# wzx99/DCFP

Measured on AMD Instinct MI355X. Metric: training images/sec at 1024x2048 DeepLabv3-R101, higher is better.
Workload: dtype f32; 1 GPU; DeepLabv3-resnet101+ASPP os8, 4x3x1024x2048 per GPU, CE+0.4*deepsup CE (fused upsample), 3x3 stride-1 convs with >= 256 channels as fp32 Winograd F(2x2,3x3) (fwd / dgrad / wgrad), all other convs direct implicit GEMM, EIC step, SGD m0.9 wd5e-4; global_batch=4, parallelism=dp1

## Files before the change

### dcfp_amd/_lib.py

```python
import ctypes as C
import os
import subprocess
import threading

_HERE = os.path.dirname(os.path.abspath(__file__))
LIB_PATH = os.environ.get("DCFP_LIB") or os.path.join(_HERE, "libdcfp_hip.so")
CSRC = os.path.join(_HERE, "csrc")

_lib = None
_lock = threading.Lock()


class ConvDesc(C.Structure):
    _fields_ = [(n, C.c_int32) for n in
                ("N", "Cin", "H", "W", "Cout", "KH", "KW", "stride", "pad", "dil", "Hout", "Wout",
                 "x_pitch", "dy_pitch")]


class ConvF16Desc(C.Structure):
    _fields_ = [(n, C.c_int32) for n in
                ("N", "H", "W", "Cin8", "x_pitch", "Cout", "K", "stride", "pad", "dil", "Hout", "Wout",
                 "y_pitch", "y_off", "res_pitch", "res_off", "relu")]


class ConvF8Desc(C.Structure):
    _fields_ = [(n, C.c_int32) for n in
                ("N", "H", "W", "Cin16", "x_pitch", "Cout", "K", "stride", "pad", "dil", "Hout", "Wout",
                 "y_pitch", "y_off", "res_pitch", "res_off", "relu")] + [("res_mul", C.c_float)]


class EicEntry(C.Structure):
    _fields_ = [("gamma", C.c_void_p), ("grad", C.c_void_p), ("eic", C.c_void_p),
                ("n", C.c_int32), ("pad_", C.c_int32)]


class SgdEntry(C.Structure):
    _fields_ = [("param", C.c_void_p), ("grad", C.c_void_p), ("momentum_buf", C.c_void_p),
                ("n", C.c_int64), ("first_chunk", C.c_int64),
                ("weight_decay", C.c_float), ("pad_", C.c_int32)]


class GateEntry(C.Structure):
    _fields_ = [("gamma", C.c_void_p), ("beta", C.c_void_p), ("ggrad", C.c_void_p), ("bgrad", C.c_void_p),
                ("score", C.c_void_p), ("n", C.c_int32), ("pad_", C.c_int32)]


class FilterEntry(C.Structure):
    _fields_ = [("w", C.c_void_p), ("g", C.c_void_p), ("out", C.c_void_p), ("rows", C.c_int32), ("K", C.c_int32),
                ("first_unit", C.c_int64)]


class FpgmEntry(C.Structure):
    _fields_ = [("w", C.c_void_p), ("out", C.c_void_p), ("C", C.c_int32), ("K", C.c_int32),
                ("first_tile", C.c_int64), ("ws_off", C.c_int64)]


class AdamEntry(C.Structure):
    _fields_ = [("param", C.c_void_p), ("grad", C.c_void_p), ("exp_avg", C.c_void_p), ("exp_avg_sq", C.c_void_p),
                ("n", C.c_int64), ("first_chunk", C.c_int64)]


class BnRunning(C.Structure):
    _fields_ = [("running_mean", C.c_void_p), ("running_var", C.c_void_p), ("num_batches_tracked", C.c_void_p),
                ("momentum", C.c_float), ("pad_", C.c_int32)]


class WpEntry(C.Structure):
    _fields_ = [("w", C.c_void_p), ("wp", C.c_void_p), ("first_block", C.c_int64), ("n_blocks", C.c_int64)] + \
               [(n, C.c_int32) for n in ("T", "Ck", "CkP", "M", "Mpad", "sAm", "sAc", "perm8")]


class AugTap(C.Structure):
    _fields_ = [(n, C.c_int32) for n in ("src", "c0", "c1", "lsrc")]


class AugSample(C.Structure):
    _fields_ = [("image", C.c_void_p), ("label", C.c_void_p)] + \
               [(n, C.c_int32) for n in ("src_h", "src_w", "col_off", "row_off", "lut_a_off", "lut_b_off",
                                         "hsv_flags", "hue_delta")] + \
               [("sat_alpha", C.c_float), ("pad_", C.c_int32)]


class CcSample(C.Structure):
    _fields_ = [("label", C.c_void_p)] + \
               [(n, C.c_int32) for n in ("src_h", "src_w", "dst_h", "dst_w", "Hp", "Wp", "row_off", "col_off", "cls",
                                         "pad_")] + \
               [("work_off", C.c_int64)]


class VoteMap(C.Structure):
    _fields_ = [("logits", C.c_void_p)] + [(n, C.c_int32) for n in ("h", "w", "hs", "ws", "flip")] + \
               [("weight", C.c_float)]


class SlidePass(C.Structure):
    _fields_ = [("logits", C.c_void_p)] + \
               [(n, C.c_int32) for n in ("lh", "lw", "hs", "ws", "th", "tw", "rows", "cols", "flip")] + \
               [("weight", C.c_float)]


SLIDE_MAX_PASSES, SLIDE_MAX_TILES_PER_AXIS = 16, 32
AUG_SATURATION, AUG_HUE = 1, 2
SGD_CHUNK = 16384
FILTER_ABS_SUM, FILTER_L2, FILTER_DOT_SQ_ACC = 0, 1, 2
FPGM_TILE = 64
CONV_FWD, CONV_DGRAD, CONV_WGRAD = 0, 1, 2
E_BADDESC, E_UNSUPPORTED, E_WORKSPACE = -1, -2, -3

_P, _I, _L, _F, _Z = C.c_void_p, C.c_int, C.c_int64, C.c_float, C.c_size_t
_D = C.POINTER(ConvDesc)
_R = C.POINTER(BnRunning)
_H = C.POINTER(ConvF16Desc)
_H8 = C.POINTER(ConvF8Desc)

SIGNATURES = {
    "dcfp_abi_version": (_I, []),
    "dcfp_conv2d_workspace_bytes": (_Z, [_D, _I]),
    "dcfp_conv2d_wp_layout": (_I, [_D, _I, C.POINTER(WpEntry)]),
    "dcfp_conv2d_permute_weights_multi_f32": (_I, [_P, _I, _L, _P]),
    "dcfp_conv2d_pitch_supported": (_I, [_D]),
    "dcfp_conv2d_kernel_name": (_I, [_D, _I, C.c_char_p, _I]),
    "dcfp_conv2d_executed_fraction": (C.c_double, [_D, _I]),
    "dcfp_conv2d_workspace_is_scratch": (_I, [_D, _I]),
    "dcfp_conv2d_dgrad_fanin_supported": (_I, [_D]),
    "dcfp_conv2d_dgrad_fanin_f32_nchw": (_I, [_D, _P, _L, _P, _P, _P, _P, _P, _Z, _I, _P]),
    "dcfp_conv2d_dgrad_fanin_red_slots": (_L, [_D]),
    "dcfp_conv2d_dgrad_fanin_red_f32_nchw": (_I, [_D, _P, _L, _P, _P, _P, _P, _P, _P, _P, _P, _P, _Z, _I, _P]),
    "dcfp_bn_bwd_sums_from_partials_f32": (_I, [_P, _L, _I, _P, _F, _P, _P, _P, _P, _P]),
    "dcfp_conv2d_xform_bytes": (_Z, [_D]),
    "dcfp_conv2d_fwd_keep_f32_nchw": (_I, [_D, _P, _P, _P, _L, _P, _Z, _P, _P, _Z, _P]),
    "dcfp_conv2d_wgrad_kept_f32_nchw": (_I, [_D, _P, _L, _P, _Z, _P, _P, _Z, _P]),
    "dcfp_conv2d_fwd_f32_nchw": (_I, [_D, _P, _P, _P, _P, _L, _P, _Z, _I, _P]),
    "dcfp_conv2d_fwd_fused_f32_nchw": (_I, [_D, _P, _P, _P, _P, _P, _I, _P, _P, _Z, _I, _P]),
    "dcfp_conv2d_dgrad_f32_nchw": (_I, [_D, _P, _L, _P, _P, _I, _P, _Z, _I, _P]),
    "dcfp_conv2d_wgrad_f32_nchw": (_I, [_D, _P, _L, _P, _P, _P, _P, _Z, _P]),
    "dcfp_bn_workspace_bytes": (_Z, [_I, _I, _I]),
    "dcfp_bn_stats_f32": (_I, [_P, _L, _I, _I, _I, _P, _P, _R, _P, _Z, _P]),
    "dcfp_bn_apply_f32": (_I, [_P, _P, _P, _P, _P, _F, _P, _I, _P, _L, _I, _I, _I, _I, _I, _P]),
    "dcfp_bn_bwd_reduce_f32": (_I, [_P, _L, _P, _P, _L, _P, _P, _P, _P, _F, _I, _I, _I, _I, _P, _P, _P, _P,
                                    _P, _Z, _P]),
    "dcfp_bn_update_running_f32": (_I, [_P, _P, _I, _F, _F, _P, _P, _P, _P]),
    "dcfp_syncbn_combine_f32": (_I, [_P, _I, _I, _P, _P, _P, _R, _P]),
    "dcfp_syncbn_p2p_mailbox_bytes": (_Z, [_I, _I]),
    "dcfp_p2p_alloc": (_I, [_Z, _I, C.POINTER(C.c_void_p)]),
    "dcfp_p2p_free": (_I, [_P]),
    "dcfp_p2p_export": (_I, [_P, _P]),
    "dcfp_p2p_import": (_I, [_P, C.POINTER(C.c_void_p)]),
    "dcfp_p2p_unmap": (_I, [_P]),
    "dcfp_syncbn_p2p_exchange_f32": (_I, [C.POINTER(C.c_void_p), _I, _I, C.c_uint32, _I, _P, _I, _I, _P, _R,
                                          C.c_uint32, _P, _P]),
    "dcfp_bn_apply_relu_mask_f32": (_I, [_P, _P, _P, _P, _P, _F, _P, _P, _P, _I, _I, _I, _P]),
    "dcfp_conv2d_fwd_stat_slots": (_L, [_D, _P, _L]),
    "dcfp_conv2d_fwd_stats_f32_nchw": (_I, [_D, _P, _P, _P, _L, _P, _P, _Z, _I, _P]),
    "dcfp_bn_stats_from_partials_f32": (_I, [_P, _L, _I, _I, _P, _P, _R, _P]),
    "dcfp_bn_bwd_apply_f32": (_I, [_P, _L, _P, _P, _L, _P, _P, _P, _P, _F, _P, _P, _F, _P, _I, _P, _P,
                                   _I, _I, _I, _I, _I, _P]),
    "dcfp_bn_bwd_fused_sync_bytes": (_Z, [_I, _I, _I]),
    "dcfp_bn_bwd_fused_f32": (_I, [_P, _L, _P, _P, _L, _P, _P, _P, _P, _F, _F, _I, _P, _P, _I, _I, _I, _I, _I,
                                   _P, _P, _P, _P, _P, _Z, C.c_uint32, C.c_uint32, _P, _P]),
    "dcfp_maxpool3x3s2_fwd_f32": (_I, [_P, _P, _P, _I, _I, _I, _I, _I, _I, _P]),
    "dcfp_maxpool3x3s2_bwd_f32": (_I, [_P, _P, _P, _I, _I, _I, _I, _I, _I, _P]),
    "dcfp_rowsum_f32": (_I, [_P, _L, _P, _F, _I, _I, _I, _P]),
    "dcfp_broadcast_hw_f32": (_I, [_P, _F, _P, _L, _I, _I, _I, _I, _P]),
    "dcfp_add_f32": (_I, [_P, _P, _P, _L, _P]),
    "dcfp_channel_scale_f32": (_I, [_P, _P, _P, _I, _I, _I, _P]),
    "dcfp_upsample_bilinear_fwd_f32": (_I, [_P, _P, _I, _I, _I, _I, _I, _I, _I, _P]),
    "dcfp_upsample_bilinear_bwd_f32": (_I, [_P, _P, _I, _I, _I, _I, _I, _I, _I, _P]),
    "dcfp_resize_bilinear_into_f32": (_I, [_P, _L, _I, _I, _I, _I, _P, _L, _I, _I, _I, _I, _P]),
    "dcfp_resize_bilinear_adjoint_f32": (_I, [_P, _L, _I, _I, _I, _I, _I, _P, _L, _I, _I, _I, _I, _P]),
    "dcfp_ppm_pool_f32": (_I, [_P, _I, _I, _I, _I, _I, _P, _P, _I, _P, _L, _I, _P]),
    "dcfp_ppm_pool_adjoint_f32": (_I, [_P, _I, _I, _I, _I, _I, _P, _P, _L, _I, _P, _P]),
    "dcfp_ppm_resize_adjoint_f32": (_I, [_P, _L, _I, _I, _I, _I, _I, _P, _P, _I, _P]),
    "dcfp_upsample_ce_workspace_bytes": (_Z, [_I, _I, _I]),
    "dcfp_upsample_ce_fwd_f32": (_I, [_P, _P, _P, _I, _I, _I, _I, _I, _I, _I, _I, _P, _P, _P, _P,
                                      _Z, _P]),
    "dcfp_upsample_ce_bwd_f32": (_I, [_P, _P, _P, _I, _I, _I, _I, _I, _I, _I, _I, _P, _P, _P, _P]),
    "dcfp_upsample_ce_bwd_plan": (_I, [_I, _I, _I, _I, _I, _I, C.POINTER(C.c_int), C.POINTER(C.c_int),
                                       C.POINTER(C.c_int)]),
    "dcfp_ohem_zoom_gt_prob_f32": (_I, [_P, _P, _P, _I, _I, _I, _I, _I, _I, _I, _I, _I, _P, _P, _P]),
    "dcfp_ohem_threshold_f32": (_I, [_P, _P, _L, _I, _F, _L, _P, _P]),
    "dcfp_ohem_keep_mask_u8": (_I, [_P, _P, _L, _P, _P]),
    "dcfp_upsample_margin_f32": (_I, [_P, _I, _I, _I, _I, _I, _I, _I, _P, _P]),
    "dcfp_maxfilter2d_s1_f32": (_I, [_P, _P, _I, _I, _I, _I, _P]),
    "dcfp_upsample_wce_workspace_bytes": (_Z, [_I, _I, _I]),
    "dcfp_upsample_wce_fwd_f32": (_I, [_P, _P, _P, _I, _I, _I, _I, _I, _I, _I, _I, _P, _P, _P, _Z, _P]),
    "dcfp_upsample_wce_bwd_f32": (_I, [_P, _P, _P, _I, _I, _I, _I, _I, _I, _I, _I, _P, _P, _P, _P]),
    "dcfp_upsample_argmax_f32": (_I, [_P, _I, _I, _I, _I, _I, _I, _I, _P, _P]),
    "dcfp_confusion_matrix_i64": (_I, [_P, _P, _I, _L, _I, _P, _P]),
    "dcfp_vote_multiscale_f32": (_I, [C.POINTER(VoteMap), _I, _I, _I, _I, _I, _I, _I, _I, _P, _P, _P, _I, _P, _P]),
    "dcfp_gather_tiles_f32": (_I, [_P, _I, _I, _I, _I, _P, _I, _P, _I, _I, _I, _I, _P, _P]),
    "dcfp_vote_sliding_f32": (_I, [C.POINTER(SlidePass), _I, _P, _P, _I, _I, _I, _I, _I, _I, _I, _P, _P, _P, _I, _P, _P]),
    "dcfp_label_boundary_workspace_bytes": (_Z, [_I, _I, _I]),
    "dcfp_label_boundary_i32": (_I, [_P, _P, _I, _I, _I, _I, _I, _I, _P, _Z, _P]),
    "dcfp_label_boundary_i64": (_I, [_P, _P, _I, _I, _I, _I, _I, _I, _P, _Z, _P]),
    "dcfp_png_deflate_bound": (_Z, [_I, _I]),
    "dcfp_png_deflate_workspace_bytes": (_Z, [_I, _I, _I, _I]),
    "dcfp_png_deflate_labels_i32": (_I, [_P, _I, _I, _I, _P, _I, _P, _Z, _P, _P, _P, _Z, _P]),
    "dcfp_augment_u8_to_f32_nchw": (_I, [C.POINTER(AugSample), _I, _I, _I, _P, _L, _P, _L, _P, _L, _P, _I, _P, _P, _P, _P]),
    "dcfp_balance_weight_f32": (_I, [_P, _P, _P, _I, _L, _I, _I, _I, C.c_double, _P, _P]),
    "dcfp_components_workspace_bytes": (_Z, [_I, _I]),
    "dcfp_label_components_u8": (_I, [C.POINTER(CcSample), _I, _P, _L, _P, _P, _Z, _P, _P]),
    "dcfp_component_pixel_i32": (_I, [C.POINTER(CcSample), _I, _P, _Z, _P, _P, _P, _P, _P]),
    "dcfp_eic_update_f32": (_I, [_P, _I, _F, _F, _P]),
    "dcfp_sgd_momentum_f32": (_I, [_P, _I, _L, _F, _F, _I, _P]),
    "dcfp_adamw_f32": (_I, [_P, _I, _L, _F, _F, _F, _F, _F, _F, _F, _P]),
    "dcfp_conv2d_fwd_f16_nhwc": (_I, [_H, _P, _P, _P, _P, _P, _P]),
    "dcfp_conv2d_fwd_f16_nhwc_to_f32_nchw": (_I, [_H, _P, _P, _P, _P, _P]),
    "dcfp_maxpool3x3s2_nhwc_f16": (_I, [_P, _P, _I, _I, _I, _I, _I, _I, _I, _I, _P]),
    "dcfp_avgpool_nhwc_f16_workspace_bytes": (_Z, [_I, _I, _L]),
    "dcfp_avgpool_nhwc_f16": (_I, [_P, _P, _I, _L, _I, _I, _I, _P, _Z, _P]),
    "dcfp_broadcast_nhwc_f16": (_I, [_P, _I, _P, _I, _L, _I, _I, _I, _P]),
    "dcfp_nchw_f32_to_nhwc_f16": (_I, [_P, _P, _I, _I, _I, _I, _I, _P]),
    "dcfp_conv2d_fwd_f8_nhwc": (_I, [_H8, _P, _P, _P, _P, _P, _P, _P]),
    "dcfp_conv2d_fwd_f8_nhwc_to_f32_nchw": (_I, [_H8, _P, _P, _P, _P, _P, _P]),
    "dcfp_cast_nhwc_f16_to_f8": (_I, [_P, _I, _P, _I, _I, _L, _I, _F, _P]),
    "dcfp_maxpool3x3s2_nhwc_f8": (_I, [_P, _P, _I, _I, _I, _I, _I, _I, _I, _I, _P]),
    "dcfp_avgpool_nhwc_f8_to_f16": (_I, [_P, _P, _I, _L, _I, _I, _I, _F, _P, _Z, _P]),
    "dcfp_broadcast_nhwc_f16_to_f8": (_I, [_P, _I, _P, _I, _L, _I, _I, _I, _F, _P]),
    "dcfp_resize_bilinear_nhwc_f16": (_I, [_P, _I, _I, _I, _I, _I, _P, _I, _I, _I, _I, _I, _P]),
    "dcfp_pyramid_pool_nhwc_f16_workspace_bytes": (_Z, [_I, _I, _I, _I, _I, _P]),
    "dcfp_pyramid_pool_nhwc_f16": (_I, [_P, _I, _I, _I, _I, _I, _I, _I, _P, _P, _P, _P, _Z, _P]),
    "dcfp_kd_workspace_bytes": (_Z, [_I, _I, _I, _I, _I]),
    "dcfp_kd_fwd_f32": (_I, [_P, _P, _I, _I, _I, _I, _I, _F, _P, _Z, _P, _P, _P]),
    "dcfp_lovasz_workspace_bytes": (_Z, [_I, _I]),
    "dcfp_lovasz_hist_f32": (_I, [_P, _P, _I, _I, _I, _I, _I, _I, _I, _I, _I, _P, _P, _Z, _P]),
    "dcfp_lovasz_scan_f32": (_I, [_I, _I, _P, _Z, _P, _P, _P]),
    "dcfp_lovasz_bwd_f32": (_I, [_P, _P, _I, _I, _I, _I, _I, _I, _I, _I, _I, _P, _P, _P, _P, _P, _P]),
    "dcfp_lovasz_errors_u32": (_I, [_P, _P, _I, _I, _I, _I, _I, _I, _I, _I, _P, _P]),
    "dcfp_gate_taylor_f32": (_I, [_P, _I, _P]),
    "dcfp_gate_l1reg_f32": (_I, [_P, _I, _F, _P]),
    "dcfp_filter_reduce_units": (_L, [_I, _I]),
    "dcfp_filter_reduce_f32": (_I, [_P, _I, _L, _I, _P]),
    "dcfp_fpgm_workspace_bytes": (_Z, [_I]),
    "dcfp_fpgm_f32": (_I, [_P, _I, _L, _P, _Z, _P]),
}


def build(verbose=False):
    cmd = ["make", "-C", CSRC, "-j", str(min(8, os.cpu_count() or 1))]
    r = subprocess.run(cmd, capture_output=True, text=True)
    if verbose or r.returncode != 0:
        print(r.stdout[-4000:])
        print(r.stderr[-4000:])
    if r.returncode != 0:
        raise RuntimeError("building libdcfp_hip.so failed")
    return LIB_PATH


def lib():
    global _lib
    if _lib is not None:
        return _lib
    with _lock:
        if _lib is not None:
            return _lib
        if not os.path.exists(LIB_PATH):
            raise RuntimeError(
                f"{LIB_PATH} not found: run `python -c 'import __graft_entry__ as g; g.build()'` "
                "(or `make -C dcfp_amd/csrc`). dcfp_amd has no non-HIP fallback.")
        try:
            import torch
        except Exception:
            pass
        handle = C.CDLL(LIB_PATH, mode=C.RTLD_GLOBAL)
        for name, (res, args) in SIGNATURES.items():
            fn = getattr(handle, name)
            fn.restype = res
            fn.argtypes = args
        _lib = handle
    return _lib


def check(status, what):
    if status != 0:
        kind = "descriptor/shape" if status < 0 else "hipError_t"
        raise RuntimeError(f"{what} failed: status {status} ({kind})")
```

### dcfp_amd/csrc/conv_igemm.hip

```cpp
#include "common.h"
#include <string.h>
#include <stdio.h>
#include <stdlib.h>

namespace {

int check_desc(const DcfpConvDesc* d) {
    if (!d) return DCFP_E_BADDESC;
    if (d->N <= 0 || d->Cin <= 0 || d->Cout <= 0 || d->H <= 0 || d->W <= 0 || d->stride <= 0 ||
        d->dil <= 0 || d->pad < 0)
        return DCFP_E_BADDESC;
    if (d->KH != d->KW || (d->KH != 1 && d->KH != 3)) return DCFP_E_UNSUPPORTED;
    const int ho = (d->H + 2 * d->pad - d->dil * (d->KH - 1) - 1) / d->stride + 1;
    const int wo = (d->W + 2 * d->pad - d->dil * (d->KW - 1) - 1) / d->stride + 1;
    if (ho != d->Hout || wo != d->Wout || ho <= 0 || wo <= 0) return DCFP_E_BADDESC;
    if ((d->x_pitch != 0 && (d->x_pitch < d->W || (d->x_pitch & 3))) ||
        (d->dy_pitch != 0 && (d->dy_pitch < d->Wout || (d->dy_pitch & 3))))
        return DCFP_E_BADDESC;
    if ((long long)d->Cin * d->H * (d->x_pitch ? d->x_pitch : d->W) >= (1LL << 29) ||
        (long long)d->Cout * d->Hout * (d->dy_pitch ? d->dy_pitch : d->Wout) >= (1LL << 29) ||
        (long long)d->Cout * d->Cin * d->KH * d->KW >= (1LL << 29))
        return DCFP_E_UNSUPPORTED;
    return DCFP_OK;
}

}

extern "C" int dcfp_abi_version(void) { return 2; }

int dcfp_wgrad_kernel_name(const DcfpConvDesc* d, char* buf, int buf_len);
double dcfp_wgrad_exec_fraction(const DcfpConvDesc* d);
double dcfp_igemm2_exec_fraction(int T, int M, int Ck, int N, int Hi, int Wi, int Ho, int Wo, int sn, int sd,
                                 int off0, int offstep, bool pitched);
size_t dcfp_igemm2_workspace_bytes(int T, int M, int Ck, long long px, int sd);
const char* dcfp_igemm2_cfg_args(int M, long long px, int sd);
int dcfp_igemm2_run(const float* in, long long in_nstride, const float* w, int sAm, int sAc,
                    const float* bias, float* out, long long out_nstride, int N, int M, int Ck, int T,
                    int Hi, int Wi, int Ho, int Wo, int sn, int sd, int off0, int offstep,
                    int accumulate, void* workspace, size_t workspace_bytes, hipStream_t stream,
                    const float* scale = nullptr, const float* shift = nullptr,
                    const float* residual = nullptr, int relu = 0, float* stat_part = nullptr, int wp_valid = 0,
                    int in_pitch = 0, long long wp_nstride = 0, const float* fan_src = nullptr,
                    const unsigned long long* fan_mask = nullptr, const Igemm2Red* red = nullptr);
bool dcfp_wino_ok(int N, int H, int W, int d, int M, int Ck);
size_t dcfp_wino_workspace_bytes(int N, int H, int W, int d, int M, int Ck);
double dcfp_wino_exec_fraction(int N, int H, int W, int d, int M, int Ck);
int dcfp_wino_run(const float* in, long long in_nstride, int in_pitch, const float* w, int sAm, int sAc, int flip,
                  float* out, long long out_nstride, int N, int M, int Ck, int H, int W, int d, int accumulate,
                  void* workspace, size_t workspace_bytes, hipStream_t stream, float* xform_out = nullptr,
                  float* stat_part = nullptr, const float* scale = nullptr, const float* shift = nullptr,
                  const float* residual = nullptr, int relu = 0, int wp_valid = 0);
long long dcfp_wino_stat_slots(int N, int H, int W, int d);
bool dcfp_stem_shape(const DcfpConvDesc* d);
int dcfp_stem_fwd(const DcfpConvDesc* d, const float* x, const float* w, const float* bias, float* y, long long y_nstride,
                  hipStream_t stream, float* stat_part = nullptr);
long long dcfp_stem_stat_slots(const DcfpConvDesc* d, const float* y, long long y_nstride);
bool dcfp_gemv_shape(const DcfpConvDesc* d);
int dcfp_gemv_fwd(const DcfpConvDesc* d, const float* x, const float* w, const float* bias, float* y, long long y_nstride,
                  hipStream_t stream);
int dcfp_gemv_dgrad(const DcfpConvDesc* d, const float* dy, long long dy_nstride, const float* w, float* dx, int accumulate,
                    hipStream_t stream);
bool dcfp_wino_fused_ok(int N, int H, int W, int d, int M, int Ck, long long in_nstride, int pitch);
size_t dcfp_wino_fused_workspace_bytes(int N, int H, int W, int d, int M, int Ck);
void dcfp_wino_fused_pads(int N, int H, int W, int d, int M, int Ck, int* CkP, int* Mpad);
size_t dcfp_wino_xform_bytes(int N, int H, int W, int d, int C);
bool dcfp_wgrad_is_winograd(const DcfpConvDesc* d);
bool dcfp_wgrad_wants_xform(const DcfpConvDesc* d);
long long dcfp_igemm2_stat_slots(int M, int P, int N, long long out_nstride, const float* out);
bool dcfp_igemm2_dma_shape(int T, int M, int Ck, int P, long long px, int sn, int sd, int off0, int HiWi, int Wo);
bool dcfp_igemm2_persist();
void dcfp_igemm2_wp_layout(int T, int M, int Ck, int P, long long px, int sn, int sd, int off0, int offstep, int HiWi,
                           int Wo, bool pitched, int sAm, int sAc, DcfpWpEntry* e);
bool dcfp_igemm2_use_dma8(int T, int M, int P, long long px, int sn, int sd, int off0, int offstep, int HiWi,
                          int Wo, bool pitched);
int dcfp_igemm2_permute_multi(const DcfpWpEntry* table, int n, long long total_blocks, hipStream_t stream);


size_t dcfp_igemm3_workspace_bytes(int T, int M, int Ck);
int dcfp_igemm3_run(const float* in, long long in_nstride, const float* w, int sAm, int sAc,
                    const float* bias, float* out, long long out_nstride, int N, int M, int Ck, int T,
                    int Hi, int Wi, int Ho, int Wo, int off0, int offstep, int accumulate,
                    void* workspace, size_t workspace_bytes, hipStream_t stream,
                    const float* scale = nullptr, const float* shift = nullptr,
                    const float* residual = nullptr, int relu = 0, int wp_valid = 0);
int dcfp_igemm2_cfg_id(int M, long long px, int sd);
static bool math_bf16x3() {
    static const bool v = [] { const char* e = getenv("DCFP_CONV_MATH"); return e && !strcmp(e, "bf16x3"); }();
    return v;
}
static bool igemm3_ok(int M, long long px, int sn, int sd) {
    return math_bf16x3() && sn == 1 && sd == 1 && dcfp_igemm2_cfg_id(M, px, sd) == 4;
}

static int wino_kind(const DcfpConvDesc* d, int pass) {
    static const int mode = [] { const char* e = getenv("DCFP_CONV_WINOGRAD"); return e ? atoi(e) : 1; }();
    if (mode == 0) return 0;
    if (d->KH != 3 || d->KW != 3 || d->stride != 1 || d->pad != d->dil || d->Hout != d->H || d->Wout != d->W)
        return 0;
    if (math_bf16x3()) return 0;
    const bool fwd = pass == DCFP_CONV_FWD;
    const int M = fwd ? d->Cout : d->Cin, Ck = fwd ? d->Cin : d->Cout;
    const int sp = fwd ? d->x_pitch : d->dy_pitch;
    const bool pitched = sp && sp != d->W;
    const bool three = dcfp_wino_ok(d->N, d->H, d->W, d->dil, M, Ck);
    const bool fused = dcfp_wino_fused_ok(d->N, d->H, d->W, d->dil, M, Ck, (long long)Ck * d->H * (sp ? sp : d->W), sp);
    if (!three && !fused) return 0;
    if (mode == 2) return three ? 1 : 2;
    const double nominal = 2.0 * d->N * (double)d->H * d->W * (double)M * Ck * 9.0;
    const double f_direct = fwd ? dcfp_igemm2_exec_fraction(9, M, Ck, d->N, d->H, d->W, d->H, d->W, 1, 1, -d->pad, d->dil, pitched)
                                : dcfp_igemm2_exec_fraction(9, M, Ck, d->N, d->H, d->W, d->H, d->W, 1, 1, d->pad, -d->dil, pitched);
    const double t_direct = nominal * f_direct / (M % 256 != 0 ? 115e12 : 143e12);
    const double f_wino = dcfp_wino_exec_fraction(d->N, d->H, d->W, d->dil, M, Ck);
    double t_wino = 1e30;
    if (three) {
        const double tiles = f_wino * 9.0 / 16.0 * d->N * (double)d->H * d->W;
        const double rate = Ck <= 256 ? (M >= 1024 ? 130e12 : 118e12) : (M <= 256 ? 127e12 : 135e12);
        const double pix = (double)d->N * d->H * d->W;
        const double t_in = (4.0 * pix * Ck + 64.0 * tiles * Ck) / 4.2e12;
        const double t_out = (64.0 * tiles * M + 4.0 * pix * M * (fwd ? 1.0 : 2.0)) / 5.4e12;
        const double mpad = (double)((M + 255) / 256 * 256) / M;
        t_wino = nominal * f_wino * mpad / rate + t_in + t_out + 20e-6;
    }
    if (fused) {
        const double nk = (double)((Ck + 15) / 16 * 2);
        const double mpad = (double)((M + 63) / 64 * 64) / M;
        const double t_f = nominal * f_wino * mpad / (125e12 * nk / (nk + 4.0)) + 10e-6;
        if (t_f < t_wino) t_wino = t_f;
    }
    if (!(t_wino < 0.97 * t_direct)) return 0;
    return three ? 1 : 2;
}
static bool wino_pass(const DcfpConvDesc* d, int pass) { return wino_kind(d, pass) != 0; }

static bool wino_keeps_u(const DcfpConvDesc* d, int pass) {
    static const bool on = [] { const char* e = getenv("DCFP_WINO_KEEP_U"); return !e || atoi(e) != 0; }();
    if (!on || (pass != DCFP_CONV_FWD && pass != DCFP_CONV_DGRAD) || !wino_pass(d, pass)) return false;
    const bool fwd = pass == DCFP_CONV_FWD;
    const int M = fwd ? d->Cout : d->Cin, Ck = fwd ? d->Cin : d->Cout;
    const int sp = fwd ? d->x_pitch : d->dy_pitch;
    if (!dcfp_wino_fused_ok(d->N, d->H, d->W, d->dil, M, Ck, (long long)Ck * d->H * (sp ? sp : d->W), sp)) return false;
    if (fwd && Ck > 256 && dcfp_wino_ok(d->N, d->H, d->W, d->dil, M, Ck) && dcfp_conv2d_xform_bytes(d) > 0) return false;
    return true;
}

extern "C" int dcfp_conv2d_workspace_is_scratch(const DcfpConvDesc* d, int pass) {
    if (check_desc(d) != DCFP_OK || pass == DCFP_CONV_WGRAD) return 0;
    return (wino_pass(d, pass) && !wino_keeps_u(d, pass)) ? 1 : 0;
}

size_t dcfp_conv2d_fwd_dgrad_workspace_bytes_(const DcfpConvDesc* d, int pass) {
    if (check_desc(d) != DCFP_OK) return 0;
    if (const int wk = wino_kind(d, pass)) {
        const int M = pass == DCFP_CONV_FWD ? d->Cout : d->Cin, Ck = pass == DCFP_CONV_FWD ? d->Cin : d->Cout;
        if (wino_keeps_u(d, pass)) {
            const size_t u = dcfp_wino_fused_workspace_bytes(d->N, d->H, d->W, d->dil, M, Ck);
            const size_t direct = dcfp_igemm2_workspace_bytes(9, M, Ck, (long long)d->N * d->H * d->W, 1);
            return u > direct ? u : direct;
        }
        return wk == 1 ? dcfp_wino_workspace_bytes(d->N, d->H, d->W, d->dil, M, Ck)
                       : dcfp_wino_fused_workspace_bytes(d->N, d->H, d->W, d->dil, M, Ck);
    }
    const int T = d->KH * d->KW;
    size_t b2, b3 = 0;
    if (pass == DCFP_CONV_FWD) {
        const long long px = (long long)d->N * d->Hout * d->Wout;
        b2 = dcfp_igemm2_workspace_bytes(T, d->Cout, d->Cin, px, 1);
        if (igemm3_ok(d->Cout, px, d->stride, 1)) b3 = dcfp_igemm3_workspace_bytes(T, d->Cout, d->Cin);
    } else {
        const long long px = (long long)d->N * d->H * d->W;
        b2 = dcfp_igemm2_workspace_bytes(T, d->Cin, d->Cout, px, d->stride);
        if (igemm3_ok(d->Cin, px, 1, d->stride)) b3 = dcfp_igemm3_workspace_bytes(T, d->Cin, d->Cout);
    }
    return b2 > b3 ? b2 : b3;
}

extern "C" int dcfp_conv2d_kernel_name(const DcfpConvDesc* d, int pass, char* buf, int buf_len) {
    int rc = check_desc(d);
    if (rc) return rc;
    if (!buf || buf_len <= 0) return DCFP_E_BADDESC;
    if (dcfp_gemv_shape(d)) return snprintf(buf, buf_len, "gemv_1x1_map_kernel");
    if (pass == DCFP_CONV_WGRAD) return dcfp_wgrad_kernel_name(d, buf, buf_len);
    if (pass == DCFP_CONV_FWD && dcfp_stem_shape(d)) return snprintf(buf, buf_len, "stem_fwd_kernel");
    if (const int wk = wino_kind(d, pass))
        return wk == 1 ? snprintf(buf, buf_len, "winograd_f2x2_3x3 (igemm2_dma1p_kernel<false,true>)")
                       : snprintf(buf, buf_len, "winograd_f2x2_3x3 fused (wino_fused_kernel)");
    const int M = pass == DCFP_CONV_FWD ? d->Cout : d->Cin;
    const long long px = pass == DCFP_CONV_FWD ? (long long)d->N * d->Hout * d->Wout : (long long)d->N * d->H * d->W;
    const int sd = pass == DCFP_CONV_FWD ? 1 : d->stride;
    if (igemm3_ok(M, px, pass == DCFP_CONV_FWD ? d->stride : 1, sd))
        return snprintf(buf, buf_len, "igemm3_kernel<%d>", d->KH * d->KW);
    const int P = pass == DCFP_CONV_FWD ? d->Hout * d->Wout : d->H * d->W;
    const int HiWi = pass == DCFP_CONV_FWD ? d->H * d->W : d->Hout * d->Wout;
    const int Ck = pass == DCFP_CONV_FWD ? d->Cin : d->Cout;
    {
        const int sp = pass == DCFP_CONV_FWD ? d->x_pitch : d->dy_pitch;
        const bool pitched = sp && sp != (pass == DCFP_CONV_FWD ? d->W : d->Wout);
        if (dcfp_igemm2_use_dma8(d->KH * d->KW, M, P, px, pass == DCFP_CONV_FWD ? d->stride : 1, sd,
                                 pass == DCFP_CONV_FWD ? -d->pad : d->pad, pass == DCFP_CONV_FWD ? d->dil : -d->dil,
                                 HiWi, pass == DCFP_CONV_FWD ? d->Wout : d->W, pitched))
            return snprintf(buf, buf_len, "igemm2_dma8_kernel<%d>", d->KH * d->KW);
    }
    if (dcfp_igemm2_dma_shape(d->KH * d->KW, M, Ck, P, px, pass == DCFP_CONV_FWD ? d->stride : 1, sd, d->pad, HiWi,
                              pass == DCFP_CONV_FWD ? d->Wout : d->W)) {
        if (d->KH == 1 && dcfp_igemm2_persist()) return snprintf(buf, buf_len, "igemm2_dma1p_kernel");
        const int src_pitch = pass == DCFP_CONV_FWD ? d->x_pitch : d->dy_pitch;
        const bool pitched = src_pitch && src_pitch != (pass == DCFP_CONV_FWD ? d->W : d->Wout);
        return snprintf(buf, buf_len, "igemm2_dma_kernel<%d,%s>", d->KH * d->KW,
                        (d->KH == 3 && ((d->pad | d->dil) & 3) != 0 && !pitched) ? "true" : "false");
    }
    return snprintf(buf, buf_len, "igemm2_kernel<%d,%s>", d->KH * d->KW, dcfp_igemm2_cfg_args(M, px, sd));
}

extern "C" double dcfp_conv2d_executed_fraction(const DcfpConvDesc* d, int pass) {
    if (check_desc(d) != DCFP_OK) return 1.0;
    if (pass == DCFP_CONV_WGRAD) return dcfp_wgrad_exec_fraction(d);
    const bool fwd = pass == DCFP_CONV_FWD;
    if (wino_pass(d, pass))
        return fwd ? dcfp_wino_exec_fraction(d->N, d->H, d->W, d->dil, d->Cout, d->Cin)
                   : dcfp_wino_exec_fraction(d->N, d->H, d->W, d->dil, d->Cin, d->Cout);
    const int M = fwd ? d->Cout : d->Cin;
    const long long px = fwd ? (long long)d->N * d->Hout * d->Wout : (long long)d->N * d->H * d->W;
    if (igemm3_ok(M, px, fwd ? d->stride : 1, fwd ? 1 : d->stride)) return 1.0;
    const int sp = fwd ? d->x_pitch : d->dy_pitch;
    const bool pitched = sp && sp != (fwd ? d->W : d->Wout);
    return fwd ? dcfp_igemm2_exec_fraction(d->KH * d->KW, d->Cout, d->Cin, d->N, d->H, d->W, d->Hout, d->Wout, d->stride, 1,
                                           -d->pad, d->dil, pitched)
               : dcfp_igemm2_exec_fraction(d->KH * d->KW, d->Cin, d->Cout, d->N, d->Hout, d->Wout, d->H, d->W, 1, d->stride,
                                           d->pad, -d->dil, pitched);
}

extern "C" int64_t dcfp_conv2d_fwd_stat_slots(const DcfpConvDesc* d, const float* y, int64_t y_nstride);

extern "C" size_t dcfp_conv2d_xform_bytes(const DcfpConvDesc* d) {
    if (check_desc(d) != DCFP_OK) return 0;
    if (!wino_pass(d, DCFP_CONV_FWD) || !dcfp_wgrad_wants_xform(d)) return 0;
    return dcfp_wino_xform_bytes(d->N, d->H, d->W, d->dil, d->Cin);
}

extern "C" int dcfp_conv2d_fwd_keep_f32_nchw(const DcfpConvDesc* d, const float* x, const float* w, float* y,
                                             int64_t y_nstride, float* xform_out, size_t xform_bytes,
                                             float* stat_partials, void* workspace, size_t workspace_bytes,
                                             dcfp_stream_t stream) {
    int rc = check_desc(d);
    if (rc) return rc;
    if (!x || !w || !y || !xform_out) return DCFP_E_BADDESC;
    const size_t need = dcfp_conv2d_xform_bytes(d);
    if (need == 0) return DCFP_E_UNSUPPORTED;
    if (xform_bytes < need) return DCFP_E_WORKSPACE;
    const int T = 9;
    return dcfp_wino_run(x, (long long)d->Cin * d->H * (d->x_pitch ? d->x_pitch : d->W), d->x_pitch, w, d->Cin * T, T, 0, y,
                         y_nstride ? y_nstride : (long long)d->Cout * d->Hout * d->Wout, d->N, d->Cout, d->Cin, d->H, d->W,
                         d->dil, 0, workspace, workspace_bytes, dcfp_s(stream), xform_out,
                         (stat_partials && dcfp_conv2d_fwd_stat_slots(d, y, y_nstride) > 0) ? stat_partials : nullptr);
}

extern "C" int dcfp_conv2d_fwd_f32_nchw(const DcfpConvDesc* d, const float* x, const float* w,
                                        const float* bias, float* y, int64_t y_nstride,
                                        void* workspace, size_t workspace_bytes, int wp_valid,
                                        dcfp_stream_t stream) {
    int rc = check_desc(d);
    if (rc) return rc;
    if (!x || !w || !y) return DCFP_E_BADDESC;
    const int T = d->KH * d->KW;
    if (d->x_pitch && d->x_pitch != d->W && math_bf16x3()) return DCFP_E_UNSUPPORTED;
    if (dcfp_gemv_shape(d)) return dcfp_gemv_fwd(d, x, w, bias, y, y_nstride, dcfp_s(stream));
    if (dcfp_stem_shape(d)) return dcfp_stem_fwd(d, x, w, bias, y, y_nstride, dcfp_s(stream));
    if (!bias && wino_pass(d, DCFP_CONV_FWD))
        return dcfp_wino_run(x, (long long)d->Cin * d->H * (d->x_pitch ? d->x_pitch : d->W), d->x_pitch, w, d->Cin * T, T,
                             0, y, y_nstride ? y_nstride : (long long)d->Cout * d->Hout * d->Wout, d->N, d->Cout,
                             d->Cin, d->H, d->W, d->dil, 0, workspace, workspace_bytes, dcfp_s(stream), nullptr, nullptr,
                             nullptr, nullptr, nullptr, 0, (wp_valid && wino_keeps_u(d, DCFP_CONV_FWD)) ? 1 : 0);
    if (!bias && igemm3_ok(d->Cout, (long long)d->N * d->Hout * d->Wout, d->stride, 1))
        return dcfp_igemm3_run(x, (long long)d->Cin * d->H * d->W, w, d->Cin * T, T, bias, y,
                               y_nstride ? y_nstride : (long long)d->Cout * d->Hout * d->Wout, d->N,
                               d->Cout, d->Cin, T, d->H, d->W, d->Hout, d->Wout, -d->pad, d->dil, 0,
                               workspace, workspace_bytes, dcfp_s(stream), nullptr, nullptr, nullptr, 0, wp_valid);
    return dcfp_igemm2_run(x, (long long)d->Cin * d->H * (d->x_pitch ? d->x_pitch : d->W), w, d->Cin * T, T, bias, y,
                           y_nstride ? y_nstride : (long long)d->Cout * d->Hout * d->Wout, d->N,
                           d->Cout, d->Cin, T, d->H, d->W, d->Hout, d->Wout, d->stride, 1, -d->pad,
                           d->dil, 0, workspace, workspace_bytes, dcfp_s(stream), nullptr, nullptr, nullptr, 0,
                           nullptr, wp_valid, d->x_pitch);
}

extern "C" int64_t dcfp_conv2d_fwd_stat_slots(const DcfpConvDesc* d, const float* y, int64_t y_nstride) {
    if (check_desc(d) != DCFP_OK) return 0;
    if (dcfp_stem_shape(d)) return dcfp_stem_stat_slots(d, y, y_nstride);
    if (wino_pass(d, DCFP_CONV_FWD))
        return (y_nstride % 4 == 0 && dcfp_aligned16(y)) ? dcfp_wino_stat_slots(d->N, d->H, d->W, d->dil) : 0;
    if (igemm3_ok(d->Cout, (long long)d->N * d->Hout * d->Wout, d->stride, 1)) return 0;
    return dcfp_igemm2_stat_slots(d->Cout, d->Hout * d->Wout, d->N,
                                  y_nstride ? y_nstride : (long long)d->Cout * d->Hout * d->Wout, y);
}

extern "C" int dcfp_conv2d_fwd_stats_f32_nchw(const DcfpConvDesc* d, const float* x, const float* w,
                                              float* y, int64_t y_nstride, float* stat_partials,
                                              void* workspace, size_t workspace_bytes, int wp_valid,
                                              dcfp_stream_t stream) {
    int rc = check_desc(d);
    if (rc) return rc;
    if (!x || !w || !y || !stat_partials) return DCFP_E_BADDESC;
    if (dcfp_conv2d_fwd_stat_slots(d, y, y_nstride) <= 0) return DCFP_E_UNSUPPORTED;
    const int T = d->KH * d->KW;
    if (dcfp_stem_shape(d)) return dcfp_stem_fwd(d, x, w, nullptr, y, y_nstride, dcfp_s(stream), stat_partials);
    if (wino_pass(d, DCFP_CONV_FWD))
        return dcfp_wino_run(x, (long long)d->Cin * d->H * (d->x_pitch ? d->x_pitch : d->W), d->x_pitch, w, d->Cin * T, T, 0, y,
                             y_nstride ? y_nstride : (long long)d->Cout * d->Hout * d->Wout, d->N, d->Cout, d->Cin, d->H, d->W,
                             d->dil, 0, workspace, workspace_bytes, dcfp_s(stream), nullptr, stat_partials, nullptr, nullptr,
                             nullptr, 0, (wp_valid && wino_keeps_u(d, DCFP_CONV_FWD)) ? 1 : 0);
    return dcfp_igemm2_run(x, (long long)d->Cin * d->H * (d->x_pitch ? d->x_pitch : d->W), w, d->Cin * T, T, nullptr, y,
                           y_nstride ? y_nstride : (long long)d->Cout * d->Hout * d->Wout, d->N,
                           d->Cout, d->Cin, T, d->H, d->W, d->Hout, d->Wout, d->stride, 1, -d->pad,
                           d->dil, 0, workspace, workspace_bytes, dcfp_s(stream), nullptr, nullptr,
                           nullptr, 0, stat_partials, wp_valid, d->x_pitch);
}

extern "C" int dcfp_conv2d_dgrad_f32_nchw(const DcfpConvDesc* d, const float* dy,
                                          int64_t dy_nstride, const float* w, float* dx,
                                          int accumulate, void* workspace, size_t workspace_bytes,
                                          int wp_valid, dcfp_stream_t stream) {
    int rc = check_desc(d);
    if (rc) return rc;
    if (!dy || !w || !dx) return DCFP_E_BADDESC;
    const int T = d->KH * d->KW;
    if (d->dy_pitch && d->dy_pitch != d->Wout && math_bf16x3()) return DCFP_E_UNSUPPORTED;
    if (dcfp_gemv_shape(d)) return dcfp_gemv_dgrad(d, dy, dy_nstride, w, dx, accumulate ? 1 : 0, dcfp_s(stream));
    if (wino_pass(d, DCFP_CONV_DGRAD))
        return dcfp_wino_run(dy, dy_nstride ? dy_nstride : (long long)d->Cout * d->Hout * (d->dy_pitch ? d->dy_pitch : d->Wout),
                             d->dy_pitch, w, T, d->Cin * T, 1, dx, (long long)d->Cin * d->H * d->W, d->N, d->Cin, d->Cout,
                             d->H, d->W, d->dil, accumulate ? 1 : 0, workspace, workspace_bytes, dcfp_s(stream), nullptr,
                             nullptr, nullptr, nullptr, nullptr, 0, (wp_valid && wino_keeps_u(d, DCFP_CONV_DGRAD)) ? 1 : 0);
    if (igemm3_ok(d->Cin, (long long)d->N * d->H * d->W, 1, d->stride))
        return dcfp_igemm3_run(dy, dy_nstride ? dy_nstride : (long long)d->Cout * d->Hout * d->Wout, w,
                               T, d->Cin * T, nullptr, dx, (long long)d->Cin * d->H * d->W, d->N, d->Cin,
                               d->Cout, T, d->Hout, d->Wout, d->H, d->W, d->pad, -d->dil,
                               accumulate ? 1 : 0, workspace, workspace_bytes, dcfp_s(stream), nullptr, nullptr,
                               nullptr, 0, wp_valid);
    return dcfp_igemm2_run(dy, dy_nstride ? dy_nstride : (long long)d->Cout * d->Hout * (d->dy_pitch ? d->dy_pitch : d->Wout), w,
                           T, d->Cin * T, nullptr, dx, (long long)d->Cin * d->H * d->W, d->N, d->Cin,
                           d->Cout, T, d->Hout, d->Wout, d->H, d->W, 1, d->stride, d->pad, -d->dil,
                           accumulate ? 1 : 0, workspace, workspace_bytes, dcfp_s(stream), nullptr, nullptr, nullptr, 0,
                           nullptr, wp_valid, d->dy_pitch);
}

extern "C" int dcfp_conv2d_dgrad_fanin_supported(const DcfpConvDesc* d) {
    if (check_desc(d) != DCFP_OK || d->KH != 1 || d->stride != 1 || d->pad != 0 || math_bf16x3()) return 0;
    const int P = d->H * d->W;
    const long long px = (long long)d->N * P;
    if (d->Cin % 256 != 0 || P % 256 != 0 || !dcfp_igemm2_persist()) return 0;
    if (igemm3_ok(d->Cin, px, 1, 1)) return 0;
    return dcfp_igemm2_dma_shape(1, d->Cin, d->Cout, P, px, 1, 1, 0, P, d->W) ? 1 : 0;
}

extern "C" int dcfp_conv2d_dgrad_fanin_f32_nchw(const DcfpConvDesc* d, const float* dy, int64_t dy_nstride, const float* w,
                                                float* dx, const float* fan_src, const void* fan_mask, void* workspace,
                                                size_t workspace_bytes, int wp_valid, dcfp_stream_t stream) {
    int rc = check_desc(d);
    if (rc) return rc;
    if (!dy || !w || !dx || !fan_src || !fan_mask) return DCFP_E_BADDESC;
    if (!dcfp_conv2d_dgrad_fanin_supported(d)) return DCFP_E_UNSUPPORTED;
    return dcfp_igemm2_run(dy, dy_nstride ? dy_nstride : (long long)d->Cout * d->Hout * d->Wout, w, 1, d->Cin, nullptr, dx,
                           (long long)d->Cin * d->H * d->W, d->N, d->Cin, d->Cout, 1, d->Hout, d->Wout, d->H, d->W, 1, 1, 0, -1,
                           0, workspace, workspace_bytes, dcfp_s(stream), nullptr, nullptr, nullptr, 0, nullptr, wp_valid, 0, 0,
                           fan_src, static_cast<const unsigned long long*>(fan_mask));
}

bool dcfp_igemm2p_fan_red_ok(int Mpad, int CkP);
int dcfp_igemm2_ck_pad();
extern "C" int64_t dcfp_conv2d_dgrad_fanin_red_slots(const DcfpConvDesc* d) {
    if (!dcfp_conv2d_dgrad_fanin_supported(d)) return 0;
    const int pad = dcfp_igemm2_ck_pad();
    const int ckp = (d->Cout + pad - 1) / pad * pad;
    if (!dcfp_igemm2p_fan_red_ok(d->Cin, ckp)) return 0;
    return (int64_t)d->N * d->H * d->W / 128;
}

extern "C" int dcfp_conv2d_dgrad_fanin_red_f32_nchw(const DcfpConvDesc* d, const float* dy, int64_t dy_nstride,
                                                    const float* w, float* dx, const float* fan_src, const void* fan_mask,
                                                    const float* red_x, const void* red_mask, const float* red_mean,
                                                    float* red_part, void* workspace, size_t workspace_bytes, int wp_valid,
                                                    dcfp_stream_t stream) {
    int rc = check_desc(d);
    if (rc) return rc;
    if (!dy || !w || !dx || !fan_src || !fan_mask || !red_x || !red_mask || !red_mean || !red_part) return DCFP_E_BADDESC;
    if (dcfp_conv2d_dgrad_fanin_red_slots(d) <= 0) return DCFP_E_UNSUPPORTED;
    if (reinterpret_cast<uintptr_t>(red_part) & 7u) return DCFP_E_BADDESC;
    const Igemm2Red red = {red_x, static_cast<const unsigned long long*>(red_mask), red_mean, red_part};
    return dcfp_igemm2_run(dy, dy_nstride ? dy_nstride : (long long)d->Cout * d->Hout * d->Wout, w, 1, d->Cin, nullptr, dx,
                           (long long)d->Cin * d->H * d->W, d->N, d->Cin, d->Cout, 1, d->Hout, d->Wout, d->H, d->W, 1, 1, 0, -1,
                           0, workspace, workspace_bytes, dcfp_s(stream), nullptr, nullptr, nullptr, 0, nullptr, wp_valid, 0, 0,
                           fan_src, static_cast<const unsigned long long*>(fan_mask), &red);
}

extern "C" int dcfp_conv2d_fwd_fused_f32_nchw(const DcfpConvDesc* d, const float* x, const float* w,
                                              const float* scale, const float* shift,
                                              const float* residual, int relu, float* y,
                                              void* workspace, size_t workspace_bytes, int wp_valid,
                                              dcfp_stream_t stream) {
    int rc = check_desc(d);
    if (rc) return rc;
    if (!x || !w || !y || !scale || !shift) return DCFP_E_BADDESC;
    const int T = d->KH * d->KW;
    if (wino_pass(d, DCFP_CONV_FWD))
        return dcfp_wino_run(x, (long long)d->Cin * d->H * d->W, 0, w, d->Cin * T, T, 0, y,
                             (long long)d->Cout * d->Hout * d->Wout, d->N, d->Cout, d->Cin, d->H, d->W, d->dil, 0, workspace,
                             workspace_bytes, dcfp_s(stream), nullptr, nullptr, scale, shift, residual, relu ? 1 : 0);
    if (igemm3_ok(d->Cout, (long long)d->N * d->Hout * d->Wout, d->stride, 1))
        return dcfp_igemm3_run(x, (long long)d->Cin * d->H * d->W, w, d->Cin * T, T, nullptr, y,
                               (long long)d->Cout * d->Hout * d->Wout, d->N, d->Cout, d->Cin, T, d->H, d->W,
                               d->Hout, d->Wout, -d->pad, d->dil, 0, workspace, workspace_bytes,
                               dcfp_s(stream), scale, shift, residual, relu ? 1 : 0, wp_valid);
    return dcfp_igemm2_run(x, (long long)d->Cin * d->H * d->W, w, d->Cin * T, T, nullptr, y,
                           (long long)d->Cout * d->Hout * d->Wout, d->N, d->Cout, d->Cin, T, d->H, d->W,
                           d->Hout, d->Wout, d->stride, 1, -d->pad, d->dil, 0, workspace, workspace_bytes,
                           dcfp_s(stream), scale, shift, residual, relu ? 1 : 0, nullptr, wp_valid);
}

extern "C" int dcfp_conv2d_wp_layout(const DcfpConvDesc* d, int pass, DcfpWpEntry* e) {
    int rc = check_desc(d);
    if (rc) return rc;
    if (!e || (pass != DCFP_CONV_FWD && pass != DCFP_CONV_DGRAD)) return DCFP_E_BADDESC;
    const int T = d->KH * d->KW;
    if (wino_pass(d, pass)) {
        if (!wino_keeps_u(d, pass)) return DCFP_E_UNSUPPORTED;
        const bool fwd = pass == DCFP_CONV_FWD;
        e->T = 16; e->M = fwd ? d->Cout : d->Cin; e->Ck = fwd ? d->Cin : d->Cout;
        dcfp_wino_fused_pads(d->N, d->H, d->W, d->dil, e->M, e->Ck, &e->CkP, &e->Mpad);
        e->sAm = fwd ? d->Cin * T : T; e->sAc = fwd ? T : d->Cin * T; e->perm8 = fwd ? 2 : 3;
        const long long pairs = (long long)e->CkP * e->Mpad;
        e->n_blocks = (pairs + DCFP_WP_BLOCK_ELEMS - 1) / DCFP_WP_BLOCK_ELEMS;
        return DCFP_OK;
    }
    if (pass == DCFP_CONV_FWD) {
        const long long px = (long long)d->N * d->Hout * d->Wout;
        if (igemm3_ok(d->Cout, px, d->stride, 1)) return DCFP_E_UNSUPPORTED;
        dcfp_igemm2_wp_layout(T, d->Cout, d->Cin, d->Hout * d->Wout, px, d->stride, 1, -d->pad, d->dil, d->H * d->W,
                              d->Wout, d->x_pitch && d->x_pitch != d->W, d->Cin * T, T, e);
    } else {
        const long long px = (long long)d->N * d->H * d->W;
        if (igemm3_ok(d->Cin, px, 1, d->stride)) return DCFP_E_UNSUPPORTED;
        dcfp_igemm2_wp_layout(T, d->Cin, d->Cout, d->H * d->W, px, 1, d->stride, d->pad, -d->dil, d->Hout * d->Wout,
                              d->W, d->dy_pitch && d->dy_pitch != d->Wout, T, d->Cin * T, e);
    }
    const long long total = (long long)e->T * e->CkP * e->Mpad;
    e->n_blocks = (total + DCFP_WP_BLOCK_ELEMS - 1) / DCFP_WP_BLOCK_ELEMS;
    return DCFP_OK;
}

extern "C" int dcfp_conv2d_permute_weights_multi_f32(const DcfpWpEntry* table, int n, int64_t total_blocks,
                                                     dcfp_stream_t stream) {
    if (n == 0 || total_blocks == 0) return DCFP_OK;
    if (!table || n < 0 || total_blocks < 0 || total_blocks > 0x7fffffffLL) return DCFP_E_BADDESC;
    return dcfp_igemm2_permute_multi(table, n, total_blocks, dcfp_s(stream));
}

bool dcfp_wgrad_pitch_ok(const DcfpConvDesc* d);

extern "C" int dcfp_conv2d_pitch_supported(const DcfpConvDesc* d) {
    if (check_desc(d) != DCFP_OK || math_bf16x3()) return 0;
    if (d->KH != 3 || d->stride != 1 || d->pad != d->dil || d->Hout != d->H || d->Wout != d->W) return 0;
    const int xp = d->x_pitch ? d->x_pitch : d->W, dp = d->dy_pitch ? d->dy_pitch : d->Wout;
    if (xp < d->W + d->pad && xp != d->W) return 0;
    if (dp < d->Wout + d->pad && dp != d->Wout) return 0;
    const long long pxo = (long long)d->N * d->Hout * d->Wout, pxi = (long long)d->N * d->H * d->W;
    if (xp != d->W && dp != d->Wout && wino_kind(d, DCFP_CONV_FWD) == 2 && wino_kind(d, DCFP_CONV_DGRAD) == 2)
        return dcfp_wgrad_pitch_ok(d) ? 1 : 0;
    if (!dcfp_igemm2_dma_shape(9, d->Cout, d->Cin, d->Hout * d->Wout, pxo, 1, 1, -d->pad, d->H * d->W, d->Wout) &&
        !dcfp_igemm2_use_dma8(9, d->Cout, d->Hout * d->Wout, pxo, 1, 1, -d->pad, d->dil, d->H * d->W, d->Wout, true))
        return 0;
    if (!dcfp_igemm2_dma_shape(9, d->Cin, d->Cout, d->H * d->W, pxi, 1, 1, d->pad, d->Hout * d->Wout, d->W) &&
        !dcfp_igemm2_use_dma8(9, d->Cin, d->H * d->W, pxi, 1, 1, d->pad, -d->dil, d->Hout * d->Wout, d->W, true))
        return 0;
    return dcfp_wgrad_pitch_ok(d) ? 1 : 0;
}
```

### dcfp_amd/csrc/conv_igemm2.hip

```cpp
#include "igemm2_common.h"
#include <queue>
#include <vector>
#include <stdio.h>
#include <stdlib.h>

namespace {

__device__ __forceinline__ int wp_row(int m, int perm8) {
    if (!perm8) return m;
    const int j = m & 255;
    return (m & ~255) + 32 * (j & 7) + (j >> 3);
}

__global__ void __launch_bounds__(256)
permute_weights_kernel(const float* __restrict__ w, float* __restrict__ wp, int T, int Ck, int CkP,
                       int M, int Mpad, int sAm, int sAc, int perm8) {
    const long long total = (long long)T * CkP * Mpad;
    for (long long i = (long long)blockIdx.x * 256 + threadIdx.x; i < total;
         i += (long long)gridDim.x * 256) {
        const int m = wp_row((int)(i % Mpad), perm8);
        const long long r = i / Mpad;
        const int c = (int)(r % CkP);
        const int t = (int)(r / CkP);
        float v = 0.f;
        if (m < M && c < Ck) v = w[(long long)m * sAm + (long long)c * sAc + t];
        wp[i] = v;
    }
}

constexpr int kWpBlockElems = DCFP_WP_BLOCK_ELEMS;
__global__ void __launch_bounds__(256)
permute_weights_multi_kernel(const DcfpWpEntry* __restrict__ table, int n) {
    const long long blk = blockIdx.x;
    int lo = 0, hi = n - 1;
    while (lo < hi) {
        const int mid = (lo + hi + 1) >> 1;
        if (table[mid].first_block <= blk) lo = mid; else hi = mid - 1;
    }
    const DcfpWpEntry e = table[lo];
    const long long base = (blk - e.first_block) * kWpBlockElems;
    if (e.perm8 >= 2) {
        const long long pairs = (long long)e.CkP * e.Mpad;
#pragma unroll 1
        for (int u = 0; u < kWpBlockElems / 256; ++u) {
            const long long i = base + u * 256 + threadIdx.x;
            if (i >= pairs) return;
            wino_filter2_pair(e.w, e.sAm, e.sAc, e.perm8 == 3, e.M, e.Ck, e.Mpad, i, e.wp);
        }
        return;
    }
    const long long total = (long long)e.T * e.CkP * e.Mpad;
#pragma unroll
    for (int u = 0; u < kWpBlockElems / 256; ++u) {
        const long long i = base + u * 256 + threadIdx.x;
        if (i >= total) return;
        const int m = wp_row((int)(i % e.Mpad), e.perm8);
        const long long r = i / e.Mpad;
        const int c = (int)(r % e.CkP);
        const int t = (int)(r / e.CkP);
        float v = 0.f;
        if (m < e.M && c < e.Ck) v = e.w[(long long)m * e.sAm + (long long)c * e.sAc + t];
        e.wp[i] = v;
    }
}

__device__ __forceinline__ float half_xor(float v, int mask) {
    switch (mask) {
        case 1: return __builtin_bit_cast(float, __builtin_amdgcn_ds_swizzle(__builtin_bit_cast(int, v), (1 << 10) | 0x1f));
        case 2: return __builtin_bit_cast(float, __builtin_amdgcn_ds_swizzle(__builtin_bit_cast(int, v), (2 << 10) | 0x1f));
        case 4: return __builtin_bit_cast(float, __builtin_amdgcn_ds_swizzle(__builtin_bit_cast(int, v), (4 << 10) | 0x1f));
        case 8: return __builtin_bit_cast(float, __builtin_amdgcn_ds_swizzle(__builtin_bit_cast(int, v), (8 << 10) | 0x1f));
        default: return __builtin_bit_cast(float, __builtin_amdgcn_ds_swizzle(__builtin_bit_cast(int, v), (16 << 10) | 0x1f));
    }
}

template <int TAPS, int TM, int TN, int WM, int WN, bool SD, bool ACC, int KB = 16>
__global__ void __launch_bounds__(64 * WM * WN, (TM * TN <= 8 && WM * WN == 4 && !ACC) ? 2 : 1)
igemm2_kernel(const Igemm2Params p) {
    constexpr int BK = KB;
    constexpr int NPART = BK / 4;
    constexpr int BM = WM * TM * 32, BN = WN * TN * 32, NT = 64 * WM * WN;
    constexpr int AX = BM / 4;
    constexpr int AROWS = (NT / AX) < BK ? (NT / AX) : BK;
    constexpr int APASS = BK / AROWS;
    constexpr int TX = BN / 4, TY = NT / TX, RPT = BK / TY;
    static_assert(APASS >= 1 && APASS * AROWS == BK, "A loader shape");
    static_assert(TY >= 1 && RPT >= 1 && TY * RPT == BK, "B loader shape");

    extern __shared__ __attribute__((aligned(16))) float smem[];
    float* As = smem;
    float* Bs = smem + 2 * BK * BM;

    const int group = 8 * p.tiles_m;
    const int g = blockIdx.x / group, local = blockIdx.x - g * group;
    const int nt = g * 8 + (local & 7);
    const int mt = local >> 3;
    if (nt >= p.tiles_n_total) return;
    const int img = nt / p.tiles_per_img;
    const int ti_img = nt - img * p.tiles_per_img;
    const int phase = SD ? (p.zfold ? p.zfold - 1 : ti_img / p.tiles_per_phase) : 0;
    const int ph_h = SD ? phase / p.sd : 0, ph_w = SD ? phase - ph_h * p.sd : 0;
    const int p0 = (SD && !p.zfold ? ti_img - phase * p.tiles_per_phase : ti_img) * BN;
    const int m0 = mt * BM;

    const int tid = threadIdx.x;
    const int lane = tid & 63, wid = tid >> 6;
    const int wm = wid / WN, wn = wid - wm * WN;
    const int l31 = lane & 31, lhi = lane >> 5;

    const int ax = tid % AX, ay = tid / AX;
    const bool a_on = ay < BK;
    const float* a_src = p.wp + m0 + 4 * ax;

    const int tx = tid % TX, ty = tid / TX;
    int bh[4], bw[4];
    bool pv[4];
#pragma unroll
    for (int e = 0; e < 4; ++e) {
        const int pp = p0 + 4 * tx + e;
        if constexpr (SD) {
            const int a = pp / p.Wc, b = pp - a * p.Wc;
            const int oh = a * p.sd + ph_h, ow = b * p.sd + ph_w;
            pv[e] = a < p.Hc && oh < p.Ho && ow < p.Wo;
            bh[e] = oh * p.sn;
            bw[e] = ow * p.sn;
        } else {
            pv[e] = pp < p.P;
            const int oh = pp / p.Wo;
            const int ow = pp - oh * p.Wo;
            bh[e] = oh * p.sn;
            bw[e] = ow * p.sn;
        }
    }
    const int HiWi = p.Hi * p.Wi;
    const __amdgpu_buffer_rsrc_t b_rsrc = __builtin_amdgcn_make_buffer_rsrc(
        const_cast<float*>(p.in + (long long)img * p.in_nstride), 0, p.Ck * HiWi * 4, 0x00020000);

    const int ksteps_per_tap = p.CkP / BK;
    unsigned long long tap_list = 0;
    int ntaps = TAPS;
    if constexpr (SD) {
        ntaps = 0;
        for (int t = 0; t < TAPS; ++t) {
            const int kh = (TAPS == 9) ? t / 3 : 0, kw = (TAPS == 9) ? t - kh * 3 : 0;
            const int sh = ph_h + p.off0 + kh * p.offstep, sw = ph_w + p.off0 + kw * p.offstep;
            if (sh % p.sd == 0 && sw % p.sd == 0) {
                tap_list |= (unsigned long long)t << (4 * ntaps);
                ++ntaps;
            }
        }
    }
    const int nk = ntaps * ksteps_per_tap;

    unsigned boff[4];
    bool bvec = false;
    f32x4 areg[APASS];
    float breg[RPT][4];

    auto set_tap = [&](int t) {
        const int kh = (TAPS == 9) ? t / 3 : 0;
        const int kw = (TAPS == 9) ? t - kh * 3 : 0;
        const int offh = p.off0 + kh * p.offstep;
        const int offw = p.off0 + kw * p.offstep;
#pragma unroll
        for (int e = 0; e < 4; ++e) {
            int hh = bh[e] + offh, ww = bw[e] + offw;
            bool ok = pv[e] && hh >= 0 && ww >= 0;
            if (SD) {
                ok = ok && (hh % p.sd == 0) && (ww % p.sd == 0);
                hh /= p.sd;
                ww /= p.sd;
            }
            ok = ok && hh < p.Hi && ww < p.Wi;
            boff[e] = ok ? (unsigned)(hh * p.Wi + ww) * 4u : kOob;
        }
        const bool none = boff[0] == kOob && boff[1] == kOob && boff[2] == kOob && boff[3] == kOob;
        const bool run = boff[0] != kOob && boff[1] == boff[0] + 4u && boff[2] == boff[0] + 8u &&
                         boff[3] == boff[0] + 12u;
        bvec = none || run;
    };
    auto load_part = [&](int kt, auto part_) {
        constexpr int PART = decltype(part_)::value;
#ifdef DCFP_TAP_INNER
        const int cb = kt / TAPS;
        const int t = kt - cb * TAPS;
        const int c0 = cb * BK;
        if (PART == 0 && (TAPS > 1 || kt == 0)) set_tap(t);
#else
        const int ti_ = kt / ksteps_per_tap;
        const int c0 = (kt - ti_ * ksteps_per_tap) * BK;
        const int t = SD ? (int)((tap_list >> (4 * ti_)) & 15ull) : ti_;
        if (PART == 0 && c0 == 0) set_tap(t);
#endif
        static_for<0, APASS>([&](auto j_) {
            constexpr int j = decltype(j_)::value;
            if constexpr ((j % NPART) == PART) {
                if (a_on)
                    areg[j] = *reinterpret_cast<const f32x4*>(
                        a_src + (long long)(t * p.CkP + c0 + ay + AROWS * j) * p.Mpad);
            }
        });
        static_for<0, RPT>([&](auto q_) {
            constexpr int q = decltype(q_)::value;
// ... 656 lines not shown
size_t dcfp_igemm2_workspace_bytes(int T, int M, int Ck, long long px, int sd) {
    return (size_t)T * round_up(Ck, ck_pad()) * round_up(M, 256) * sizeof(float);
}

int dcfp_igemm2_cfg_id(int M, long long px, int sd) { return pick_cfg(M, px, sd).id; }

long long dcfp_igemm2_stat_slots(int M, int P, int N, long long out_nstride, const float* out) {
    const TileCfg c = pick_cfg(M, (long long)N * P, 1);
    if (c.id != 0 && c.id != 1 && c.id != 2 && c.id != 4) return 0;
    if (M % c.bm != 0 || P % c.bn != 0 || P % 4 != 0 || out_nstride % 4 != 0 || !dcfp_aligned16(out)) return 0;
    return (long long)N * (P / c.bn) * (c.bn / 128);
}

const char* dcfp_igemm2_cfg_args(int M, long long px, int sd) {
    switch (pick_cfg(M, px, sd).id) {
        case 0: return "1,4,1,4,0";
        case 1: return "2,4,1,4,0";
        case 2: return "2,4,2,2,0";
        case 3: return "2,2,2,2,0";
        case 4: return "4,4,2,2,0";
        default: return "2,4,2,2,1";
    }
}

bool dcfp_igemm2_use_dma8(int T, int M, int P, long long px, int sn, int sd, int off0, int offstep, int HiWi,
                          int Wo, bool pitched) {
    static const int mode = [] { const char* e = getenv("DCFP_IGEMM_DMA8"); return e ? atoi(e) : 1; }();
    static const bool dma = [] { const char* e = getenv("DCFP_IGEMM_DMA"); return !e || atoi(e) != 0; }();
    const bool on = mode != 0;
    if (!on || !dma || deep_k() || sn != 1 || sd != 1 || HiWi != P || Wo % 4 != 0) return false;
    if (T == 1 ? off0 != 0 : ((((off0 | offstep) & 3) != 0 && !pitched) || off0 + 2 * offstep != -off0)) return false;
    const long long tiles = ((long long)P + 255) / 256 * (px / P) * ((M + 255) / 256);
    if (tiles < 192) return false;
    if (mode == 2) return true;
    const TileCfg c = pick_cfg(M, px, sd);
    if (M % c.bm == 0) return false;
    if (c.bm <= 64) return true;
    const long long old_rows = (long long)((M + c.bm - 1) / c.bm) * c.bm, new_rows = (long long)((M + 31) / 32) * 32;
    return 10 * new_rows <= 9 * old_rows;
}

bool dcfp_igemm2_dma_shape(int T, int M, int Ck, int P, long long px, int sn, int sd, int off0, int HiWi, int Wo);

static int tile_live_rows(const Igemm2Params& p, int ti) {
    int oh_lo, oh_hi;
    if (p.tile2d) {
        const int rows = 256 >> p.tile2d;
        oh_lo = (ti / (p.Wi >> p.tile2d)) * rows;
        oh_hi = oh_lo + rows - 1;
    } else {
        const int p0 = ti * 256;
        oh_lo = p0 / p.Wo;
        oh_hi = (p0 + 255 < p.P ? p0 + 255 : p.P - 1) / p.Wo;
    }
    oh_hi = oh_hi < p.Ho ? oh_hi : p.Ho - 1;
    int lo = 0, hi = 2;
    auto live = [&](int kh) { const int o = p.off0 + kh * p.offstep; return oh_hi + o >= 0 && oh_lo + o < p.Hi; };
    while (lo < 2 && !live(lo)) ++lo;
    while (hi > lo && !live(hi)) --hi;
    return hi - lo + 1;
}

static int pick_tapskip(const Igemm2Params& p, int bn) {
    static const int forced = [] { const char* e = getenv("DCFP_IGEMM_TAPSKIP"); return e ? atoi(e) : -1; }();
    if (bn != 256) return 0;
    const bool t2d = p.tile2d != 0;
    if (forced >= 0) return (forced == 2 && t2d) ? 1 : forced;
    if (t2d) return 1;
    struct Key { int Ho, Wo, Hi, N, tm, off0, offstep, mode; };
    thread_local Key cache[16];
    thread_local int used = 0;
    for (int i = 0; i < used; ++i) {
        const Key& k = cache[i];
        if (k.Ho == p.Ho && k.Wo == p.Wo && k.Hi == p.Hi && k.N == p.N && k.tm == p.tiles_m && k.off0 == p.off0 &&
            k.offstep == p.offstep)
            return k.mode;
    }
    const int T = p.tiles_per_img, cus = dcfp_num_cus();
    std::vector<float> work((size_t)T);
    bool any = false;
    for (int ti = 0; ti < T; ++ti) {
        const int live = tile_live_rows(p, ti);
        any |= live < 3;
        work[ti] = (float)live + 0.1f;
    }
    int mode = 0;
    if (any) {
        auto makespan = [&](int m) {
            std::priority_queue<float, std::vector<float>, std::greater<float>> free_at;
            for (int i = 0; i < cus; ++i) free_at.push(0.f);
            float end = 0.f;
            const long long groups = ((long long)p.tiles_n_total + 7) / 8;
            for (long long g = 0; g < groups; ++g)
                for (int mt = 0; mt < p.tiles_m; ++mt)
                    for (int l = 0; l < 8; ++l) {
                        const long long nt = g * 8 + l;
                        if (nt >= p.tiles_n_total) continue;
                        int ti = (int)(nt % T);
                        if (m == 2) {
                            const int k = (int)(nt / p.N), c = T >> 1;
                            ti = (k & 1) ? c - 1 - (k >> 1) : c + (k >> 1);
                        }
                        const float t0 = free_at.top();
                        free_at.pop();
                        const float t1 = t0 + (m == 0 ? 3.1f : work[ti]);
                        free_at.push(t1);
                        end = t1 > end ? t1 : end;
                    }
            return end;
        };
        const float m0 = makespan(0), m1 = makespan(1), m2 = makespan(2);
        const float best = m2 <= m1 ? m2 : m1;
        if (best <= 0.97f * m0) mode = m2 <= m1 ? 2 : 1;
    }
    if (used < 16) {
        cache[used++] = Key{p.Ho, p.Wo, p.Hi, p.N, p.tiles_m, p.off0, p.offstep, mode};
    }
    return mode;
}

double dcfp_igemm2_exec_fraction(int T, int M, int Ck, int N, int Hi, int Wi, int Ho, int Wo, int sn, int sd,
                                 int off0, int offstep, bool pitched) {
    if (T != 9 || sn != 1 || sd != 1) return 1.0;
    const long long px = (long long)N * Ho * Wo;
    const bool d8 = dcfp_igemm2_use_dma8(T, M, Ho * Wo, px, sn, sd, off0, offstep, Hi * Wi, Wo, pitched);
    if (!d8 && !dcfp_igemm2_dma_shape(T, M, Ck, Ho * Wo, px, sn, sd, off0, Hi * Wi, Wo)) return 1.0;
    Igemm2Params p = {};
    p.N = N; p.Hi = Hi; p.Wi = Wi; p.Ho = Ho; p.Wo = Wo; p.P = Ho * Wo; p.off0 = off0; p.offstep = offstep;
    p.tiles_per_img = (p.P + 255) / 256; p.tiles_n_total = p.tiles_per_img * N; p.tiles_m = (M + 255) / 256;
    {
        static const int t2d = [] { const char* e = getenv("DCFP_IGEMM_2D"); return e ? atoi(e) : 5; }();
        const bool fits = (t2d == 4 || t2d == 5) && Hi % (256 >> t2d) == 0 && Wi % (1 << t2d) == 0;
        p.tile2d = (!d8 && fits && !pitched && ((off0 | offstep) & 3) != 0 && Ho == Hi && Wo == Wi) ? t2d : 0;
    }
    if (pick_tapskip(p, 256) == 0) return 1.0;
    long long live = 0;
    for (int ti = 0; ti < p.tiles_per_img; ++ti) live += tile_live_rows(p, ti);
    return (double)live / (3.0 * p.tiles_per_img);
}

void dcfp_igemm2_wp_layout(int T, int M, int Ck, int P, long long px, int sn, int sd, int off0, int offstep, int HiWi,
                           int Wo, bool pitched, int sAm, int sAc, DcfpWpEntry* e) {
    const TileCfg c = pick_cfg(M, px, sd);
    const bool d8 = dcfp_igemm2_use_dma8(T, M, P, px, sn, sd, off0, offstep, HiWi, Wo, pitched);
    e->T = T; e->Ck = Ck; e->CkP = round_up(Ck, ck_pad()); e->M = M; e->Mpad = round_up(M, d8 ? 256 : c.bm);
    e->sAm = sAm; e->sAc = sAc; e->perm8 = d8 ? 1 : 0;
}

int dcfp_igemm2_permute_multi(const DcfpWpEntry* table, int n, long long total_blocks, hipStream_t stream) {
    hipLaunchKernelGGL(permute_weights_multi_kernel, dim3((unsigned)total_blocks), dim3(256), 0, stream, table, n);
    DCFP_RETURN_LAUNCH();
}

bool dcfp_igemm2_persist() {
    static const bool persist = [] { const char* e = getenv("DCFP_IGEMM_PERSIST"); return !e || atoi(e) != 0; }();
    return persist;
}

bool dcfp_igemm2_dma_shape(int T, int M, int Ck, int P, long long px, int sn, int sd, int off0, int HiWi, int Wo) {
    static const bool dma = [] { const char* e = getenv("DCFP_IGEMM_DMA"); return !e || atoi(e) != 0; }();
    static const bool dma9 = [] { const char* e = getenv("DCFP_IGEMM_DMA9"); return !e || atoi(e) != 0; }();
    if (!dma || pick_cfg(M, px, sd).id != 4 || sn != 1 || sd != 1 || HiWi != P || Wo % 4 != 0) return false;
    return T == 1 ? off0 == 0 : dma9;
}

int dcfp_igemm2_run(const float* in, long long in_nstride, const float* w, int sAm, int sAc,
                    const float* bias, float* out, long long out_nstride, int N, int M, int Ck, int T,
                    int Hi, int Wi, int Ho, int Wo, int sn, int sd, int off0, int offstep,
                    int accumulate, void* workspace, size_t workspace_bytes, hipStream_t stream,
                    const float* scale, const float* shift, const float* residual, int relu,
                    float* stat_part, int wp_valid, int in_pitch, long long wp_nstride, const float* fan_src,
                    const unsigned long long* fan_mask, const Igemm2Red* red) {
    const long long px = (long long)N * Ho * Wo;
    const TileCfg c = pick_cfg(M, px, sd);
    Igemm2Params p;
    p.stat_part = stat_part;
    p.wp_nstride = wp_nstride;
    p.fan_src = fan_src; p.fan_mask = fan_mask;
    p.red_x = red ? red->x : nullptr; p.red_mask = red ? red->mask : nullptr;
    p.red_mean = red ? red->mean : nullptr; p.red_part = red ? red->part : nullptr;
    if (red && !fan_src) return DCFP_E_BADDESC;
    p.in = in; p.bias = bias; p.out = out;
    p.scale = scale; p.shift = shift; p.residual = residual; p.relu = relu;
    p.in_nstride = in_nstride; p.out_nstride = out_nstride;
    p.N = N; p.M = M; p.Ck = Ck; p.CkP = round_up(Ck, ck_pad()); p.Mpad = round_up(M, c.bm);
    const bool plain = !scale && !relu && !stat_part;
    const bool d8 = plain && !wp_nstride && !fan_src && dcfp_igemm2_use_dma8(T, M, Ho * Wo, px, sn, sd, off0, offstep, Hi * Wi, Wo,
                                                                 in_pitch > 0 && in_pitch != Wi);
    if (d8) p.Mpad = round_up(M, 256);
    p.Hi = Hi; p.Wi = Wi; p.Ho = Ho; p.Wo = Wo; p.P = Ho * Wo;
    p.in_pitch = in_pitch > 0 ? in_pitch : Wi;
    const bool pitched = p.in_pitch != Wi;
    if (pitched) {
        const int reach = off0 < 0 ? -off0 : off0;
        if (T != 9 || p.in_pitch < Wi + reach || off0 + 2 * offstep != -off0 || (p.in_pitch & 3) ||
            (!d8 && (bias || !dcfp_igemm2_dma_shape(T, M, Ck, Ho * Wo, px, sn, sd, off0, Hi * Wi, Wo))) || scale || relu)
            return DCFP_E_UNSUPPORTED;
        if (!d8 && stat_part && dcfp_igemm2_use_dma8(T, M, Ho * Wo, px, sn, sd, off0, offstep, Hi * Wi, Wo, true))
            return DCFP_E_UNSUPPORTED;
    }
    {
        static const int t2d = [] { const char* e = getenv("DCFP_IGEMM_2D"); return e ? atoi(e) : 5; }();
        const bool fits = (t2d == 4 || t2d == 5) && Hi % (256 >> t2d) == 0 && Wi % (1 << t2d) == 0;
        p.tile2d = (fits && !pitched && T == 9 && ((off0 | offstep) & 3) != 0 && Ho == Hi && Wo == Wi) ? t2d : 0;
    }
    p.tapskip = 0;
    {
        static const int nt = [] { const char* e = getenv("DCFP_IGEMM_NT"); return e ? atoi(e) : 0; }();
        p.nt_store = nt;
    }
    p.tiles_per_img = (p.P + (d8 ? 256 : c.bn) - 1) / (d8 ? 256 : c.bn);
    p.Hc = p.Wc = p.tiles_per_phase = p.zfold = 0;
    if (sd > 1) {
        p.Hc = (Ho + sd - 1) / sd; p.Wc = (Wo + sd - 1) / sd;
        p.tiles_per_phase = (p.Hc * p.Wc + c.bn - 1) / c.bn;
        p.tiles_per_img = sd * sd * p.tiles_per_phase;
        if (T == 1) {
            const int ph = ((-off0) % sd + sd) % sd;
            p.zfold = ph * sd + ph + 1;
            p.tiles_per_img = p.tiles_per_phase;
        }
    }
    p.tiles_n_total = p.tiles_per_img * N;
    p.tiles_m = p.Mpad / (d8 ? 256 : c.bm);
    p.sn = sn; p.sd = sd; p.off0 = off0; p.offstep = offstep;
    p.accumulate = accumulate;
    p.vec_store = (p.P % 4 == 0) && (out_nstride % 4 == 0) && dcfp_aligned16(out);
    if (T == 9 && sd == 1 && sn == 1) p.tapskip = pick_tapskip(p, d8 ? 256 : c.bn);
    const size_t need = (size_t)T * p.CkP * p.Mpad * sizeof(float);
    if (!workspace || workspace_bytes < need || !dcfp_aligned16(workspace)) return DCFP_E_WORKSPACE;
    float* wp = static_cast<float*>(workspace);
    p.wp = wp;
    if (!wp_valid) {
        const long long total = (long long)T * p.CkP * p.Mpad;
        long long b = (total + 255) / 256;
        if (b > 2048) b = 2048;
        hipLaunchKernelGGL(permute_weights_kernel, dim3((unsigned)b), dim3(256), 0, stream, w, wp, T,
                           Ck, p.CkP, M, p.Mpad, sAm, sAc, d8 ? 1 : 0);
    }
    if (d8) {
        if (!p.vec_store || wp_nstride || fan_src) return DCFP_E_UNSUPPORTED;
        return dcfp_igemm2n_launch(p, T, stream);
    }
    if (dcfp_igemm2_dma_shape(T, M, Ck, p.P, px, sn, sd, off0, Hi * Wi, Wo) && p.vec_store && !bias && !scale &&
        !relu && !(stat_part && accumulate)) {
        const long long groups = ((long long)p.tiles_n_total + 7) / 8;
        const long long blocks = groups * 8 * p.tiles_m;
        const size_t lds = stat_part ? (size_t)4 * 64 * 33 * 8 : (size_t)2 * BK * 512 * sizeof(float);
        auto launch = [&](auto kern) -> int {
            hipError_t e = hipFuncSetAttribute(reinterpret_cast<const void*>(kern),
                                               hipFuncAttributeMaxDynamicSharedMemorySize, (int)lds);
            if (e != hipSuccess) return (int)e;
            hipLaunchKernelGGL(kern, dim3((unsigned)blocks), dim3(256), lds, stream, p);
            DCFP_RETURN_LAUNCH();
        };
        if (T == 1) {
            if (fan_src && (M % 256 != 0 || p.P % 256 != 0 || !dcfp_igemm2_persist())) return DCFP_E_UNSUPPORTED;
            if (dcfp_igemm2_persist()) return dcfp_igemm2p_launch(p, stream);
            if (wp_nstride) return DCFP_E_UNSUPPORTED;
            return accumulate ? launch(igemm2_dma_kernel<1, false, true>) : launch(igemm2_dma_kernel<1, false, false>);
        }
        if (((off0 | offstep) & 3) == 0 || pitched)
            return accumulate ? launch(igemm2_dma_kernel<9, false, true>) : launch(igemm2_dma_kernel<9, false, false>);
        return accumulate ? launch(igemm2_dma_kernel<9, true, true>) : launch(igemm2_dma_kernel<9, true, false>);
    }
    if (wp_nstride || fan_src) return DCFP_E_UNSUPPORTED;
    return T == 1 ? launch_taps<1>(p, c.id, stream) : launch_taps<9>(p, c.id, stream);
}

int dcfp_igemm2_ck_pad() { return ck_pad(); }
```

### dcfp_amd/csrc/conv_winograd.hip

```cpp
#include "igemm2_common.h"

int dcfp_igemm2_run(const float* in, long long in_nstride, const float* w, int sAm, int sAc,
                    const float* bias, float* out, long long out_nstride, int N, int M, int Ck, int T,
                    int Hi, int Wi, int Ho, int Wo, int sn, int sd, int off0, int offstep,
                    int accumulate, void* workspace, size_t workspace_bytes, hipStream_t stream,
                    const float* scale, const float* shift, const float* residual, int relu, float* stat_part,
                    int wp_valid, int in_pitch, long long wp_nstride, const float* fan_src = nullptr,
                    const unsigned long long* fan_mask = nullptr, const Igemm2Red* red = nullptr);
bool dcfp_igemm2_dma_shape(int T, int M, int Ck, int P, long long px, int sn, int sd, int off0, int HiWi, int Wo);
bool dcfp_igemm2_use_dma8(int T, int M, int P, long long px, int sn, int sd, int off0, int offstep, int HiWi,
                          int Wo, bool pitched);
bool dcfp_igemm2_persist();
int dcfp_igemm2_ck_pad();
bool dcfp_wino_fused_ok(int N, int H, int W, int d, int M, int Ck, long long in_nstride, int pitch);
size_t dcfp_wino_fused_workspace_bytes(int N, int H, int W, int d, int M, int Ck);
int dcfp_wino_fused_run(const float* in, long long in_nstride, int in_pitch, const float* w, int sAm, int sAc, int flip,
                        float* out, long long out_nstride, int N, int M, int Ck, int H, int W, int d, int accumulate,
                        void* workspace, size_t workspace_bytes, hipStream_t stream, float* xform_out, float* stat_part,
                        const float* scale, const float* shift, const float* residual, int relu, int wp_valid);

namespace {

inline long long align64(long long v) { return (v + 63) / 64 * 64; }

struct WinoPlan {
    int TH, TW;
    long long T;
    long long T16;
    int CkP, Mpad;
    long long u_floats, v_floats, m_floats;
};

WinoPlan wino_plan(int N, int H, int W, int d, int M, int Ck) {
    WinoPlan pl;
    pl.TH = d * ((H + 2 * d - 1) / (2 * d));
    pl.TW = d * ((W + 2 * d - 1) / (2 * d));
    pl.TW = (pl.TW + 3) / 4 * 4;
    pl.T = (long long)N * pl.TH * pl.TW;
    pl.T16 = (pl.T + 15) / 16 * 16;
    pl.CkP = (Ck + dcfp_igemm2_ck_pad() - 1) / dcfp_igemm2_ck_pad() * dcfp_igemm2_ck_pad();
    pl.Mpad = (M + 255) / 256 * 256;
    pl.u_floats = align64(16LL * pl.CkP * pl.Mpad);
    pl.v_floats = align64(16LL * Ck * pl.T16);
    pl.m_floats = align64(16LL * M * pl.T16);
    return pl;
}

__global__ void __launch_bounds__(256) wino_filter_kernel(const float* __restrict__ w, int sAm, int sAc, int flip,
                                                          int M, int Ck, int CkP, int Mpad, float* __restrict__ U) {
    const long long plane = (long long)CkP * Mpad;
    for (long long idx = (long long)blockIdx.x * 256 + threadIdx.x; idx < plane; idx += (long long)gridDim.x * 256) {
        const int c = (int)(idx / Mpad), m = (int)(idx - (long long)c * Mpad);
        float g[9];
        if (m < M && c < Ck) {
            const float* src = w + (long long)m * sAm + (long long)c * sAc;
#pragma unroll
            for (int t = 0; t < 9; ++t) g[t] = src[flip ? 8 - t : t];
        } else {
#pragma unroll
            for (int t = 0; t < 9; ++t) g[t] = 0.f;
        }
        float r[4][3];
#pragma unroll
        for (int k = 0; k < 3; ++k) {
            const float g0 = g[k], g1 = g[3 + k], g2 = g[6 + k];
            r[0][k] = g0;
            r[1][k] = 0.5f * ((g0 + g2) + g1);
            r[2][k] = 0.5f * ((g0 + g2) - g1);
            r[3][k] = g2;
        }
#pragma unroll
        for (int i = 0; i < 4; ++i) {
            const float a = r[i][0], b = r[i][1], cc = r[i][2];
            U[(4 * i + 0) * plane + idx] = a;
            U[(4 * i + 1) * plane + idx] = 0.5f * ((a + cc) + b);
            U[(4 * i + 2) * plane + idx] = 0.5f * ((a + cc) - b);
            U[(4 * i + 3) * plane + idx] = cc;
        }
    }
}

template <int VEC>
struct VecT;
template <>
struct VecT<1> { typedef float type; };
template <>
struct VecT<2> { typedef float type __attribute__((ext_vector_type(2))); };
template <>
struct VecT<4> { typedef float type __attribute__((ext_vector_type(4))); };

template <int VEC>
__device__ __forceinline__ void vload(const float* p, float (&v)[VEC]) {
    if constexpr (VEC == 1) v[0] = *p;
    else {
        const typename VecT<VEC>::type t = *reinterpret_cast<const typename VecT<VEC>::type*>(p);
#pragma unroll
        for (int i = 0; i < VEC; ++i) v[i] = t[i];
    }
}
template <int VEC>
__device__ __forceinline__ void vstore(float* p, const float (&v)[VEC]) {
    if constexpr (VEC == 1) *p = v[0];
    else {
        typename VecT<VEC>::type t;
#pragma unroll
        for (int i = 0; i < VEC; ++i) t[i] = v[i];
        *reinterpret_cast<typename VecT<VEC>::type*>(p) = t;
    }
}

template <int VEC>
__global__ void __launch_bounds__(256) wino_input_kernel(const float* __restrict__ x, long long x_nstride, int pitch,
                                                         int N, int C, int H, int W, int d, int TH, int TW,
                                                         float* __restrict__ V, long long rowlen) {
    const int tpi = TH * TW;
    const long long tg = ((long long)blockIdx.x * 256 + threadIdx.x) * VEC;
    if (tg >= rowlen) return;
    const int c = blockIdx.z;
    const int n = (int)(tg / tpi), t = (int)(tg - (long long)n * tpi);
    const long long plane = (long long)C * rowlen;
    float* dst = V + (long long)c * rowlen + tg;
    float q[4][4][VEC];
    if (n >= N) {
        float z[VEC];
#pragma unroll
        for (int v = 0; v < VEC; ++v) z[v] = 0.f;
#pragma unroll
        for (int k = 0; k < 16; ++k) vstore<VEC>(dst + k * plane, z);
        return;
    }
    const int trow = t / TW, tcol = t - trow * TW;
    const int h0 = trow + d * (trow / d) - d, w0 = tcol + d * (tcol / d) - d;
    const float* src = x + (long long)n * x_nstride + (long long)c * H * pitch;
    float p[4][4][VEC];
#pragma unroll
    for (int r = 0; r < 4; ++r) {
        const int h = h0 + r * d;
        const bool hok = (unsigned)h < (unsigned)H;
#pragma unroll
        for (int s = 0; s < 4; ++s) {
            const int ww = w0 + s * d;
            if (hok && ww >= 0 && ww + VEC <= W) vload<VEC>(src + (long long)h * pitch + ww, p[r][s]);
            else {
#pragma unroll
                for (int v = 0; v < VEC; ++v)
                    p[r][s][v] = (hok && (unsigned)(ww + v) < (unsigned)W) ? src[(long long)h * pitch + ww + v] : 0.f;
            }
        }
    }
#pragma unroll
    for (int s = 0; s < 4; ++s)
#pragma unroll
        for (int v = 0; v < VEC; ++v) {
            q[0][s][v] = p[0][s][v] - p[2][s][v];
            q[1][s][v] = p[1][s][v] + p[2][s][v];
            q[2][s][v] = p[2][s][v] - p[1][s][v];
            q[3][s][v] = p[1][s][v] - p[3][s][v];
        }
#pragma unroll
    for (int r = 0; r < 4; ++r) {
        float o[4][VEC];
#pragma unroll
        for (int v = 0; v < VEC; ++v) {
            o[0][v] = q[r][0][v] - q[r][2][v];
            o[1][v] = q[r][1][v] + q[r][2][v];
            o[2][v] = q[r][2][v] - q[r][1][v];
            o[3][v] = q[r][1][v] - q[r][3][v];
        }
#pragma unroll
        for (int s = 0; s < 4; ++s) vstore<VEC>(dst + (4 * r + s) * plane, o[s]);
    }
}
// ... 370 lines not shown
```

### dcfp_amd/csrc/conv_winograd2.hip

```cpp
#include "wino_patch.h"
#include <stdlib.h>

namespace {

constexpr int FBK = 8;
constexpr int FSTAGE = 16 * FBK * 64;

struct WinoFusedParams {
    const float* in;
    const float* in_base;
    unsigned in_bytes;
    int lead;
    long long in_nstride;
    int pitch;
    const float* ug;
    float* out;
    long long out_nstride;
    float* xform_out;
    float* stat_part;
    const float* scale;
    const float* shift;
    const float* residual;
    int relu;
    int N, M, Ck, H, W, d, TH, TW;
    long long T, T16;
    int mblocks, tblocks, nk;
    int accumulate;
    int ragged_c;
    int vec_epi;
    unsigned out_bytes;
};

template <int DM, bool SIDE, bool RAGGED>
__global__ void __launch_bounds__(256, 1) wino_fused_kernel(const WinoFusedParams p) {
    constexpr int NV = PatchCfg<DM>::NV;
    extern __shared__ __attribute__((aligned(16))) float smem[];
    const int tid = threadIdx.x, lane = tid & 63, wid = tid >> 6, wm = wid >> 1, wn = wid & 1;
    const int l31 = lane & 31, lhi = lane >> 5;
    const int wid_s = __builtin_amdgcn_readfirstlane(wid);
    const int xcd = blockIdx.x & 7, jb = blockIdx.x >> 3;
    const int mb = jb % p.mblocks, tb = (jb / p.mblocks) * 8 + xcd;
    if (tb >= p.tblocks) return;
    const long long t0 = (long long)tb * 64;
    const int nk = p.nk, d = p.d, H = p.H, W = p.W, TW = p.TW, tpi = p.TH * p.TW, pitch = p.pitch;

    const unsigned lds0 = (unsigned)(size_t)(lds_ptr)smem;
    const u32x4 a_desc = make_desc(p.ug, 0x7ffffffcu);
    const unsigned lane16 = lane * 16u;

    const int ch = 2 * wid + lhi;
    const long long tp = t0 + 2 * l31;
    unsigned voff[NV];
    {
        const bool tvalid = tp < p.T;
        const long long tq = tvalid ? tp : 0;
        const int n = (int)(tq / tpi), tt = (int)(tq - (long long)n * tpi);
        const int trow = tt / TW, tcol = tt - trow * TW;
        const int h0 = trow + d * (trow / d) - d, w0 = tcol + d * (tcol / d) - d;
        const long long base = (long long)n * p.in_nstride + (long long)lhi * H * pitch + p.lead;
#pragma unroll
        for (int r = 0; r < 4; ++r) {
            const int h = h0 + r * d;
            const bool rok = tvalid && (unsigned)h < (unsigned)H;
            const long long row = base + (long long)h * pitch;
            if constexpr (DM == 1 || DM == 2) {
                voff[2 * r] = (rok && w0 < W) ? (unsigned)((row + w0) * 4) : kOob;
                voff[2 * r + 1] = (rok && w0 + 4 < W) ? (unsigned)((row + w0 + 4) * 4) : kOob;
            } else {
#pragma unroll
                for (int s = 0; s < 4; ++s) {
                    const int ww = w0 + s * d;
                    voff[4 * r + s] = (rok && (unsigned)ww < (unsigned)W) ? (unsigned)((row + ww) * 4) : kOob;
                }
            }
        }
    }
    const __amdgpu_buffer_rsrc_t in_rsrc = __builtin_amdgcn_make_buffer_rsrc(const_cast<float*>(p.in_base), 0,
                                                                             p.in_bytes, 0x00020000);
    const unsigned chan_bytes = (unsigned)(H * pitch) * 4u;
    float R[2][4][8], q[4][8];
    auto load_step = [&](int kt, auto b_) {
        constexpr int b = decltype(b_)::value;
        const unsigned soff = __builtin_amdgcn_readfirstlane((unsigned)(kt * FBK + 2 * wid_s) * chan_bytes);
        if constexpr (RAGGED) {
            unsigned vm[NV];
            const bool cok = kt * FBK + ch < p.Ck;
#pragma unroll
            for (int i = 0; i < NV; ++i) vm[i] = cok ? voff[i] : kOob;
            load_patches<DM>(in_rsrc, vm, soff, R[b]);
        } else {
            load_patches<DM>(in_rsrc, voff, soff, R[b]);
        }
    };
    auto issue_a = [&](int kt, int buf) {
        const unsigned abase = (unsigned)((kt * p.mblocks + mb) * FSTAGE) * 4u;
        static_for<0, 8>([&](auto q_) {
            constexpr int qq = decltype(q_)::value;
            const unsigned piece = (unsigned)(wid_s * 8 + qq);
            const unsigned la = __builtin_amdgcn_readfirstlane(lds0 + (unsigned)(buf * 2 * FSTAGE) * 4u + piece * 1024u);
            const unsigned a_s = __builtin_amdgcn_readfirstlane(abase + piece * 1024u);
            const unsigned av = lane16;
            const u32x4 ad = a_desc;
            asm volatile("s_mov_b32 m0, %0\n\ts_nop 0\n\tbuffer_load_dwordx4 %1, %2, %3 offen lds"
                         :: "s"(la), "v"(av), "s"(ad), "s"(a_s) : "memory", "m0");
        });
    };
    auto retire = [&]() {
        asm volatile("s_waitcnt vmcnt(0) lgkmcnt(0)" ::: "memory");
        __builtin_amdgcn_s_barrier();
    };
    auto retire_keep_loads = [&](bool stored) {
        if (SIDE && stored) {
            if constexpr (NV == 8) asm volatile("s_waitcnt vmcnt(24) lgkmcnt(0)" ::: "memory");
            else asm volatile("s_waitcnt vmcnt(32) lgkmcnt(0)" ::: "memory");
        } else {
            if constexpr (NV == 8) asm volatile("s_waitcnt vmcnt(8) lgkmcnt(0)" ::: "memory");
            else asm volatile("s_waitcnt vmcnt(16) lgkmcnt(0)" ::: "memory");
        }
        __builtin_amdgcn_s_barrier();
    };
    const long long vplane = (long long)p.Ck * p.T16;
    const unsigned vs_lane = (SIDE && tp < p.T16) ? (unsigned)(((long long)lhi * p.T16 + tp) * 4) : kOob;
    auto side_on = [&](int kt) -> bool { return SIDE && kt % p.mblocks == mb; };
    auto side_off = [&](int kt) -> unsigned {
        bool on = true;
        if constexpr (RAGGED) on = kt * FBK + ch < p.Ck;
        return on ? vs_lane : kOob;
    };
    auto side_store = [&](auto xi_, f32x2 o, int kt, unsigned vs) {
        constexpr int XI = decltype(xi_)::value;
        const __amdgpu_buffer_rsrc_t v_rsrc = __builtin_amdgcn_make_buffer_rsrc(p.xform_out + XI * vplane, 0,
                                                                                (unsigned)(vplane * 4), 0x00020000);
        const unsigned soff = __builtin_amdgcn_readfirstlane((unsigned)((long long)(kt * FBK + 2 * wid_s) * p.T16 * 4));
        __builtin_amdgcn_raw_buffer_store_b64(__builtin_bit_cast(u32x2, o), v_rsrc, vs, soff, 0);
    };
    auto produce = [&](auto xi_, int buf) -> f32x2 {
        constexpr int XI = decltype(xi_)::value;
        const f32x2 o = col_transform<DM, XI>(q);
        float* bs = smem + buf * 2 * FSTAGE + FSTAGE + (XI * FBK + ch) * 64 + 2 * l31;
        *reinterpret_cast<f32x2*>(bs) = o;
        return o;
    };

    f32x16 acc[16];
#pragma unroll
    for (int i = 0; i < 16; ++i)
#pragma unroll
        for (int r = 0; r < 16; ++r) acc[i][r] = 0.f;

    load_step(0, std::integral_constant<int, 0>{});
    row_transform<DM>(R[0], q);
    __builtin_amdgcn_sched_barrier(0);
    issue_a(0, 0);
    {
        const unsigned vs = side_off(0);
        const bool st = side_on(0);
        static_for<0, 16>([&](auto xi_) {
            const f32x2 o = produce(xi_, 0);
            if constexpr (SIDE) {
                if (st) side_store(xi_, o, 0, vs);
            }
        });
    }
    load_step(1, std::integral_constant<int, 1>{});
    __builtin_amdgcn_sched_barrier(0);
    load_step(nk > 2 ? 2 : 1, std::integral_constant<int, 0>{});
    retire();

    const int a_lane = wm * 256 + lane * 4;
    const int b_lane = lhi * 64 + wn * 32 + l31;
    f32x4 af[2] = {{0.f, 0.f, 0.f, 0.f}, {0.f, 0.f, 0.f, 0.f}};
    float bf[2][4] = {{0.f, 0.f, 0.f, 0.f}, {0.f, 0.f, 0.f, 0.f}};
    auto step = [&](auto prod_, auto par_, int kt) {
        constexpr bool PROD = decltype(prod_)::value;
        constexpr int cur = decltype(par_)::value, rb = cur ^ 1;
        unsigned vs = kOob;
        bool st = false;
        if constexpr (PROD) { vs = side_off(kt + 1); st = side_on(kt + 1); }
        const float* As = smem + cur * 2 * FSTAGE + a_lane;
        const float* Bs = smem + cur * 2 * FSTAGE + FSTAGE + b_lane;
        const int ktl = kt + 3 < nk ? kt + 3 : nk - 1;
        const unsigned l_soff = __builtin_amdgcn_readfirstlane((unsigned)(ktl * FBK + 2 * wid_s) * chan_bytes);
        unsigned vm[NV];
        if constexpr (PROD) {
// ... 39 lines not shown
            if constexpr (PROD) {
                float* bs = smem + (cur ^ 1) * 2 * FSTAGE + FSTAGE + (g * FBK + ch) * 64 + 2 * l31;
                *reinterpret_cast<f32x2*>(bs) = o;
                if constexpr (SIDE) {
                    if constexpr (g < 8) okeep[g] = o;
                    else if (st) {
                        side_store(std::integral_constant<int, g - 8>{}, okeep[g - 8], kt + 1, vs);
                        side_store(g_, o, kt + 1, vs);
                    }
                }
            }
            __builtin_amdgcn_sched_barrier(0);
            acc[pg] = __builtin_amdgcn_mfma_f32_32x32x2f32(af[fb ^ 1][2], bf[fb ^ 1][2], acc[pg], 0, 0, 0);
            __builtin_amdgcn_sched_barrier(0);
            if constexpr (PROD && g >= 8) {
                constexpr int per = NV / 8;
                static_for<0, per>([&](auto j_) { load_one<DM, (g - 8) * per + decltype(j_)::value>(in_rsrc, vm, l_soff, R[rb]); });
            }
            acc[pg] = __builtin_amdgcn_mfma_f32_32x32x2f32(af[fb ^ 1][3], bf[fb ^ 1][3], acc[pg], 0, 0, 0);
            __builtin_amdgcn_sched_barrier(0);
        });
    };

    constexpr std::integral_constant<int, 0> even{};
    constexpr std::integral_constant<int, 1> odd{};
    int kt = 0;
    for (; kt + 3 < nk; kt += 2) {
        step(std::true_type{}, even, kt);
        retire_keep_loads(side_on(kt + 1));
        step(std::true_type{}, odd, kt + 1);
        retire_keep_loads(side_on(kt + 2));
    }
    step(std::true_type{}, even, nk - 2);
    retire();
    step(std::false_type{}, odd, nk - 1);
#pragma unroll
    for (int kk = 0; kk < 4; ++kk)
        acc[15] = __builtin_amdgcn_mfma_f32_32x32x2f32(af[1][kk], bf[1][kk], acc[15], 0, 0, 0);

    const long long te = t0 + wn * 32 + l31;
    const bool tv = te < p.T;
    const long long tq = tv ? te : 0;
    const int n = (int)(tq / tpi), tt = (int)(tq - (long long)n * tpi);
    const int trow = tt / TW, tcol = tt - trow * TW;
    const int ho = trow + d * (trow / d), wo = tcol + d * (tcol / d);
    const bool okr0 = tv && ho < H, okr1 = tv && ho + d < H;
    const bool okc0 = wo < W, okc1 = wo + d < W;
    const long long HW = (long long)H * W;
    const int m_lane = mb * 64 + wm * 32 + 4 * lhi;
    const int acc_out = p.accumulate;
    float* const sp0 = p.stat_part;
    const long long slot = (long long)tb * 2 + wn;
    auto out_transform = [&](int r, float (&o)[2][2]) {
        float u[2][4];
#pragma unroll
        for (int s = 0; s < 4; ++s) {
            u[0][s] = (acc[0 + s][r] + acc[4 + s][r]) + acc[8 + s][r];
            u[1][s] = (acc[4 + s][r] - acc[8 + s][r]) - acc[12 + s][r];
        }
#pragma unroll
        for (int rr = 0; rr < 2; ++rr) {
            o[rr][0] = (u[rr][0] + u[rr][1]) + u[rr][2];
            o[rr][1] = (u[rr][1] - u[rr][2]) - u[rr][3];
        }
    };
    auto red32 = [&](float v) -> float {
        auto dpp = [](float x, auto ctrl_) {
            constexpr int ctrl = decltype(ctrl_)::value;
            return __builtin_bit_cast(float, __builtin_amdgcn_update_dpp(0, __builtin_bit_cast(int, x), ctrl, 0xF, 0xF, true));
        };
        v += dpp(v, std::integral_constant<int, 0xB1>{});
        v += dpp(v, std::integral_constant<int, 0x4E>{});
        v += dpp(v, std::integral_constant<int, 0x141>{});
        v += dpp(v, std::integral_constant<int, 0x140>{});
        v += __builtin_bit_cast(float, __builtin_amdgcn_update_dpp(0, __builtin_bit_cast(int, v), 0x142, 0xA, 0xF, false));
        const float lo = __builtin_bit_cast(float, __builtin_amdgcn_readlane(__builtin_bit_cast(int, v), 31));
        const float hi = __builtin_bit_cast(float, __builtin_amdgcn_readlane(__builtin_bit_cast(int, v), 63));
        return lhi ? hi : lo;
    };
    auto stats = [&](int m, const float (&o)[2][2]) {
        const float sum = red32((o[0][0] + o[0][1]) + (o[1][0] + o[1][1]));
        const float mean = sum * (1.0f / 128.0f);
        const float d0 = o[0][0] - mean, d1 = o[0][1] - mean, d2 = o[1][0] - mean, d3 = o[1][1] - mean;
        const float m2 = red32((d0 * d0 + d1 * d1) + (d2 * d2 + d3 * d3));
        if (l31 == 0 && m < p.M && t0 + wn * 32 < p.T) {
            float* sp = sp0 + (slot * p.M + m) * 2;
            sp[0] = mean; sp[1] = m2;
        }
    };
    if (p.vec_epi) {
        auto xor1 = [](float v) { return __builtin_bit_cast(float, __builtin_amdgcn_mov_dpp(__builtin_bit_cast(int, v), 0xB1, 0xF, 0xF, true)); };
        auto xor2 = [](float v) { return __builtin_bit_cast(float, __builtin_amdgcn_mov_dpp(__builtin_bit_cast(int, v), 0x4E, 0xF, 0xF, true)); };
        const bool odd = l31 & 1, hi2 = l31 & 2;
        int row, col;
        bool ok;
        if constexpr (DM == 4) {
            const int i = l31 & 3;
            row = ho + (i >> 1) * d;
            col = wo - i + (i & 1) * d;
            ok = tv && row < H && col < W;
        } else if constexpr (DM == 2) {
            row = ho + (odd ? d : 0);
            col = wo - (odd ? 1 : 0);
            ok = tv && row < H && col < W;
        } else {
            row = ho + (odd ? 1 : 0);
            col = wo - (odd ? 2 : 0);
            ok = tv && row < H && col < W;
        }
        const unsigned evoff = ok ? (unsigned)(((long long)n * p.out_nstride + (long long)m_lane * HW + (long long)row * W + col) * 4) : kOob;
        const __amdgpu_buffer_rsrc_t o_rsrc = __builtin_amdgcn_make_buffer_rsrc(p.out, 0, p.out_bytes, 0x00020000);
        const unsigned HW4 = (unsigned)HW * 4u;
        static_for<0, 16>([&](auto r_) {
            constexpr int r = decltype(r_)::value;
            constexpr int mr = (r & 3) + 8 * (r >> 2);
            float o[2][2];
            out_transform(r, o);
            if (sp0) stats(m_lane + mr, o);
            f32x4 v;
            if constexpr (DM == 4) {
                const float x0 = odd ? o[0][0] : o[0][1], x1 = odd ? o[1][0] : o[1][1];
                const float y0 = xor1(x0), y1 = xor1(x1);
                const float b0 = odd ? y0 : o[0][0], b1 = odd ? o[0][1] : y0, b2 = odd ? y1 : o[1][0], b3 = odd ? o[1][1] : y1;
                const float z0 = hi2 ? b0 : b2, z1 = hi2 ? b1 : b3;
                const float w0 = xor2(z0), w1 = xor2(z1);
                v[0] = hi2 ? w0 : b0; v[1] = hi2 ? w1 : b1; v[2] = hi2 ? b2 : w0; v[3] = hi2 ? b3 : w1;
            } else {
                const float s0 = odd ? o[0][0] : o[1][0], s1 = odd ? o[0][1] : o[1][1];
                const float r0 = xor1(s0), r1 = xor1(s1);
                if constexpr (DM == 2) {
                    v[0] = odd ? r0 : o[0][0]; v[1] = odd ? o[1][0] : r0; v[2] = odd ? r1 : o[0][1]; v[3] = odd ? o[1][1] : r1;
                } else {
                    v[0] = odd ? r0 : o[0][0]; v[1] = odd ? r1 : o[0][1]; v[2] = odd ? o[1][0] : r0; v[3] = odd ? o[1][1] : r1;
                }
            }
            const unsigned vo = (m_lane + mr < p.M) ? evoff : kOob;
            const unsigned so = __builtin_amdgcn_readfirstlane((unsigned)mr * HW4);
            if (p.scale) {
                const int mm = m_lane + mr < p.M ? m_lane + mr : p.M - 1;
                const float sc = p.scale[mm], sf = p.shift[mm];
#pragma unroll
                for (int e = 0; e < 4; ++e) v[e] = fmaf(v[e], sc, sf);
                if (p.residual) {
                    const __amdgpu_buffer_rsrc_t r_rsrc = __builtin_amdgcn_make_buffer_rsrc(const_cast<float*>(p.residual), 0,
                                                                                            p.out_bytes, 0x00020000);
                    v += __builtin_bit_cast(f32x4, __builtin_amdgcn_raw_buffer_load_b128(r_rsrc, vo, so, 0));
                }
                if (p.relu) {
#pragma unroll
                    for (int e = 0; e < 4; ++e) v[e] = v[e] > 0.f ? v[e] : 0.f;
                }
            }
            if (acc_out) v += __builtin_bit_cast(f32x4, __builtin_amdgcn_raw_buffer_load_b128(o_rsrc, vo, so, 0));
            __builtin_amdgcn_raw_buffer_store_b128(__builtin_bit_cast(u32x4, v), o_rsrc, vo, so, 0);
        });
        return;
    }
    float* obase = p.out + (long long)n * p.out_nstride + (long long)ho * W + wo;
    const long long dW = (long long)d * W;
#pragma unroll
    for (int r = 0; r < 16; ++r) {
        const int m = m_lane + (r & 3) + 8 * (r >> 2);
        float o[2][2];
        out_transform(r, o);
        if (m < p.M && p.scale) {
            const float sc = p.scale[m], sf = p.shift[m];
            const float* rs = p.residual ? p.residual + (obase - p.out) + (long long)m * HW : nullptr;
            const long long offs[2][2] = {{0, d}, {dW, dW + d}};
            const bool oks[2][2] = {{okr0 && okc0, okr0 && okc1}, {okr1 && okc0, okr1 && okc1}};
#pragma unroll
            for (int rr = 0; rr < 2; ++rr)
#pragma unroll
                for (int cc = 0; cc < 2; ++cc) {
                    float t = fmaf(o[rr][cc], sc, sf);
                    if (rs && oks[rr][cc]) t += rs[offs[rr][cc]];
                    o[rr][cc] = p.relu ? (t > 0.f ? t : 0.f) : t;
                }
        }
        if (m < p.M) {
            float* e = obase + (long long)m * HW;
            if (acc_out) {
                if (okr0 && okc0) e[0] += o[0][0];
                if (okr0 && okc1) e[d] += o[0][1];
                if (okr1 && okc0) e[dW] += o[1][0];
                if (okr1 && okc1) e[dW + d] += o[1][1];
            } else {
                if (okr0 && okc0) e[0] = o[0][0];
                if (okr0 && okc1) e[d] = o[0][1];
                if (okr1 && okc0) e[dW] = o[1][0];
                if (okr1 && okc1) e[dW + d] = o[1][1];
            }
        }
        if (sp0) stats(m, o);
    }
}

__global__ void __launch_bounds__(256) wino_filter2_kernel(const float* __restrict__ w, int sAm, int sAc, int flip, int M,
                                                           int Ck, int CkP, int Mpad, float* __restrict__ Ug) {
    const long long total = (long long)CkP * Mpad;
    for (long long idx = (long long)blockIdx.x * 256 + threadIdx.x; idx < total; idx += (long long)gridDim.x * 256)
        wino_filter2_pair(w, sAm, sAc, flip, M, Ck, Mpad, idx, Ug);
}

struct FusedPlan {
    int TH, TW, mblocks, tblocks, nk, CkP, Mpad;
    long long T, T16, ug_floats;
};
FusedPlan fused_plan(int N, int H, int W, int d, int M, int Ck) {
    FusedPlan pl;
    pl.TH = d * ((H + 2 * d - 1) / (2 * d));
    pl.TW = d * ((W + 2 * d - 1) / (2 * d));
    pl.TW = (pl.TW + 3) / 4 * 4;
    pl.T = (long long)N * pl.TH * pl.TW;
    pl.T16 = (pl.T + 15) / 16 * 16;
    pl.CkP = (Ck + 15) / 16 * 16;
    pl.Mpad = (M + 63) / 64 * 64;
    pl.mblocks = pl.Mpad / 64;
    pl.tblocks = (int)((pl.T + 63) / 64);
    pl.nk = pl.CkP / 8;
    pl.ug_floats = ((long long)16 * pl.CkP * pl.Mpad + 63) / 64 * 64;
    return pl;
}

}

bool dcfp_wino_fused_enabled() {
    static const int v = [] { const char* e = getenv("DCFP_WINO_FUSED"); return e ? atoi(e) : 1; }();
    return v != 0;
}

static int fused_mode(int N, int H, int W, int d, int Ck, long long in_nstride, int pitch) {
    if (pitch <= 0) pitch = W;
    const long long span = (long long)(N - 1) * in_nstride + (long long)((Ck + 15) / 16 * 16) * H * pitch + 64;
    if (span * 4 >= 0x7fffff00LL) return -1;
    if (d == 1 && pitch >= W + 4) return 1;
    if (d == 2 && pitch >= W + 4) return 2;
    if (d >= 4 && d % 2 == 0 && W % 2 == 0) return 4;
    return -1;
}

bool dcfp_wino_fused_ok(int N, int H, int W, int d, int M, int Ck, long long in_nstride, int pitch) {
    if (!dcfp_wino_fused_enabled()) return false;
    if (M < 48 || Ck < 48) return false;
    const FusedPlan pl = fused_plan(N, H, W, d, M, Ck);
    if (pl.T16 >= (1LL << 30) || (long long)pl.tblocks * pl.mblocks + 8 * pl.mblocks >= (1LL << 31)) return false;
    if ((long long)pl.CkP * pl.Mpad * 16 * 4 >= 0x7fffff00LL) return false;
    return fused_mode(N, H, W, d, Ck, in_nstride, pitch) >= 0;
}

void dcfp_wino_fused_pads(int N, int H, int W, int d, int M, int Ck, int* CkP, int* Mpad) {
    const FusedPlan pl = fused_plan(N, H, W, d, M, Ck);
    *CkP = pl.CkP; *Mpad = pl.Mpad;
}

size_t dcfp_wino_fused_workspace_bytes(int N, int H, int W, int d, int M, int Ck) {
    return (size_t)fused_plan(N, H, W, d, M, Ck).ug_floats * sizeof(float);
}

int dcfp_wino_fused_run(const float* in, long long in_nstride, int in_pitch, const float* w, int sAm, int sAc, int flip,
                        float* out, long long out_nstride, int N, int M, int Ck, int H, int W, int d, int accumulate,
                        void* workspace, size_t workspace_bytes, hipStream_t stream, float* xform_out, float* stat_part,
                        const float* scale, const float* shift, const float* residual, int relu, int wp_valid) {
    const FusedPlan pl = fused_plan(N, H, W, d, M, Ck);
    if (!workspace || !dcfp_aligned16(workspace) || workspace_bytes < (size_t)pl.ug_floats * sizeof(float))
        return DCFP_E_WORKSPACE;
    const int pitch = in_pitch > 0 ? in_pitch : W;
    const int mode = fused_mode(N, H, W, d, Ck, in_nstride, pitch);
    if (mode < 0) return DCFP_E_UNSUPPORTED;
    float* Ug = static_cast<float*>(workspace);
    if (!wp_valid) {
        long long b = ((long long)pl.CkP * pl.Mpad + 255) / 256;
        if (b > 4096) b = 4096;
        hipLaunchKernelGGL(wino_filter2_kernel, dim3((unsigned)b), dim3(256), 0, stream, w, sAm, sAc, flip, M, Ck, pl.CkP,
                           pl.Mpad, Ug);
    }
    WinoFusedParams p;
    p.in = in;
    p.lead = (mode == 1 || mode == 2) ? 4 : 0;
    p.in_base = in - p.lead;
    p.in_bytes = (unsigned)(((long long)(N - 1) * in_nstride + (long long)Ck * H * pitch + p.lead) * 4);
    p.in_nstride = in_nstride;
    p.pitch = pitch;
    p.ug = Ug;
    p.out = out;
    p.out_nstride = out_nstride;
    p.xform_out = xform_out;
    p.stat_part = stat_part;
    p.scale = scale; p.shift = shift; p.residual = residual; p.relu = relu;
    p.N = N; p.M = M; p.Ck = Ck; p.H = H; p.W = W; p.d = d; p.TH = pl.TH; p.TW = pl.TW;
    p.T = pl.T; p.T16 = pl.T16;
    p.mblocks = pl.mblocks; p.tblocks = pl.tblocks; p.nk = pl.nk;
    p.accumulate = accumulate;
    p.ragged_c = (Ck % 16) != 0;
    {
        const long long ospan = ((long long)(N - 1) * out_nstride + (long long)M * H * W) * 4;
        p.vec_epi = W % 4 == 0 && out_nstride % 4 == 0 && dcfp_aligned16(out) && ospan < 0x7fffff00LL &&
                    (mode != 4 || d % 4 == 0);
        p.out_bytes = p.vec_epi ? (unsigned)ospan : 0u;
        static const int no_vec = [] { const char* e = getenv("DCFP_WF_SCALAR_EPI"); return e ? atoi(e) : 0; }();
        if (no_vec) p.vec_epi = 0;
    }
    const long long grid = (long long)((pl.tblocks + 7) / 8) * 8 * pl.mblocks;
    const size_t lds = (size_t)4 * FSTAGE * sizeof(float);
    auto launch = [&](auto kern) -> int {
        hipError_t e = hipFuncSetAttribute(reinterpret_cast<const void*>(kern), hipFuncAttributeMaxDynamicSharedMemorySize,
                                           (int)lds);
        if (e != hipSuccess) return (int)e;
        hipLaunchKernelGGL(kern, dim3((unsigned)grid), dim3(256), lds, stream, p);
        DCFP_RETURN_LAUNCH();
    };
    if (xform_out && (long long)Ck * pl.T16 * 4 >= 0x7fffff00LL) return DCFP_E_UNSUPPORTED;
    const bool ragged = (Ck % 16) != 0;
#define DCFP_WF(DM_) (xform_out ? (ragged ? launch(wino_fused_kernel<DM_, true, true>) : launch(wino_fused_kernel<DM_, true, false>)) \
                                : (ragged ? launch(wino_fused_kernel<DM_, false, true>) : launch(wino_fused_kernel<DM_, false, false>)))
    switch (mode) {
        case 1: return DCFP_WF(1);
        case 2: return DCFP_WF(2);
        case 4: return DCFP_WF(4);
        default: return DCFP_E_UNSUPPORTED;
    }
#undef DCFP_WF
}
```

### dcfp_amd/csrc/conv_winograd3.hip

```cpp
#include "wino_patch.h"
#include <stdlib.h>

namespace {

constexpr int GBK = 8;
constexpr int GKH = 144;
constexpr int GHALF = 2 * GKH;
constexpr int GCOMP = 2 * GHALF;
constexpr int GSTAGE = 16 * GCOMP;
constexpr unsigned kSat = 0xffffffffu;

struct WinoWgParams {
    const float* x_base;
    unsigned x_bytes;
    const float* dy_base;
    unsigned dy_bytes;
    const unsigned* table;
    unsigned table_bytes;
    float* out;
    int M, C, mblocks, cblocks, nblk;
    unsigned x_chan_bytes, dy_chan_bytes;
    int kchunk;
    long long T16;
    int d;
};

__global__ void __launch_bounds__(256) wino_wg_table_kernel(unsigned* __restrict__ table, long long npairs, long long T, int N,
                                                            int H, int W, int d, int TH, int TW, long long x_nstride,
                                                            int x_pitch, int lead, long long dy_nstride, int dy_pitch, int dm) {
    const long long pi = (long long)blockIdx.x * 256 + threadIdx.x;
    if (pi >= npairs) return;
    unsigned e[8] = {kOob, kOob, kOob, kOob, kOob, kOob, 0u, 0u};
    const long long t = 2 * pi;
    if (t < T) {
        const int tpi = TH * TW;
        const int n = (int)(t / tpi), tt = (int)(t - (long long)n * tpi);
        const int trow = tt / TW, tcol = tt - trow * TW;
        const int ho = trow + d * (trow / d), wo = tcol + d * (tcol / d);
        if (ho < H && wo < W) {
            const int h0 = ho - d, w0 = wo - d;
            for (int r = 0; r < 4; ++r) {
                const int h = h0 + r * d;
                if (h >= 0 && h < H)
                    e[r] = dm == 4 ? (unsigned)(((long long)n * x_nstride + (long long)h * x_pitch) * 4)
                                   : (unsigned)(((long long)n * x_nstride + (long long)h * x_pitch + w0 + lead) * 4);
            }
            for (int r = 0; r < 2; ++r) {
                const int h = ho + r * d;
                if (h < H)
                    e[4 + r] = dm == 4 ? (unsigned)(((long long)n * dy_nstride + (long long)h * dy_pitch) * 4)
                                       : (unsigned)(((long long)n * dy_nstride + (long long)h * dy_pitch + wo) * 4);
            }
            if (dm == 4) {
                unsigned m = 0;
                for (int s = 0; s < 4; ++s)
                    if (w0 + s * d >= 0 && w0 + s * d < W) m |= 1u << s;
                for (int s = 0; s < 2; ++s)
                    if (wo + s * d < W) m |= 16u << s;
                e[6] = m;
                e[7] = (unsigned)(w0 * 4);
            }
        }
    }
    u32x4* dst = reinterpret_cast<u32x4*>(table + pi * 8);
    dst[0] = u32x4{e[0], e[1], e[2], e[3]};
    dst[1] = u32x4{e[4], e[5], e[6], e[7]};
}

__global__ void __launch_bounds__(256) wino_dw_reduce_kernel(const float* __restrict__ slabs, int splits, long long mc,
                                                             float* __restrict__ dw) {
    const long long i = (long long)blockIdx.x * 256 + threadIdx.x;
    if (i >= mc) return;
    float u[16];
#pragma unroll
    for (int k = 0; k < 16; ++k) u[k] = slabs[k * mc + i];
    int s = 1;
    for (; s + 4 <= splits; s += 4) {
        float v[4][16];
#pragma unroll
        for (int q = 0; q < 4; ++q) {
            const float* sl = slabs + (long long)(s + q) * 16 * mc + i;
#pragma unroll
            for (int k = 0; k < 16; ++k) v[q][k] = sl[k * mc];
        }
#pragma unroll
        for (int q = 0; q < 4; ++q)
#pragma unroll
            for (int k = 0; k < 16; ++k) u[k] += v[q][k];
    }
    for (; s < splits; ++s) {
        const float* sl = slabs + (long long)s * 16 * mc + i;
#pragma unroll
        for (int k = 0; k < 16; ++k) u[k] += sl[k * mc];
    }
    float t[3][4];
#pragma unroll
    for (int s = 0; s < 4; ++s) {
        const float u0 = u[0 + s], u1 = u[4 + s], u2 = u[8 + s], u3 = u[12 + s];
        t[0][s] = u0 + 0.5f * (u1 + u2);
        t[1][s] = 0.5f * (u1 - u2);
        t[2][s] = 0.5f * (u1 + u2) + u3;
    }
    float* o = dw + i * 9;
#pragma unroll
    for (int r = 0; r < 3; ++r) {
        o[3 * r + 0] = t[r][0] + 0.5f * (t[r][1] + t[r][2]);
        o[3 * r + 1] = 0.5f * (t[r][1] - t[r][2]);
        o[3 * r + 2] = 0.5f * (t[r][1] + t[r][2]) + t[r][3];
    }
}

__device__ __forceinline__ unsigned sat_add(unsigned a, unsigned b) {
    unsigned r;
    asm("v_add_u32_e64 %0, %1, %2 clamp" : "=v"(r) : "v"(a), "v"(b));
    return r;
}

template <int DM> __device__ __forceinline__ constexpr int dcolA(int s) { return DM == 1 ? s : 2 * s; }
template <int DM> __device__ __forceinline__ constexpr int dcolB(int s) { return DM == 1 ? 2 + s : 2 * s + 1; }
template <int DM> struct DyCfg { static constexpr int NY = DM == 4 ? 4 : 2; };

template <int DM, int I>
__device__ __forceinline__ void load_dy_one(const __amdgpu_buffer_rsrc_t rsrc, const unsigned (&voff)[DyCfg<DM>::NY],
                                            float (&D)[2][4]) {
    if constexpr (DM == 4) {
        constexpr int r = I >> 1, s = I & 1;
        const f32x2 a = __builtin_bit_cast(f32x2, __builtin_amdgcn_raw_buffer_load_b64(rsrc, voff[I], 0, 0));
        D[r][2 * s] = a[0]; D[r][2 * s + 1] = a[1];
    } else {
        const f32x4 a = __builtin_bit_cast(f32x4, __builtin_amdgcn_raw_buffer_load_b128(rsrc, voff[I], 0, 0));
        D[I][0] = a[0]; D[I][1] = a[1]; D[I][2] = a[2]; D[I][3] = a[3];
    }
}

template <int DM, int XI>
__device__ __forceinline__ f32x2 dy_component(const float (&U)[4][4]) {
    constexpr int i = XI >> 2, j = XI & 3;
    const float a0 = U[i][dcolA<DM>(0)], a1 = U[i][dcolA<DM>(1)], b0 = U[i][dcolB<DM>(0)], b1 = U[i][dcolB<DM>(1)];
    f32x2 o;
    if constexpr (j == 0) { o[0] = a0; o[1] = b0; }
    if constexpr (j == 1) { o[0] = a0 + a1; o[1] = b0 + b1; }
    if constexpr (j == 2) { o[0] = a0 - a1; o[1] = b0 - b1; }
    if constexpr (j == 3) { o[0] = a1; o[1] = b1; }
    return o;
}

template <int DM, bool RAGGED>
__global__ void __launch_bounds__(256, 1) wino_wgrad_fused_kernel(const WinoWgParams p) {
    constexpr int NX = PatchCfg<DM>::NV, NY = DyCfg<DM>::NY, NT = 2 + NX + NY;
    extern __shared__ __attribute__((aligned(16))) float smem[];
    const int tid = threadIdx.x, lane = tid & 63, wid = tid >> 6, wm = wid >> 1, wn = wid & 1;
    const int l31 = lane & 31, lhi = lane >> 5;
    const int per = (p.nblk + 7) >> 3;
    const int xcd = blockIdx.x & 7, jb = blockIdx.x >> 3;
// ... 86 lines not shown
            if constexpr (g == 0) { U[0][c] = Dd[0][c]; U[3][c] = Dd[1][c]; }
            if constexpr (g == 1) { U[1][c] = Dd[0][c] + Dd[1][c]; asm volatile("" : "+v"(U[1][c])); }
            if constexpr (g == 2) { U[2][c] = Dd[0][c] - Dd[1][c]; asm volatile("" : "+v"(U[2][c])); }
        }
    };
    auto retire = [&]() {
        __builtin_amdgcn_s_waitcnt(0xC07F);
        __builtin_amdgcn_s_barrier();
    };

    f32x16 acc[16];
#pragma unroll
    for (int i = 0; i < 16; ++i)
#pragma unroll
        for (int r = 0; r < 16; ++r) acc[i][r] = 0.f;

    constexpr std::integral_constant<int, 0> even{};
    constexpr std::integral_constant<int, 1> odd{};
    load_entry(0); make_offsets(); load_all(even);
    load_entry(1); make_offsets(); load_all(odd);
    row_transform<DM>(R[0], q);
    static_for<0, 4>([&](auto g_) { dy_rows(g_, D[0]); });
    __builtin_amdgcn_sched_barrier(0);
    static_for<0, 16>([&](auto xi_) { produce_y(xi_, 0); produce_x(xi_, 0); });
    load_entry(nk > 2 ? 2 : 1); make_offsets(); load_all(even);
    load_entry(nk > 3 ? 3 : nk - 1);
    asm volatile("s_waitcnt vmcnt(0) lgkmcnt(0)" ::: "memory");
    __builtin_amdgcn_s_barrier();

    const int a_lane = wm * GHALF + lhi * GKH + l31 * 4;
    const int b_lane = wn * GHALF + lhi * GKH + l31 * 4;
    f32x4 af[2] = {{0.f, 0.f, 0.f, 0.f}, {0.f, 0.f, 0.f, 0.f}};
    f32x4 bf[2] = {{0.f, 0.f, 0.f, 0.f}, {0.f, 0.f, 0.f, 0.f}};
    auto step = [&](auto prod_, auto par_, int kt) {
        constexpr bool PROD = decltype(prod_)::value;
        constexpr int cur = decltype(par_)::value, rb = cur ^ 1;
        const float* As = smem + cur * 2 * GSTAGE + a_lane;
        const float* Bs = smem + cur * 2 * GSTAGE + GSTAGE + b_lane;
        const int k_entry = kt + 4 < nk ? kt + 4 : nk - 1;
        static_for<0, 16>([&](auto g_) {
            constexpr int g = decltype(g_)::value;
            constexpr int fb = g & 1, pg = (g + 15) & 15;
            af[fb] = *reinterpret_cast<const f32x4*>(As + g * GCOMP);
            bf[fb] = *reinterpret_cast<const f32x4*>(Bs + g * GCOMP);
            f32x2 ox = {0.f, 0.f}, oy = {0.f, 0.f};
            if constexpr (PROD) {
                if constexpr (g < 4) {
                    row_transform_one<DM, g>(R[rb], q);
#pragma unroll
                    for (int c = 0; c < PatchCfg<DM>::NCOL; ++c) asm volatile("" : "+v"(q[g][c]));
                    dy_rows(g_, D[rb]);
                }
                oy = dy_component<DM, g>(U);
                ox = col_transform<DM, g>(q);
                asm volatile("" : "+v"(ox), "+v"(oy));
                if constexpr (g == 7) make_offsets();
            }
            __builtin_amdgcn_sched_barrier(0);
            acc[pg] = __builtin_amdgcn_mfma_f32_32x32x2f32(af[fb ^ 1][0], bf[fb ^ 1][0], acc[pg], 0, 0, 0);
            acc[pg] = __builtin_amdgcn_mfma_f32_32x32x2f32(af[fb ^ 1][1], bf[fb ^ 1][1], acc[pg], 0, 0, 0);
            __builtin_amdgcn_sched_barrier(0);
            if constexpr (PROD) {
                *reinterpret_cast<f32x2*>(smem + rb * 2 * GSTAGE + g * GCOMP + pw) = oy;
                *reinterpret_cast<f32x2*>(smem + rb * 2 * GSTAGE + GSTAGE + g * GCOMP + pw) = ox;
            }
            __builtin_amdgcn_sched_barrier(0);
            acc[pg] = __builtin_amdgcn_mfma_f32_32x32x2f32(af[fb ^ 1][2], bf[fb ^ 1][2], acc[pg], 0, 0, 0);
            __builtin_amdgcn_sched_barrier(0);
            if constexpr (PROD && g >= 8) {
                constexpr int lo = (g - 8) * NT / 8, hi = (g - 7) * NT / 8;
                static_for<lo, hi>([&](auto i_) { vmem_op(i_, std::integral_constant<int, rb>{}, k_entry); });
            }
            acc[pg] = __builtin_amdgcn_mfma_f32_32x32x2f32(af[fb ^ 1][3], bf[fb ^ 1][3], acc[pg], 0, 0, 0);
            __builtin_amdgcn_sched_barrier(0);
        });
    };

    int kt = 0;
    for (; kt + 3 < nk; kt += 2) {
        step(std::true_type{}, even, kt);
        retire();
        step(std::true_type{}, odd, kt + 1);
        retire();
    }
    step(std::true_type{}, even, nk - 2);
    retire();
    step(std::false_type{}, odd, nk - 1);
#pragma unroll
    for (int kk = 0; kk < 4; ++kk)
        acc[15] = __builtin_amdgcn_mfma_f32_32x32x2f32(af[1][kk], bf[1][kk], acc[15], 0, 0, 0);

    const long long mc = (long long)p.M * p.C;
    const __amdgpu_buffer_rsrc_t o_rsrc = __builtin_amdgcn_make_buffer_rsrc(p.out + (long long)split * 16 * mc, 0,
                                                                            (unsigned)(16 * mc * 4), 0x00020000);
    const int m0 = mb * 64 + wm * 32 + 4 * lhi, c0 = cb * 64 + wn * 32 + l31;
    const unsigned ov = (!RAGGED || c0 < p.C) ? (unsigned)(((long long)m0 * p.C + c0) * 4) : kOob;
    const unsigned C4 = (unsigned)p.C * 4u, mc4 = (unsigned)(mc * 4);
    static_for<0, 16>([&](auto xi_) {
        constexpr int XI = decltype(xi_)::value;
        constexpr bool neg = ((XI >> 2) == 3) != ((XI & 3) == 3);
        static_for<0, 16>([&](auto r_) {
            constexpr int r = decltype(r_)::value, mr = (r & 3) + 8 * (r >> 2);
            const unsigned so = __builtin_amdgcn_readfirstlane((unsigned)XI * mc4 + (unsigned)mr * C4);
            const unsigned vo = (!RAGGED || m0 + mr < p.M) ? ov : kOob;
            const float v = neg ? -acc[XI][r] : acc[XI][r];
            __builtin_amdgcn_raw_buffer_store_b32(__builtin_bit_cast(unsigned, v), o_rsrc, vo, so, 0);
        });
    });
}

struct WgPlan {
    int TH, TW, mblocks, cblocks, splits, kchunk, mode, lead;
    long long T, T16, table_floats, slab_floats;
};

int wg_mode(int N, int H, int W, int d, int M, int C, long long x_nstride, int x_pitch, long long dy_nstride, int dy_pitch) {
    const long long xspan = ((long long)(N - 1) * x_nstride + (long long)((C + 63) / 64 * 64) * H * x_pitch + 64) * 4;
    const long long yspan = ((long long)(N - 1) * dy_nstride + (long long)((M + 63) / 64 * 64) * H * dy_pitch + 64) * 4;
    if (xspan >= 0x7fffff00LL || yspan >= 0x7fffff00LL) return -1;
    if ((d == 1 || d == 2) && x_pitch >= W + 4 && W % 4 == 0) return d;
    if (d >= 4 && d % 2 == 0 && W % 2 == 0) return 4;
    return -1;
}

WgPlan wg_plan(int N, int H, int W, int d, int M, int C) {
    WgPlan pl;
    pl.TH = d * ((H + 2 * d - 1) / (2 * d));
    pl.TW = d * ((W + 2 * d - 1) / (2 * d));
    pl.TW = (pl.TW + 3) / 4 * 4;
    pl.T = (long long)N * pl.TH * pl.TW;
    pl.T16 = (pl.T + 15) / 16 * 16;
    pl.mblocks = (M + 63) / 64;
    pl.cblocks = (C + 63) / 64;
    const long long tiles = (long long)pl.mblocks * pl.cblocks, slots = dcfp_num_cus();
    long long max_splits = pl.T16 / (32 * GBK);
    if (max_splits < 1) max_splits = 1;
    long long splits = 1;
    double best = -1.0;
    for (long long sp = 1; sp <= max_splits && tiles * sp <= 2 * slots; ++sp) {
        const long long blocks = tiles * sp, rounds = (blocks + slots - 1) / slots;
        const double eff = (double)blocks / (double)(rounds * slots);
        if (eff > best + 0.02) { best = eff; splits = sp; }
    }
    long long kchunk = (pl.T16 + splits - 1) / splits;
    kchunk = (kchunk + 15) / 16 * 16;
    splits = (pl.T16 + kchunk - 1) / kchunk;
    pl.splits = (int)splits;
    pl.kchunk = (int)kchunk;
    pl.table_floats = (pl.T16 / 2 * 8 + 63) / 64 * 64;
    pl.slab_floats = (long long)pl.splits * 16 * M * C;
    return pl;
}

}

bool dcfp_wino_wgrad_fused_enabled() {
    static const int v = [] { const char* e = getenv("DCFP_WINO_WGRAD_FUSED"); return e ? atoi(e) : 1; }();
    return v != 0;
}

bool dcfp_wino_wgrad_fused_ok(int N, int H, int W, int d, int M, int C, long long x_nstride, int x_pitch,
                              long long dy_nstride, int dy_pitch) {
    if (!dcfp_wino_wgrad_fused_enabled()) return false;
    if (M < 48 || C < 48) return false;
    if (x_pitch <= 0) x_pitch = W;
    if (dy_pitch <= 0) dy_pitch = W;
    if (wg_mode(N, H, W, d, M, C, x_nstride, x_pitch, dy_nstride, dy_pitch) < 0) return false;
    const WgPlan pl = wg_plan(N, H, W, d, M, C);
    if (pl.T16 >= (1LL << 30) || pl.T16 / 2 * 32 >= 0x7fffff00LL) return false;
    if (16LL * M * C * 4 >= 0x7fffff00LL) return false;
    return (long long)pl.mblocks * pl.cblocks * pl.splits < (1LL << 28);
}

size_t dcfp_wino_wgrad_fused_workspace_bytes(int N, int H, int W, int d, int M, int C) {
    const WgPlan pl = wg_plan(N, H, W, d, M, C);
    return (size_t)(pl.table_floats + pl.slab_floats) * sizeof(float);
}

int dcfp_wino_wgrad_fused_run(const float* dy, long long dy_nstride, int dy_pitch, const float* x, long long x_nstride,
                              int x_pitch, float* dw, int N, int M, int C, int H, int W, int d, void* workspace,
                              size_t workspace_bytes, hipStream_t stream) {
    if (x_pitch <= 0) x_pitch = W;
    if (dy_pitch <= 0) dy_pitch = W;
    const int mode = wg_mode(N, H, W, d, M, C, x_nstride, x_pitch, dy_nstride, dy_pitch);
    if (mode < 0) return DCFP_E_UNSUPPORTED;
    const WgPlan pl = wg_plan(N, H, W, d, M, C);
    if (!workspace || !dcfp_aligned16(workspace) || workspace_bytes < dcfp_wino_wgrad_fused_workspace_bytes(N, H, W, d, M, C))
        return DCFP_E_WORKSPACE;
    unsigned* table = static_cast<unsigned*>(workspace);
    float* slabs = static_cast<float*>(workspace) + pl.table_floats;
    const int lead = mode == 4 ? 0 : 4;
    const long long npairs = pl.T16 / 2;
    hipLaunchKernelGGL(wino_wg_table_kernel, dim3((unsigned)((npairs + 255) / 256)), dim3(256), 0, stream, table, npairs, pl.T,
                       N, H, W, d, pl.TH, pl.TW, x_nstride, x_pitch, lead, dy_nstride, dy_pitch, mode);
    WinoWgParams p;
    p.x_base = x - lead;
    p.x_bytes = (unsigned)(((long long)(N - 1) * x_nstride + (long long)C * H * x_pitch + lead) * 4);
    p.dy_base = dy;
    p.dy_bytes = (unsigned)(((long long)(N - 1) * dy_nstride + (long long)M * H * dy_pitch) * 4);
    p.table = table;
    p.table_bytes = (unsigned)(npairs * 32);
    p.out = slabs;
    p.M = M; p.C = C; p.mblocks = pl.mblocks; p.cblocks = pl.cblocks;
    p.nblk = pl.mblocks * pl.cblocks * pl.splits;
    p.x_chan_bytes = (unsigned)((long long)H * x_pitch * 4);
    p.dy_chan_bytes = (unsigned)((long long)H * dy_pitch * 4);
    p.kchunk = pl.kchunk;
    p.T16 = pl.T16;
    p.d = d;
    const unsigned grid = (unsigned)(((p.nblk + 7) / 8) * 8);
    const size_t lds = (size_t)4 * GSTAGE * sizeof(float);
    auto launch = [&](auto kern) -> int {
        hipError_t e = hipFuncSetAttribute(reinterpret_cast<const void*>(kern), hipFuncAttributeMaxDynamicSharedMemorySize,
                                           (int)lds);
        if (e != hipSuccess) return (int)e;
        hipLaunchKernelGGL(kern, dim3(grid), dim3(256), lds, stream, p);
        hipError_t e2 = hipGetLastError();
        return e2 == hipSuccess ? DCFP_OK : (int)e2;
    };
    const bool ragged = (M % 64) != 0 || (C % 64) != 0;
    int rc;
#define DCFP_WG(DM_) (ragged ? launch(wino_wgrad_fused_kernel<DM_, true>) : launch(wino_wgrad_fused_kernel<DM_, false>))
    switch (mode) {
        case 1: rc = DCFP_WG(1); break;
        case 2: rc = DCFP_WG(2); break;
        default: rc = DCFP_WG(4); break;
    }
#undef DCFP_WG
    if (rc) return rc;
    const long long mc = (long long)M * C;
    hipLaunchKernelGGL(wino_dw_reduce_kernel, dim3((unsigned)((mc + 255) / 256)), dim3(256), 0, stream, slabs, pl.splits, mc, dw);
    DCFP_RETURN_LAUNCH();
}
```

### dcfp_amd/ops.py

```python
import ctypes as C
import os
import weakref

import torch
import torch.distributed as dist

from . import _lib, arena, syncbn_p2p
from ._lib import ConvDesc, BnRunning, check

_ws_cache = {}
WEIGHT_EPOCH = [0]

_PROFILE = None


def profile_start():
    global _PROFILE
    _PROFILE = []


def profile_stop():
    global _PROFILE
    recs, _PROFILE = _PROFILE, None
    torch.cuda.synchronize()
# ... 153 lines not shown
_WP_TABLE = {"version": 0, "built": -1, "dev": None, "n": 0, "blocks": 0, "entries": []}


def _wp_buffer(w, which, d, nbytes, variant=""):
    key = (which, d.N, d.H, d.W, d.stride, d.pad, d.dil, d.x_pitch, d.dy_pitch, variant)
    tag = (w.data_ptr(), w._version, WEIGHT_EPOCH[0], torch.cuda.current_stream().cuda_stream)
    cache = getattr(w, "_dcfp_wp", None)
    if cache is None:
        cache = {}
        try:
            w._dcfp_wp = cache
            _WP_OWNERS.add(w)
        except Exception:
            return _workspace("conv", nbytes, w.device), 0
    ent = cache.get(key)
    if ent is not None and ent[1].numel() >= nbytes:
        if ent[0] == tag:
            return ent[1], 1
        cache[key] = (tag, ent[1], ent[2])
        return ent[1], 0
    if len(cache) > 8:
        cache.clear()
    buf = torch.empty(max(int(nbytes), 256), dtype=torch.uint8, device=w.device)
    cache[key] = (tag, buf, ConvDesc(*[getattr(d, f[0]) for f in ConvDesc._fields_]))
    _WP_TABLE["version"] += 1
    return buf, 0


def _conv_workspace(w, which, d, variant=""):
    L = _lib.lib()
    nbytes = L.dcfp_conv2d_workspace_bytes(C.byref(d), which)
    if L.dcfp_conv2d_workspace_is_scratch(C.byref(d), which):
        return _workspace("conv_scratch", nbytes, w.device), 0
    return _wp_buffer(w, which, d, nbytes, variant)


def refresh_wp():
    T = _WP_TABLE
    L = _lib.lib()
    stream = torch.cuda.current_stream().cuda_stream
    if T["built"] != T["version"]:
        ents, recs, first = [], [], 0
        for w in list(_WP_OWNERS):
            if not w.is_cuda or not w.is_contiguous():
                continue
            for key, (tag, buf, desc) in list(w._dcfp_wp.items()):
                if key[-1]:
                    continue
                e = _lib.WpEntry()
                if L.dcfp_conv2d_wp_layout(C.byref(desc), key[0], C.byref(e)) != 0:
                    continue
                e.w, e.wp, e.first_block = w.data_ptr(), buf.data_ptr(), first
                first += e.n_blocks
                recs.append(e); ents.append((weakref.ref(w), key))
        T["entries"], T["n"], T["blocks"] = ents, len(recs), first
        if recs:
            arr = (_lib.WpEntry * len(recs))(*recs)
            host = torch.frombuffer(bytearray(bytes(arr)), dtype=torch.uint8)
            T["dev"] = host.to(torch.device("cuda", torch.cuda.current_device()))
        T["built"] = T["version"]
        T["ptrs"] = [e.w for e in recs]
    if not T["n"]:
        return
    live = []
    for (wr, key), ptr in zip(T["entries"], T["ptrs"]):
        w = wr()
        if w is None or w.data_ptr() != ptr or key not in w._dcfp_wp:
            T["version"] += 1
            return
        live.append((w, key))
    check(L.dcfp_conv2d_permute_weights_multi_f32(C.c_void_p(T["dev"].data_ptr()), T["n"], T["blocks"],
                                                  C.c_void_p(stream)), "permute_weights_multi")
    for w, key in live:
        _, buf, desc = w._dcfp_wp[key]
        w._dcfp_wp[key] = ((w.data_ptr(), w._version, WEIGHT_EPOCH[0], stream), buf, desc)


def _bn_run(running_mean, running_var, momentum, nbt):
    upd = running_mean is not None and momentum is not None
    if not upd and nbt is None:
        return None
    r = BnRunning()
    r.running_mean = running_mean.data_ptr() if upd else None
    r.running_var = running_var.data_ptr() if upd else None
    r.num_batches_tracked = nbt.data_ptr() if nbt is not None else None
    r.momentum = float(momentum) if upd else 0.0
    return r


def _rp(run):
    return C.byref(run) if run is not None else None


FANIN_RED_USED = [0]
FANIN_BN_SUMS = os.environ.get("DCFP_FANIN_BN_SUMS", "1") not in ("0",)
FANIN_BN_SUMS_ALWAYS = os.environ.get("DCFP_FANIN_BN_SUMS", "1") == "2"
KEEP_XFORM = os.environ.get("DCFP_KEEP_XFORM", "1") not in ("0",)


def conv2d_fwd(x, w, bias=None, stride=1, pad=0, dil=1, want_stats=False, bn_run=None, out=None, keep=None):
    _require(x, "x"); _require(w, "weight")
    xp = _pitch_of(x)
    if not xp:
        x = x.contiguous()
    w = w if w.is_contiguous() else w.contiguous()
    d = _desc(x.shape, w.shape, stride, pad, dil, xp, 0)
    yns = 0
    if out is None:
        y = torch.empty((d.N, d.Cout, d.Hout, d.Wout), dtype=torch.float32, device=x.device)
    else:
        y = out
        st = y.stride()
        if tuple(y.shape) != (d.N, d.Cout, d.Hout, d.Wout) or st[3] != 1 or st[2] != d.Wout or st[1] != d.Hout * d.Wout:
            raise RuntimeError("conv2d_fwd: out must be [N,Cout,Ho,Wo] with dense images (a channel slice is fine)")
        yns = st[0]
    if bias is not None:
        _require(bias, "bias"); bias = bias.contiguous()
    L = _lib.lib()
    variant = "bias" if (bias is not None and d.KH == 3 and conv_kernel_name(d, _lib.CONV_FWD).startswith("winograd")) else ""
    ws, valid = _conv_workspace(w, _lib.CONV_FWD, d, variant)
    if keep is not None and KEEP_XFORM and bias is None:
        xb = L.dcfp_conv2d_xform_bytes(C.byref(d))
        if xb > 0:
            xf = torch.empty(xb, dtype=torch.uint8, device=x.device)
            slots = L.dcfp_conv2d_fwd_stat_slots(C.byref(d), _p(y), yns) if want_stats else 0
            part = _workspace("bn_stat_partials", slots * d.Cout * 2 * 4, x.device) if slots > 0 else None
            _timed("conv_fwd", d, _conv_flops(d), lambda: check(
                L.dcfp_conv2d_fwd_keep_f32_nchw(C.byref(d), _p(x), _p(w), _p(y), yns, _p(xf), xb, _p(part), _p(ws),
                                                ws.numel(), _stream()), "conv2d_fwd_keep"))
            keep["xform"] = xf
            if part is not None:
                mv = torch.empty((2, d.Cout), dtype=torch.float32, device=x.device)
                check(L.dcfp_bn_stats_from_partials_f32(_p(part), slots, 128, d.Cout, _p(mv[0]), _p(mv[1]),
                                                        _rp(bn_run), _stream()), "bn_stats_from_partials")
                return y, (mv[0], mv[1], bn_run is not None)
            return (y, None) if want_stats else y
    if want_stats and bias is None:
        slots = L.dcfp_conv2d_fwd_stat_slots(C.byref(d), _p(y), yns)
        if slots > 0:
            part = _workspace("bn_stat_partials", slots * d.Cout * 2 * 4, x.device)
            _timed("conv_fwd", d, _conv_flops(d), lambda: check(
                L.dcfp_conv2d_fwd_stats_f32_nchw(C.byref(d), _p(x), _p(w), _p(y), yns, _p(part), _p(ws),
                                                 ws.numel(), valid, _stream()), "conv2d_fwd_stats"))
            mv = torch.empty((2, d.Cout), dtype=torch.float32, device=x.device)
            check(L.dcfp_bn_stats_from_partials_f32(_p(part), slots, 128, d.Cout, _p(mv[0]), _p(mv[1]),
                                                    _rp(bn_run), _stream()), "bn_stats_from_partials")
            return y, (mv[0], mv[1], bn_run is not None)
    _timed("conv_fwd", d, _conv_flops(d), lambda: check(
        L.dcfp_conv2d_fwd_f32_nchw(C.byref(d), _p(x), _p(w), _p(bias), _p(y), yns, _p(ws), ws.numel(), valid,
                                   _stream()), "conv2d_fwd"))
    return (y, None) if want_stats else y


def conv2d_dgrad(dy, w, xshape, stride, pad, dil, out=None, accumulate=False):
    _require(dy, "dy")
    w = w if w.is_contiguous() else w.contiguous()
    dp = _pitch_of(dy)
    d = _desc(xshape, w.shape, stride, pad, dil, 0, dp)
    if dp:
        ns = dy.stride(0)
    else:
        dy, ns = _batch_strided(dy)
    if out is not None:
        if tuple(out.shape) != tuple(xshape) or not out.is_contiguous():
            raise RuntimeError("conv2d_dgrad: out must be a contiguous tensor of the input shape")
        dx = out
    else:
        dx = torch.empty(xshape, dtype=torch.float32, device=dy.device)
        accumulate = False
    L = _lib.lib()
    ws, valid = _conv_workspace(w, _lib.CONV_DGRAD, d)
    _timed("conv_dgrad", d, _conv_flops(d), lambda: check(
        L.dcfp_conv2d_dgrad_f32_nchw(C.byref(d), _p(dy), ns, _p(w), _p(dx), int(bool(accumulate)),
                                     _p(ws), ws.numel(), valid, _stream()), "conv2d_dgrad"))
    return dx


MASKED_FANIN = os.environ.get("DCFP_MASKED_FANIN", "1") not in ("0",)


def conv2d_dgrad_fanin_ok(dyshape, w, xshape):
    d = _desc(xshape, w.shape, 1, 0, 1)
    return MASKED_FANIN and bool(_lib.lib().dcfp_conv2d_dgrad_fanin_supported(C.byref(d)))


def conv2d_dgrad_fanin(dy, w, xshape, fan_src, fan_mask):
    _require(dy, "dy"); _require(fan_src, "fan_src")
    w = w if w.is_contiguous() else w.contiguous()
    d = _desc(xshape, w.shape, 1, 0, 1)
    dy, ns = _batch_strided(dy)
    if tuple(fan_src.shape) != tuple(xshape) or not fan_src.is_contiguous():
        raise RuntimeError("conv2d_dgrad_fanin: fan_src must be a contiguous tensor of the input shape")
    dx = torch.empty(xshape, dtype=torch.float32, device=dy.device)
    ws, valid = _conv_workspace(w, _lib.CONV_DGRAD, d)
    _timed("conv_dgrad", d, _conv_flops(d), lambda: check(
        _lib.lib().dcfp_conv2d_dgrad_fanin_f32_nchw(C.byref(d), _p(dy), ns, _p(w), _p(dx), _p(fan_src), _p(fan_mask),
                                                    _p(ws), ws.numel(), valid, _stream()), "conv2d_dgrad_fanin"))
    return dx


def conv2d_dgrad_fanin_red_slots(w, xshape):
    if not (MASKED_FANIN and FANIN_BN_SUMS):
        return 0
    d = _desc(xshape, w.shape, 1, 0, 1)
    return int(_lib.lib().dcfp_conv2d_dgrad_fanin_red_slots(C.byref(d)))


def conv2d_dgrad_fanin_red(dy, w, xshape, fan_src, fan_mask, red_x, red_mask, red_mean, slots):
    _require(dy, "dy"); _require(fan_src, "fan_src"); _require(red_x, "red_x")
    w = w if w.is_contiguous() else w.contiguous()
    d = _desc(xshape, w.shape, 1, 0, 1)
    dy, ns = _batch_strided(dy)
    if tuple(fan_src.shape) != tuple(xshape) or not fan_src.is_contiguous():
        raise RuntimeError("conv2d_dgrad_fanin_red: fan_src must be a contiguous tensor of the input shape")
    if tuple(red_x.shape) != tuple(xshape) or not red_x.is_contiguous() or red_mean.numel() != xshape[1]:
        raise RuntimeError("conv2d_dgrad_fanin_red: red_x / red_mean must match the input shape")
    dx = torch.empty(xshape, dtype=torch.float32, device=dy.device)
    part = torch.empty((slots, xshape[1], 2), dtype=torch.float32, device=dy.device)
    ws, valid = _conv_workspace(w, _lib.CONV_DGRAD, d)
    _timed("conv_dgrad_red", d, _conv_flops(d), lambda: check(
        _lib.lib().dcfp_conv2d_dgrad_fanin_red_f32_nchw(C.byref(d), _p(dy), ns, _p(w), _p(dx), _p(fan_src), _p(fan_mask),
                                                        _p(red_x), _p(red_mask), _p(red_mean), _p(part), _p(ws),
                                                        ws.numel(), valid, _stream()), "conv2d_dgrad_fanin_red"))
    return dx, part


def bn_bwd_sums_from_partials(part, var, eps, dgamma=None, dbeta=None):
    slots, Cc, _ = part.shape
    s = torch.empty((2, Cc), dtype=torch.float32, device=part.device)
    if dgamma is None:
        dgamma = torch.empty(Cc, dtype=torch.float32, device=part.device)
    _timed("bn_bwd_reduce", None, 8.0 * part.numel() / 2, lambda: check(
        _lib.lib().dcfp_bn_bwd_sums_from_partials_f32(_p(part), slots, Cc, _p(var), float(eps), _p(s[0]), _p(s[1]),
                                                      _p(dgamma), _p(dbeta), _stream()), "bn_bwd_sums_from_partials"))
    return s[0], s[1], dgamma


def conv2d_wgrad(dy, x, wshape, stride, pad, dil, need_bias=False, dw=None, db=None, xform=None):
    _require(dy, "dy"); _require(x, "x")
    xp, dp = _pitch_of(x), _pitch_of(dy)
    if not xp:
        x = x.contiguous()
    d = _desc(x.shape, wshape, stride, pad, dil, xp, dp)
    if dp:
        ns = dy.stride(0)
    else:
        dy, ns = _batch_strided(dy)
    L = _lib.lib()
    nbytes = L.dcfp_conv2d_workspace_bytes(C.byref(d), _lib.CONV_WGRAD)
    ws = _workspace("conv_scratch", nbytes, x.device)
    if dw is None:
        dw = torch.empty(wshape, dtype=torch.float32, device=x.device)
    elif tuple(dw.shape) != tuple(wshape) or not dw.is_contiguous():
        raise RuntimeError("conv2d_wgrad: dw must be a contiguous tensor of the weight shape")
    if need_bias and db is None:
        db = torch.empty((wshape[0],), dtype=torch.float32, device=x.device)
    if xform is not None and not need_bias and L.dcfp_conv2d_xform_bytes(C.byref(d)) == xform.numel():
        _timed("conv_wgrad", d, _conv_flops(d), lambda: check(
            L.dcfp_conv2d_wgrad_kept_f32_nchw(C.byref(d), _p(dy), ns, _p(xform), xform.numel(), _p(dw), _p(ws), ws.numel(),
                                              _stream()), "conv2d_wgrad_kept"))
        return dw, None
    _timed("conv_wgrad", d, _conv_flops(d), lambda: check(
        L.dcfp_conv2d_wgrad_f32_nchw(C.byref(d), _p(dy), ns, _p(x), _p(dw), _p(db) if need_bias else None, _p(ws),
                                     ws.numel(), _stream()), "conv2d_wgrad"))
    return dw, (db if need_bias else None)


def add_into(dst, src):
    check(_lib.lib().dcfp_add_f32(_p(dst), _p(src), _p(dst), dst.numel(), _stream()), "add")


def wgrad_into_param(dy, x, w, bias, stride, pad, dil, keep=None):
    tw, kw = arena.grad_target(w)
    tb, kb = arena.grad_target(bias) if bias is not None else (None, 0)
    xform = keep.pop("xform", None) if keep else None
    conv2d_wgrad(dy, x, tuple(w.shape), stride, pad, dil, need_bias=bias is not None, dw=tw, db=tb, xform=xform)
    dw = arena.grad_commit(w, tw, kw, add_into)
    db = arena.grad_commit(bias, tb, kb, add_into) if bias is not None else None
    return dw, db


class Conv2dFn(torch.autograd.Function):

    @staticmethod
    def forward(ctx, x, w, bias, stride, pad, dil):
        ctx.keep = {} if ctx.needs_input_grad[1] else None
        y = conv2d_fwd(x, w, bias, stride, pad, dil, keep=ctx.keep)
        ctx.save_for_backward(x)
        ctx.params = (w, bias)
        ctx.cfg = (stride, pad, dil)
        return y

    @staticmethod
    def backward(ctx, dy):
        (x,) = ctx.saved_tensors
        w, bias = ctx.params
        stride, pad, dil = ctx.cfg
        dx = dw = db = None
        if ctx.needs_input_grad[0]:
            dx = conv2d_dgrad(dy, w, tuple(x.shape), stride, pad, dil)
        if ctx.needs_input_grad[1] or (bias is not None and ctx.needs_input_grad[2]):
            dw, db = wgrad_into_param(dy, x, w, bias, stride, pad, dil, keep=ctx.keep)
        return dx, dw, db, None, None, None


def conv2d(x, w, bias=None, stride=1, pad=0, dil=1):
    return Conv2dFn.apply(x, w, bias, stride, pad, dil)


def bn_stats(x, run=None):
    _require(x, "x")
    N, Cc, H, W = x.shape
    x, ns = _batch_strided(x)
    L = _lib.lib()
    ws = _workspace("bn", L.dcfp_bn_workspace_bytes(N, Cc, H * W), x.device)
    mean = torch.empty(Cc, dtype=torch.float32, device=x.device)
    var = torch.empty(Cc, dtype=torch.float32, device=x.device)
    _timed("bn_stats", None, 4.0 * x.numel(), lambda: check(
        L.dcfp_bn_stats_f32(_p(x), ns, N, Cc, H * W, _p(mean), _p(var), _rp(run), _p(ws), ws.numel(), _stream()),
        "bn_stats"))
    return mean, var


def bn_apply(x, mean, var, gamma, beta, eps, residual=None, relu=False, out=None):
# ... 421 lines not shown
        ctx.prev_rec = getattr(x, "_dcfp_bn3_rec", None) if FANIN_BN_SUMS else None
        x = x.contiguous()
        has_ds = len(tensors) == 12
        w1, g1, b1, w2, g2, b2, w3, g3, b3 = tensors[:9]
        bnargs = cfg["bn"]
        stride, dil = cfg["stride"], cfg["dil"]

        N_, _, H_, W_ = x.shape
        y1_shape = (N_, w1.shape[0], H_, W_)
        pitch = conv_pitch(y1_shape, tuple(w2.shape), stride, dil, dil)
        y1_out, ctx.pitch_slot = None, None
        if pitch:
            y1_out, ctx.pitch_slot = owner_pitched(cfg.get("owner"), y1_shape, pitch, x.device)
        ctx.pitch = pitch
        c1, y1, st1 = _conv_bn_fwd(x, w1, bnargs[0], g1, b1, out=y1_out)
        ctx.keep2 = {} if ctx.needs_input_grad[5] else None
        c2, y2, st2 = _conv_bn_fwd(y1, w2, bnargs[1], g2, b2, stride, dil, dil, keep=ctx.keep2)
        if has_ds:
            wd, gd, bd = tensors[9:]
            cd, res, std = _conv_bn_fwd(x, wd, bnargs[3], gd, bd, stride, 0, 1, relu=False)
        else:
            cd, res, std = None, x, None
        c3, out, st3 = _conv_bn_fwd(y2, w3, bnargs[2], g3, b3, res=res, want_mask=True)
        ctx.has_ds = has_ds
        ctx.cfg = (stride, dil, [a[2] for a in bnargs], [a[4] for a in bnargs])
        ctx.params = tensors
        flat, ctx.meta = _pack_bn_states((st1, st2, st3, std))
        keep_out = out if len(st3) <= 4 else None
        ctx.save_for_backward(x, c1, y1, c2, y2, c3, keep_out, cd, *flat)
        ctx.rec = None
        fused_bn3 = BN_BWD_FUSED and st3[3] is None and not FANIN_BN_SUMS_ALWAYS
        if FANIN_BN_SUMS and not fused_bn3 and len(st3) > 4 and any(ctx.needs_input_grad):
            ctx.rec = {"c3": c3, "mask": st3[4], "mean": st3[0]}
            out._dcfp_bn3_rec = ctx.rec
        return out

    @staticmethod
    def backward(ctx, dout):
        x, c1, y1, c2, y2, c3, out, cd = ctx.saved_tensors[:8]
        flat = ctx.saved_tensors[8:]
        tensors = ctx.params
        w1, g1, b1, w2, g2, b2, w3, g3, b3 = tensors[:9]
        stride, dil, training, eps = ctx.cfg
        st1, st2, st3, std = (_bn_state(ctx.meta, flat, i) for i in range(4))

        def wg(dy, inp, w, st=1, pd=0, dl=1, keep=None):
            return lambda: wgrad_into_param(dy, inp, w, None, st, pd, dl, keep=keep)[0]

        mask3 = st3[4] if len(st3) > 4 else None
        fanin = (not ctx.has_ds and mask3 is not None and ctx.needs_input_grad[0] and dout.is_contiguous()
                 and tuple(dout.shape) == tuple(x.shape) and conv2d_dgrad_fanin_ok(None, w1, tuple(x.shape)))
        pre, rec = None, getattr(ctx, "rec", None)
        if rec is not None:
            part, ptr, ver = rec.pop("part", None), rec.pop("dx_ptr", None), rec.pop("dx_ver", None)
            if part is not None and dout.data_ptr() == ptr and dout._version == ver and dout.is_contiguous():
                pre = part
                FANIN_RED_USED[0] += 1
            rec.clear()
            ctx.rec = None
        d_c3, dg3, db3, d_res = bn_backward_impl(dout, c3, out, g3, b3, st3, True, training[2], eps[2], not fanin, pre=pre)
        d_y2 = conv2d_dgrad(d_c3, w3, tuple(y2.shape), 1, 0, 1)
        dc2_out = pitched_buffer(tuple(c2.shape), ctx.pitch, "d_c2", c2.device) if ctx.pitch else None
        d_c2, dg2, db2, _, dw3 = bn_backward_impl(d_y2, c2, None, g2, b2, st2, True, training[1], eps[1], False,
                                                  between=wg(d_c3, y2, w3), dx_out=dc2_out)
        d_y1 = conv2d_dgrad(d_c2, w2, tuple(y1.shape), stride, dil, dil)
        d_c1, dg1, db1, _, dw2 = bn_backward_impl(d_y1, c1, None, g1, b1, st1, True, training[0], eps[0], False,
                                                  between=wg(d_c2, y1, w2, stride, dil, dil, keep=ctx.keep2))
        grads = [None, dg1, db1, dw2, dg2, db2, dw3, dg3, db3]
        if ctx.has_ds:
            wd, gd, bd = tensors[9:]
            d_cd, dgd, dbd, _, dw1 = bn_backward_impl(d_res, cd, None, gd, bd, std, False, training[3], eps[3], False,
                                                      between=wg(d_c1, x, w1))
            dwd, _ = wgrad_into_param(d_cd, x, wd, None, stride, 0, 1)
            grads += [dwd, dgd, dbd]
            dx = conv2d_dgrad(d_cd, wd, tuple(x.shape), stride, 0, 1) if ctx.needs_input_grad[0] else None
        else:
            dw1, _ = wgrad_into_param(d_c1, x, w1, None, 1, 0, 1)
            dx = d_res
        grads[0] = dw1
        prev = ctx.prev_rec
        slots = 0
        if fanin and prev is not None and tuple(prev["c3"].shape) == tuple(x.shape):
            slots = conv2d_dgrad_fanin_red_slots(w1, tuple(x.shape))
        if fanin and slots > 0:
            dx, part = conv2d_dgrad_fanin_red(d_c1, w1, tuple(x.shape), dout, mask3, prev["c3"], prev["mask"],
                                              prev["mean"], slots)
            prev["part"], prev["dx_ptr"], prev["dx_ver"] = part, dx.data_ptr(), dx._version
            del part
        elif fanin:
            dx = conv2d_dgrad_fanin(d_c1, w1, tuple(x.shape), dout, mask3)
        elif ctx.needs_input_grad[0]:
            dx = conv2d_dgrad(d_c1, w1, tuple(x.shape), 1, 0, 1, out=dx, accumulate=True)
        else:
            dx = None
        ctx.prev_rec = None
        _release_pitch(ctx)
        return (dx, None) + tuple(grads)


def bottleneck(x, cfg, tensors):
    return BottleneckFn.apply(x, cfg, *tensors)


def batch_norm_act(x, gamma, beta, running_mean, running_var, residual=None, relu=False,
                   training=True, momentum=0.1, eps=1e-5, sync=False, nbt=None, pitch_cfg=None):
    return BatchNormActFn.apply(x, gamma, beta, running_mean, running_var, residual, relu,
                                training, momentum, eps, sync, nbt, pitch_cfg)


class AsppFn(torch.autograd.Function):

    @staticmethod
    def forward(ctx, x, cfg, *tensors):
        x = x.contiguous()
        N, Cin, H, W = x.shape
        widths = [t.shape[0] for t in tensors[0::3]]
        cat = torch.empty((N, sum(widths), H, W), dtype=torch.float32, device=x.device)
        offs = [sum(widths[:k]) for k in range(5)]
        states, cs, keeps = [], [], []
        for k in range(4):
            w, g, b = tensors[3 * k:3 * k + 3]
            pad, dil = cfg["convs"][k]
            kp = {} if ctx.needs_input_grad[2 + 3 * k] else None
            keeps.append(kp)
            c, _, st = _conv_bn_fwd(x, w, cfg["bn"][k], g, b, 1, pad, dil, out=cat[:, offs[k]:offs[k] + widths[k]],
                                    keep=kp)
            cs.append(c); states.append(st)
        w5, g5, b5 = tensors[12:15]
        rm, rv, training, momentum, eps, sync, nbt = cfg["bn"][4]
        pooled = rowsum(x, 1.0 / (H * W))
        c5 = conv2d_fwd(pooled, w5, None, 1, 0, 1)
        y5, st5 = bn_forward_impl(c5, g5, b5, rm, rv, None, True, training, momentum, eps, sync, nbt=nbt)
        broadcast_hw(y5, H, W, out=cat[:, offs[4]:offs[4] + widths[4]])
        states.append(st5)
        ctx.keeps = keeps
        ctx.cfg = (cfg["convs"], [a[2] for a in cfg["bn"]], [a[4] for a in cfg["bn"]], offs, widths)
        ctx.params = tensors
        flat, ctx.meta = _pack_bn_states(states)
        ctx.save_for_backward(x, pooled, c5, *cs, *flat)
        return cat

    @staticmethod
    def backward(ctx, dcat):
        x, pooled, c5 = ctx.saved_tensors[:3]
        cs = ctx.saved_tensors[3:7]
        flat = ctx.saved_tensors[7:]
        tensors = ctx.params
        convs, training, eps, offs, widths = ctx.cfg
        N, Cin, H, W = x.shape
        need_dx = ctx.needs_input_grad[0]
        grads = [None] * 15
        dx = None
        pending = None
        for k in range(4):
            w, g, b = tensors[3 * k:3 * k + 3]
            pad, dil = convs[k]
            dslice = dcat[:, offs[k]:offs[k] + widths[k]]
            res = bn_backward_impl(dslice, cs[k], None, g, b, _bn_state(ctx.meta, flat, k), True, training[k], eps[k], False,
                                   between=pending)
            d_c, grads[3 * k + 1], grads[3 * k + 2] = res[0], res[1], res[2]
            if pending is not None:
                grads[3 * (k - 1)] = res[4]
            if need_dx:
                dx = conv2d_dgrad(d_c, w, tuple(x.shape), 1, pad, dil, out=dx, accumulate=dx is not None)
            pending = (lambda d_c=d_c, w=w, pad=pad, dil=dil, kp=ctx.keeps[k]:
                       wgrad_into_param(d_c, x, w, None, 1, pad, dil, keep=kp)[0])
        w5, g5, b5 = tensors[12:15]
        g_y5 = rowsum(dcat[:, offs[4]:offs[4] + widths[4]], 1.0)
        res = bn_backward_impl(g_y5, c5, None, g5, b5, _bn_state(ctx.meta, flat, 4), True, training[4], eps[4], False, between=pending)
        d_c5, grads[13], grads[14], grads[9] = res[0], res[1], res[2], res[4]
        grads[12], _ = wgrad_into_param(d_c5, pooled, w5, None, 1, 0, 1)
        if need_dx:
            d_pooled = conv2d_dgrad(d_c5, w5, tuple(pooled.shape), 1, 0, 1)
            dx = broadcast_hw(d_pooled, H, W, 1.0 / (H * W), out=dx, accumulate=dx is not None)
        return (dx, None) + tuple(grads)


def aspp_branches(x, cfg, tensors):
    return AsppFn.apply(x, cfg, *tensors)


def _rows(t):
    N, Cc, H, W = t.shape
    st = t.stride()
    if st[3] != 1 or st[2] < W or st[1] != H * st[2] or (st[2] != W and st[2] % 4) or (N > 1 and st[0] < Cc * H * st[2]):
        return None
    return (st[0] if N > 1 else Cc * H * st[2]), (st[2] if st[2] != W else 0)


def _rows_or_copy(t):
    r = _rows(t)
    if r is None:
        t = t.contiguous()
        r = _rows(t)
    return (t,) + r


def resize_bilinear_into(x, out, align_corners):
    _require(x, "x"); _require(out, "out")
    x, xns = _batch_strided(x)
    N, Cc, h, w = x.shape
    H, W = out.shape[2], out.shape[3]
    r = _rows(out)
    if r is None or out.shape[0] != N or out.shape[1] != Cc:
        raise RuntimeError("resize_bilinear_into: out must be [N,C,H,W] with dense rows (a channel slice is fine)")
    _timed("resize_fwd", None, 4.0 * (x.numel() + out.numel()), lambda: check(
        _lib.lib().dcfp_resize_bilinear_into_f32(_p(x), xns, N, Cc, h, w, _p(out), r[0], r[1], H, W,
                                                 int(bool(align_corners)), _stream()), "resize_bilinear_into"))
    return out


def resize_bilinear_adjoint(dy, size, align_corners, out=None, accumulate=False):
    _require(dy, "dy")
    dy, dns, dpitch = _rows_or_copy(dy)
    N, Cc, H, W = dy.shape
    h, w = int(size[0]), int(size[1])
    if out is None:
        dx = torch.empty((N, Cc, h, w), dtype=torch.float32, device=dy.device)
        accumulate = False
    else:
        dx = out
        if tuple(dx.shape) != (N, Cc, h, w) or not dx.is_contiguous():
            raise RuntimeError("resize_bilinear_adjoint: out must be a contiguous [N,C,h,w] tensor")
    _timed("resize_adjoint", None, 4.0 * (dy.numel() + dx.numel()), lambda: check(
        _lib.lib().dcfp_resize_bilinear_adjoint_f32(_p(dy), dns, dpitch, N, Cc, H, W, _p(dx), Cc * h * w, h, w,
                                                    int(bool(align_corners)), int(bool(accumulate)), _stream()),
        "resize_bilinear_adjoint"))
    return dx


class DecoderConcatFn(torch.autograd.Function):

    @staticmethod
    def forward(ctx, x, low, cfg, w1, g1, b1):
        _require(x, "x"); _require(low, "low")
        low = low.contiguous()
        N, Cx, h, w = x.shape
        _, Cl, H, W = low.shape
        C1 = w1.shape[0]
        cat = _concat_buffer(ctx, cfg, (N, Cx + C1, H, W), x.device)
        align = cfg["align"]
        resize_bilinear_into(x, cat[:, :Cx], align)
        ctx.keep = {} if ctx.needs_input_grad[3] else None
        c, _, st = _conv_bn_fwd(low, w1, cfg["bn"], g1, b1, out=cat[:, Cx:], keep=ctx.keep)
        flat, ctx.meta = _pack_bn_states([st])
        ctx.save_for_backward(low, c, *flat)
        ctx.params = (w1, g1, b1)
        ctx.cfg = (cfg["bn"][2], cfg["bn"][4], Cx, (h, w), align)
        return cat

    @staticmethod
    def backward(ctx, dcat):
        low, c = ctx.saved_tensors[:2]
        w1, g1, b1 = ctx.params
        training, eps, Cx, hw, align = ctx.cfg
        state = _bn_state(ctx.meta, ctx.saved_tensors[2:], 0)
        dx = [None]

        def adjoint():
            if ctx.needs_input_grad[0]:
                dx[0] = resize_bilinear_adjoint(dcat[:, :Cx], hw, align)
        res = bn_backward_impl(dcat[:, Cx:], c, None, g1, b1, state, True, training, eps, False, between=adjoint)
        d_c, dg, db = res[0], res[1], res[2]
        dlow = conv2d_dgrad(d_c, w1, tuple(low.shape), 1, 0, 1) if ctx.needs_input_grad[1] else None
        dw = wgrad_into_param(d_c, low, w1, None, 1, 0, 1, keep=ctx.keep)[0] if ctx.needs_input_grad[3] else None
        _release_pitch(ctx)
        return dx[0], dlow, None, dw, dg, db


def decoder_concat(x, low, cfg, w1, g1, b1):
    return DecoderConcatFn.apply(x, low, cfg, w1, g1, b1)


def _int_array(vals):
    vals = [int(v) for v in vals]
    return (C.c_int * len(vals))(*vals)


def _pool_levels(levels):
    levels = [(int(a), int(b)) for a, b in levels]
    if not 1 <= len(levels) <= 4 or any(not (1 <= a <= 8 and 1 <= b <= 8) for a, b in levels):
        raise RuntimeError(f"dcfp_amd: the pyramid pooling kernels take 1 to 4 levels of sizes 1..8, got {levels}")
    return levels


def _level_views(buf, N, widths, levels):
    out, off = [], 0
    for Cc, (a, b) in zip(widths, levels):
        n = N * Cc * a * b
        out.append(buf[off:off + n].view(N, Cc, a, b))
        off += n
    return out


def ppm_pool(x, levels, mean=True, dst=None):
    _require(x, "x")
    levels = _pool_levels(levels)
    x = x.contiguous()
    N, Cc, H, W = x.shape
    buf = torch.empty(sum(N * Cc * a * b for a, b in levels), dtype=torch.float32, device=x.device)
    dns, dpitch = 0, 0
    if dst is not None:
        _require(dst, "dst")
        r = _rows(dst)
        if r is None or tuple(dst.shape) != (N, Cc, H, W):
            raise RuntimeError("ppm_pool: dst must be [N,C,H,W] with dense rows (a channel slice is fine)")
        dns, dpitch = r
    _timed("ppm_pool", None, 4.0 * x.numel() * (2 if dst is not None else 1), lambda: check(
        _lib.lib().dcfp_ppm_pool_f32(_p(x), N, Cc, H, W, len(levels), _int_array(v for hw in levels for v in hw),
                                     _p(buf), int(bool(mean)), _p(dst), dns, dpitch, _stream()), "ppm_pool"))
    return _level_views(buf, N, [Cc] * len(levels), levels)


def ppm_pool_adjoint(dp, levels, shape, g=None):
    levels = _pool_levels(levels)
    N, Cc, H, W = [int(v) for v in shape]
    _require(dp, "dp")
    if dp.numel() != sum(N * Cc * a * b for a, b in levels) or not dp.is_contiguous():
        raise RuntimeError("ppm_pool_adjoint: dp must hold the level-major [N,C,sh,sw] blocks of every level")
    gns, gpitch = 0, 0
    if g is not None:
        _require(g, "g")
        g, gns, gpitch = _rows_or_copy(g)
        if tuple(g.shape) != (N, Cc, H, W):
            raise RuntimeError("ppm_pool_adjoint: g must be [N,C,H,W]")
    dx = torch.empty((N, Cc, H, W), dtype=torch.float32, device=dp.device)
    _timed("ppm_pool_adjoint", None, 4.0 * dx.numel() * (2 if g is not None else 1), lambda: check(
# ... 881 lines not shown
```

### include/dcfp_hip.h

```cpp
#ifndef DCFP_HIP_H
#define DCFP_HIP_H

#include <stddef.h>
#include <stdint.h>

#ifdef __cplusplus
extern "C" {
#endif

#define DCFP_OK 0
#define DCFP_E_BADDESC (-1)
#define DCFP_E_UNSUPPORTED (-2)
#define DCFP_E_WORKSPACE (-3)

typedef void* dcfp_stream_t;

int dcfp_abi_version(void);

typedef struct DcfpConvDesc {
    int32_t N, Cin, H, W;
    int32_t Cout, KH, KW;
    int32_t stride, pad, dil;
    int32_t Hout, Wout;
    int32_t x_pitch, dy_pitch;
} DcfpConvDesc;

enum { DCFP_CONV_FWD = 0, DCFP_CONV_DGRAD = 1, DCFP_CONV_WGRAD = 2 };

size_t dcfp_conv2d_workspace_bytes(const DcfpConvDesc* d, int pass);

#define DCFP_WP_BLOCK_ELEMS 2048
typedef struct DcfpWpEntry {
    const float* w;
    float* wp;
    int64_t first_block;
    int64_t n_blocks;
    int32_t T, Ck, CkP, M, Mpad, sAm, sAc;
    int32_t perm8;
} DcfpWpEntry;
int dcfp_conv2d_wp_layout(const DcfpConvDesc* d, int pass, DcfpWpEntry* entry);
int dcfp_conv2d_permute_weights_multi_f32(const DcfpWpEntry* table, int n_entries, int64_t total_blocks,
                                          dcfp_stream_t stream);

int dcfp_conv2d_pitch_supported(const DcfpConvDesc* d);

int dcfp_conv2d_workspace_is_scratch(const DcfpConvDesc* d, int pass);

size_t dcfp_conv2d_xform_bytes(const DcfpConvDesc* d);
int dcfp_conv2d_fwd_keep_f32_nchw(const DcfpConvDesc* d, const float* x, const float* w, float* y, int64_t y_nstride,
                                  float* xform_out, size_t xform_bytes,
                                  float* stat_partials ,
                                  void* workspace, size_t workspace_bytes, dcfp_stream_t stream);
int dcfp_conv2d_wgrad_kept_f32_nchw(const DcfpConvDesc* d, const float* dy, int64_t dy_nstride, const float* xform,
                                    size_t xform_bytes, float* dw, void* workspace, size_t workspace_bytes,
                                    dcfp_stream_t stream);

int dcfp_conv2d_dgrad_fanin_supported(const DcfpConvDesc* d);
int dcfp_conv2d_dgrad_fanin_f32_nchw(const DcfpConvDesc* d, const float* dy, int64_t dy_nstride, const float* w, float* dx,
                                     const float* fan_src, const void* fan_mask, void* workspace, size_t workspace_bytes,
                                     int wp_valid, dcfp_stream_t stream);
int64_t dcfp_conv2d_dgrad_fanin_red_slots(const DcfpConvDesc* d);
int dcfp_conv2d_dgrad_fanin_red_f32_nchw(const DcfpConvDesc* d, const float* dy, int64_t dy_nstride, const float* w,
                                         float* dx, const float* fan_src, const void* fan_mask, const float* red_x,
                                         const void* red_mask, const float* red_mean, float* red_part, void* workspace,
                                         size_t workspace_bytes, int wp_valid, dcfp_stream_t stream);
int dcfp_bn_bwd_sums_from_partials_f32(const float* partials, int64_t slots, int C, const float* var, float eps,
                                       float* sum_dy, float* sum_dy_xmu, float* dgamma ,
                                       float* dbeta , dcfp_stream_t stream);

int dcfp_conv2d_kernel_name(const DcfpConvDesc* d, int pass, char* buf, int buf_len);

double dcfp_conv2d_executed_fraction(const DcfpConvDesc* d, int pass);

int dcfp_conv2d_fwd_f32_nchw(const DcfpConvDesc* d, const float* x, const float* w,
                             const float* bias, float* y, int64_t y_nstride,
                             void* workspace, size_t workspace_bytes, int wp_valid,
                             dcfp_stream_t stream);
int dcfp_conv2d_fwd_fused_f32_nchw(const DcfpConvDesc* d, const float* x, const float* w,
                                   const float* scale, const float* shift, const float* residual,
                                   int relu, float* y, void* workspace, size_t workspace_bytes,
                                   int wp_valid, dcfp_stream_t stream);
int dcfp_conv2d_dgrad_f32_nchw(const DcfpConvDesc* d, const float* dy, int64_t dy_nstride,
                               const float* w, float* dx, int accumulate,
                               void* workspace, size_t workspace_bytes, int wp_valid,
                               dcfp_stream_t stream);
int dcfp_conv2d_wgrad_f32_nchw(const DcfpConvDesc* d, const float* dy, int64_t dy_nstride,
                               const float* x, float* dw, float* db,
                               void* workspace, size_t workspace_bytes,
                               dcfp_stream_t stream);

typedef struct DcfpBnRunning {
    float* running_mean;
    float* running_var;
    int64_t* num_batches_tracked;
    float momentum;
    int32_t pad_;
} DcfpBnRunning;
size_t dcfp_bn_workspace_bytes(int N, int C, int HW);
int dcfp_bn_stats_f32(const float* x, int64_t x_nstride, int N, int C, int HW,
                      float* mean, float* var, const DcfpBnRunning* run,
                      void* workspace, size_t workspace_bytes, dcfp_stream_t stream);
int dcfp_bn_apply_f32(const float* x, const float* mean, const float* var,
                      const float* gamma, const float* beta, float eps,
                      const float* residual, int relu, float* y, int64_t y_nstride,
                      int N, int C, int HW, int W, int y_pitch, dcfp_stream_t stream);
int dcfp_bn_bwd_reduce_f32(const float* dy, int64_t dy_nstride, const float* x,
                           const float* y, int64_t y_nstride, const float* mean,
                           const float* var, const float* gamma, const float* beta, float eps,
                           int relu, int N, int C, int HW,
                           float* sum_dy, float* sum_dy_xmu, float* dgamma ,
                           float* dbeta ,
                           void* workspace, size_t workspace_bytes, dcfp_stream_t stream);
int64_t dcfp_conv2d_fwd_stat_slots(const DcfpConvDesc* d, const float* y, int64_t y_nstride);
int dcfp_conv2d_fwd_stats_f32_nchw(const DcfpConvDesc* d, const float* x, const float* w, float* y,
                                   int64_t y_nstride, float* stat_partials, void* workspace,
                                   size_t workspace_bytes, int wp_valid, dcfp_stream_t stream);
int dcfp_bn_stats_from_partials_f32(const float* partials, int64_t slots, int slot_count, int C,
                                    float* mean, float* var, const DcfpBnRunning* run , dcfp_stream_t stream);
int dcfp_syncbn_combine_f32(const float* gathered, int world, int C, float* mean, float* var,
                            float* total_count, const DcfpBnRunning* run , dcfp_stream_t stream);
#define DCFP_P2P_HANDLE_BYTES 64
size_t dcfp_syncbn_p2p_mailbox_bytes(int world, int cap_floats);
int dcfp_p2p_alloc(size_t bytes, int kind, void** ptr);
int dcfp_p2p_free(void* ptr);
int dcfp_p2p_export(void* ptr, void* handle64);
int dcfp_p2p_import(const void* handle64, void** ptr);
int dcfp_p2p_unmap(void* ptr);
int dcfp_syncbn_p2p_exchange_f32(void* const* mailboxes, int world, int rank, uint32_t seq, int cap_floats,
                                 const float* local, int n, int mode, float* out, const DcfpBnRunning* run,
                                 uint32_t spin_limit, int32_t* status, dcfp_stream_t stream);
int dcfp_bn_update_running_f32(const float* mean, const float* var, int C, float momentum,
                               float count, const float* count_dev, float* running_mean,
                               float* running_var, dcfp_stream_t stream);
int dcfp_bn_apply_relu_mask_f32(const float* x, const float* mean, const float* var,
                                const float* gamma, const float* beta, float eps,
                                const float* residual, float* y, void* relu_mask,
                                int N, int C, int HW, dcfp_stream_t stream);
int dcfp_bn_bwd_apply_f32(const float* dy, int64_t dy_nstride, const float* x,
                          const float* y, int64_t y_nstride, const float* mean,
                          const float* var, const float* gamma, const float* beta, float eps,
                          const float* sum_dy, const float* sum_dy_xmu, float count,
                          const float* count_dev,
                          int relu, float* dx, float* d_residual,
                          int N, int C, int HW, int W, int dx_pitch ,
                          dcfp_stream_t stream);

size_t dcfp_bn_bwd_fused_sync_bytes(int N, int C, int HW);
int dcfp_bn_bwd_fused_f32(const float* dy, int64_t dy_nstride, const float* x, const float* y,
                          int64_t y_nstride, const float* mean, const float* var, const float* gamma,
                          const float* beta, float eps, float count, int relu, float* dx, float* d_residual,
                          int N, int C, int HW, int W, int dx_pitch, float* sum_dy, float* sum_dy_xmu,
                          float* dgamma, float* dbeta, void* sync, size_t sync_bytes, uint32_t epoch,
                          uint32_t spin_limit, int32_t* status, dcfp_stream_t stream);

int dcfp_maxpool3x3s2_fwd_f32(const float* x, float* y, int32_t* argmax,
                              int N, int C, int H, int W, int Hout, int Wout,
                              dcfp_stream_t stream);
int dcfp_maxpool3x3s2_bwd_f32(const float* dy, const int32_t* argmax, float* dx,
                              int N, int C, int H, int W, int Hout, int Wout,
                              dcfp_stream_t stream);
int dcfp_rowsum_f32(const float* x, int64_t x_nstride, float* y, float scale,
                    int N, int C, int HW, dcfp_stream_t stream);
int dcfp_broadcast_hw_f32(const float* v, float scale, float* y, int64_t y_nstride,
                          int accumulate, int N, int C, int HW, dcfp_stream_t stream);
int dcfp_add_f32(const float* a, const float* b, float* out, int64_t n,
                 dcfp_stream_t stream);
int dcfp_channel_scale_f32(const float* x, const float* mask, float* y,
                           int N, int C, int HW, dcfp_stream_t stream);

int dcfp_upsample_bilinear_fwd_f32(const float* x, float* y, int N, int C,
                                   int h, int w, int H, int W, int align_corners,
                                   dcfp_stream_t stream);
int dcfp_upsample_bilinear_bwd_f32(const float* dy, float* dx, int N, int C,
                                   int h, int w, int H, int W, int align_corners,
                                   dcfp_stream_t stream);
int dcfp_resize_bilinear_into_f32(const float* x, int64_t x_nstride, int N, int C, int h, int w,
                                  float* y, int64_t y_nstride, int y_pitch, int H, int W,
                                  int align_corners, dcfp_stream_t stream);
int dcfp_resize_bilinear_adjoint_f32(const float* dy, int64_t dy_nstride, int dy_pitch, int N, int C, int H, int W,
                                     float* dx, int64_t dx_nstride, int h, int w, int align_corners,
                                     int accumulate, dcfp_stream_t stream);
int dcfp_ppm_pool_f32(const float* x, int N, int C, int H, int W, int nlev, const int* level_hw,
                      float* out, int mean, float* dst, int64_t dst_nstride, int dst_pitch,
                      dcfp_stream_t stream);
int dcfp_ppm_pool_adjoint_f32(const float* dp, int N, int C, int H, int W, int nlev, const int* level_hw,
                              const float* g, int64_t g_nstride, int g_pitch, float* dx, dcfp_stream_t stream);
int dcfp_ppm_resize_adjoint_f32(const float* g, int64_t g_nstride, int g_pitch, int N, int H, int W,
                                int nlev, const int* level_chw, float* dp, int align_corners,
                                dcfp_stream_t stream);
size_t dcfp_upsample_ce_workspace_bytes(int N, int H, int W);
int dcfp_upsample_ce_fwd_f32(const float* logits, const int64_t* labels,
                             const uint8_t* pixel_keep, int ignore_index,
                             int N, int C, int h, int w, int H, int W, int align_corners,
                             float* lse, float* gt_prob, float* out2,
                             void* workspace, size_t workspace_bytes,
                             dcfp_stream_t stream);
int dcfp_upsample_ce_bwd_f32(const float* logits, const int64_t* labels,
                             const uint8_t* pixel_keep, int ignore_index,
                             int N, int C, int h, int w, int H, int W, int align_corners,
                             const float* lse, const float* grad_scale ,
                             float* dlogits, dcfp_stream_t stream);
int dcfp_upsample_ce_bwd_plan(int N, int C, int h, int w, int H, int W, int* variant, int* chunk_width, int* chunks);

int dcfp_ohem_zoom_gt_prob_f32(const float* logits, const int64_t* labels, const float* lse,
                               int N, int C, int h, int w, int H, int W, int align_corners,
                               int H8, int W8, float* pred8, int32_t* lab8,
                               dcfp_stream_t stream);

int dcfp_ohem_threshold_f32(const float* pred8, const int32_t* lab8, int64_t n, int ignore_label,
                            float thresh, int64_t min_kept, float* threshold ,
                            dcfp_stream_t stream);
int dcfp_ohem_keep_mask_u8(const float* gt_prob, const float* threshold , int64_t n,
                           uint8_t* keep, dcfp_stream_t stream);

int dcfp_upsample_margin_f32(const float* logits, int N, int C, int h, int w, int H, int W,
                             int align_corners, float* margin, dcfp_stream_t stream);
int dcfp_maxfilter2d_s1_f32(const float* x, float* y, int planes, int H, int W, int k,
                            dcfp_stream_t stream);
size_t dcfp_upsample_wce_workspace_bytes(int N, int H, int W);
int dcfp_upsample_wce_fwd_f32(const float* logits, const int64_t* labels, const float* pix_weight,
                              int ignore_index, int N, int C, int h, int w, int H, int W,
                              int align_corners, float* lse, float* out_per_image,
                              void* workspace, size_t workspace_bytes, dcfp_stream_t stream);
int dcfp_upsample_wce_bwd_f32(const float* logits, const int64_t* labels, const float* pix_weight,
                              int ignore_index, int N, int C, int h, int w, int H, int W,
                              int align_corners, const float* lse,
                              const float* grad_scale_per_image, float* dlogits,
                              dcfp_stream_t stream);

int dcfp_upsample_argmax_f32(const float* logits, int N, int C, int h, int w, int H, int W,
                             int align_corners, int32_t* pred, dcfp_stream_t stream);
int dcfp_confusion_matrix_i64(const int32_t* pred, const int64_t* gt, int ignore_index,
                              int64_t n_pixels, int C, int64_t* conf ,
                              dcfp_stream_t stream);

typedef struct DcfpVoteMap {
    const float* logits;
    int h, w;
    int hs, ws;
    int flip;
    float weight;
} DcfpVoteMap;
// ... 244 lines not shown
```

Baseline: 12.22 images/s.

## Fuse ASPP pooled broadcast into last dgrad, tile weight permutes, cache wgrad tables

```diff
diff --git a/dcfp_amd/_lib.py b/dcfp_amd/_lib.py
--- a/dcfp_amd/_lib.py
+++ b/dcfp_amd/_lib.py
@@ -118,6 +118,7 @@
     "dcfp_conv2d_workspace_bytes": (_Z, [_D, _I]),
     "dcfp_conv2d_wp_layout": (_I, [_D, _I, C.POINTER(WpEntry)]),
     "dcfp_conv2d_permute_weights_multi_f32": (_I, [_P, _I, _L, _P]),
+    "dcfp_conv2d_permute_weights_one_f32": (_I, [C.POINTER(WpEntry), _P]),
     "dcfp_conv2d_pitch_supported": (_I, [_D]),
     "dcfp_conv2d_kernel_name": (_I, [_D, _I, C.c_char_p, _I]),
     "dcfp_conv2d_executed_fraction": (C.c_double, [_D, _I]),
@@ -133,7 +134,10 @@
     "dcfp_conv2d_fwd_f32_nchw": (_I, [_D, _P, _P, _P, _P, _L, _P, _Z, _I, _P]),
     "dcfp_conv2d_fwd_fused_f32_nchw": (_I, [_D, _P, _P, _P, _P, _P, _I, _P, _P, _Z, _I, _P]),
     "dcfp_conv2d_dgrad_f32_nchw": (_I, [_D, _P, _L, _P, _P, _I, _P, _Z, _I, _P]),
+    "dcfp_conv2d_dgrad_chan_add_supported": (_I, [_D, _L]),
+    "dcfp_conv2d_dgrad_chan_add_f32_nchw": (_I, [_D, _P, _L, _P, _P, _P, _F, _P, _Z, _I, _P]),
     "dcfp_conv2d_wgrad_f32_nchw": (_I, [_D, _P, _L, _P, _P, _P, _P, _Z, _P]),
+    "dcfp_wino_wgrad_table_counters": (_I, [C.POINTER(C.c_int64), C.POINTER(C.c_int64)]),
     "dcfp_bn_workspace_bytes": (_Z, [_I, _I, _I]),
     "dcfp_bn_stats_f32": (_I, [_P, _L, _I, _I, _I, _P, _P, _R, _P, _Z, _P]),
     "dcfp_bn_apply_f32": (_I, [_P, _P, _P, _P, _P, _F, _P, _I, _P, _L, _I, _I, _I, _I, _I, _P]),
diff --git a/dcfp_amd/csrc/conv_igemm.hip b/dcfp_amd/csrc/conv_igemm.hip
--- a/dcfp_amd/csrc/conv_igemm.hip
+++ b/dcfp_amd/csrc/conv_igemm.hip
@@ -63,6 +63,11 @@
 bool dcfp_wino_fused_ok(int N, int H, int W, int d, int M, int Ck, long long in_nstride, int pitch);
 size_t dcfp_wino_fused_workspace_bytes(int N, int H, int W, int d, int M, int Ck);
 void dcfp_wino_fused_pads(int N, int H, int W, int d, int M, int Ck, int* CkP, int* Mpad);
+int dcfp_wino_fused_run(const float* in, long long in_nstride, int in_pitch, const float* w, int sAm, int sAc, int flip,
+                        float* out, long long out_nstride, int N, int M, int Ck, int H, int W, int d, int accumulate,
+                        void* workspace, size_t workspace_bytes, hipStream_t stream, float* xform_out, float* stat_part,
+                        const float* scale, const float* shift, const float* residual, int relu, int wp_valid,
+                        const float* chan_add, float chan_scale);
 size_t dcfp_wino_xform_bytes(int N, int H, int W, int d, int C);
 bool dcfp_wgrad_is_winograd(const DcfpConvDesc* d);
 bool dcfp_wgrad_wants_xform(const DcfpConvDesc* d);
@@ -74,6 +79,9 @@
 bool dcfp_igemm2_use_dma8(int T, int M, int P, long long px, int sn, int sd, int off0, int offstep, int HiWi,
                           int Wo, bool pitched);
 int dcfp_igemm2_permute_multi(const DcfpWpEntry* table, int n, long long total_blocks, hipStream_t stream);
+int dcfp_igemm2_permute_one(const DcfpWpEntry* e, hipStream_t stream);
+int dcfp_wino_filter2_run(const float* w, int sAm, int sAc, int flip, int M, int Ck, int CkP, int Mpad, float* Ug,
+                          hipStream_t stream);
 
 
 size_t dcfp_igemm3_workspace_bytes(int T, int M, int Ck);
@@ -342,6 +350,33 @@
                            nullptr, wp_valid, d->dy_pitch);
 }
 
+static bool dgrad_chan_add_ok(const DcfpConvDesc* d, long long dy_nstride) {
+    if (check_desc(d) != DCFP_OK || dcfp_gemv_shape(d) || !wino_pass(d, DCFP_CONV_DGRAD)) return false;
+    const int sp = d->dy_pitch;
+    const long long ns = dy_nstride ? dy_nstride : (long long)d->Cout * d->Hout * (sp ? sp : d->Wout);
+    return dcfp_wino_fused_ok(d->N, d->H, d->W, d->dil, d->Cin, d->Cout, ns, sp);
+}
+
+extern "C" int dcfp_conv2d_dgrad_chan_add_supported(const DcfpConvDesc* d, int64_t dy_nstride) {
+    return dgrad_chan_add_ok(d, dy_nstride) ? 1 : 0;
+}
+
+extern "C" int dcfp_conv2d_dgrad_chan_add_f32_nchw(const DcfpConvDesc* d, const float* dy, int64_t dy_nstride, const float* w,
+                                                   float* dx, const float* chan_add, float chan_scale, void* workspace,
+                                                   size_t workspace_bytes, int wp_valid, dcfp_stream_t stream) {
+    int rc = check_desc(d);
+    if (rc) return rc;
+    if (!dy || !w || !dx || !chan_add) return DCFP_E_BADDESC;
+    if (!dgrad_chan_add_ok(d, dy_nstride)) return DCFP_E_UNSUPPORTED;
+    const int T = d->KH * d->KW;
+    if (workspace_bytes < dcfp_wino_fused_workspace_bytes(d->N, d->H, d->W, d->dil, d->Cin, d->Cout)) return DCFP_E_WORKSPACE;
+    return dcfp_wino_fused_run(dy, dy_nstride ? dy_nstride : (long long)d->Cout * d->Hout * (d->dy_pitch ? d->dy_pitch : d->Wout),
+                               d->dy_pitch, w, T, d->Cin * T, 1, dx, (long long)d->Cin * d->H * d->W, d->N, d->Cin, d->Cout,
+                               d->H, d->W, d->dil, 1, workspace, workspace_bytes, dcfp_s(stream), nullptr, nullptr, nullptr,
+                               nullptr, nullptr, 0, (wp_valid && wino_keeps_u(d, DCFP_CONV_DGRAD)) ? 1 : 0, chan_add,
+                               chan_scale);
+}
+
 extern "C" int dcfp_conv2d_dgrad_fanin_supported(const DcfpConvDesc* d) {
     if (check_desc(d) != DCFP_OK || d->KH != 1 || d->stride != 1 || d->pad != 0 || math_bf16x3()) return 0;
     const int P = d->H * d->W;
@@ -451,6 +486,17 @@
     if (n == 0 || total_blocks == 0) return DCFP_OK;
     if (!table || n < 0 || total_blocks < 0 || total_blocks > 0x7fffffffLL) return DCFP_E_BADDESC;
     return dcfp_igemm2_permute_multi(table, n, total_blocks, dcfp_s(stream));
+}
+
+extern "C" int dcfp_conv2d_permute_weights_one_f32(const DcfpWpEntry* e, dcfp_stream_t stream) {
+    if (!e || !e->w || !e->wp || e->T < 1 || e->Ck < 1 || e->M < 1 || e->CkP < e->Ck || e->Mpad < e->M) return DCFP_E_BADDESC;
+    if (e->perm8 < 0 || e->perm8 > 3) return DCFP_E_BADDESC;
+    if (e->perm8 >= 2) {
+        if (e->CkP % 8 || e->Mpad % 64) return DCFP_E_BADDESC;
+        return dcfp_wino_filter2_run(e->w, e->sAm, e->sAc, e->perm8 == 3, e->M, e->Ck, e->CkP, e->Mpad, e->wp, dcfp_s(stream));
+    }
+    if (e->perm8 == 1 && e->Mpad % 256) return DCFP_E_BADDESC;
+    return dcfp_igemm2_permute_one(e, dcfp_s(stream));
 }
 
 bool dcfp_wgrad_pitch_ok(const DcfpConvDesc* d);
diff --git a/dcfp_amd/csrc/conv_igemm2.hip b/dcfp_amd/csrc/conv_igemm2.hip
--- a/dcfp_amd/csrc/conv_igemm2.hip
+++ b/dcfp_amd/csrc/conv_igemm2.hip
@@ -29,8 +29,99 @@
 }
 
 constexpr int kWpBlockElems = DCFP_WP_BLOCK_ELEMS;
+constexpr int kWpLdsFloats = 9 * (32 * 33 + 8);
+
+template <int T, int TC, int TM, int St>
+__device__ __forceinline__ void wp_stage_tile(const DcfpWpEntry& e, int c0, int p0, int perm, float* __restrict__ s) {
+    constexpr int L = TM / 8;
+    const bool m_runs = e.sAm == T && e.sAc != T;
+#pragma unroll 4
+    for (int f = threadIdx.x; f < T * TC * TM; f += 256) {
+        const int t = f % T, r = f / T;
+        int cl, jj;
+        if (m_runs) { jj = r % TM; cl = r / TM; } else { cl = r % TC; jj = r / TC; }
+        const int j = perm ? 8 * (jj % L) + jj / L : jj;
+        const int m = wp_row(p0 + j, perm), c = c0 + cl;
+        float v = 0.f;
+        if (m < e.M && c < e.Ck) v = e.w[(long long)m * e.sAm + (long long)c * e.sAc + t];
+        s[t * St + cl * (TM + 1) + j] = v;
+    }
+}
+
+template <int T, int TC, int TM>
+__device__ __forceinline__ void wp_copy_tiles(const DcfpWpEntry& e, long long b, float* __restrict__ s) {
+    constexpr int St = TC * (TM + 1) + 8;
+    static_assert(T * St <= kWpLdsFloats, "LDS tile");
+    const int tm = (e.Mpad + TM - 1) / TM;
+    const long long ntiles = (long long)((e.CkP + TC - 1) / TC) * tm;
+    const long long step = e.n_blocks > 0 ? e.n_blocks : 1;
+    for (long long tile = b; tile < ntiles; tile += step) {
+        const int ct = (int)(tile / tm), c0 = ct * TC, p0 = (int)(tile - (long long)ct * tm) * TM;
+        if (tile != b) __syncthreads();
+        wp_stage_tile<T, TC, TM, St>(e, c0, p0, e.perm8, s);
+        __syncthreads();
+#pragma unroll 4
+        for (int f = threadIdx.x; f < T * TC * TM; f += 256) {
+            const int j = f % TM, r = f / TM, cl = r % TC, t = r / TC;
+            if (c0 + cl < e.CkP && p0 + j < e.Mpad)
+                e.wp[((long long)t * e.CkP + (c0 + cl)) * e.Mpad + (p0 + j)] = s[t * St + cl * (TM + 1) + j];
+        }
+    }
+}
+
+__device__ __forceinline__ void wp_wino_tiles(const DcfpWpEntry& e, long long b, float* __restrict__ s) {
+    constexpr int TC = 8, TM = 64, St = TC * (TM + 1) + 16;
+    static_assert(9 * St <= kWpLdsFloats, "LDS tile");
+    const int mblocks = e.Mpad >> 6;
+    const long long ntiles = (long long)(e.CkP >> 3) * mblocks;
+    const long long step = e.n_blocks > 0 ? e.n_blocks : 1;
+    const bool flip = e.perm8 == 3;
+    const bool vec = ((unsigned long long)e.wp & 7) == 0;
+    const int tid = threadIdx.x, kh = tid & 1, ml = ((tid >> 7) << 5) + ((tid >> 1) & 31), h = (tid >> 6) & 1;
+    for (long long tile = b; tile < ntiles; tile += step) {
+        const int cb = (int)(tile / mblocks), mb = (int)(tile - (long long)cb * mblocks);
+        if (tile != b) __syncthreads();
+        wp_stage_tile<9, TC, TM, St>(e, cb * 8, mb * 64, 0, s);
+        __syncthreads();
+        float o[2][16];
+#pragma unroll
+        for (int q = 0; q < 2; ++q) {
+            const int cl = 2 * (2 * kh + q) + h;
+            float g[9];
+#pragma unroll
+            for (int t = 0; t < 9; ++t) g[t] = s[(flip ? 8 - t : t) * St + cl * (TM + 1) + ml];
+            float r[4][3];
+#pragma unroll
+            for (int k = 0; k < 3; ++k) {
+                const float g0 = g[k], g1 = g[3 + k], g2 = g[6 + k];
+                r[0][k] = g0;
+                r[1][k] = 0.5f * ((g0 + g2) + g1);
+                r[2][k] = 0.5f * ((g0 + g2) - g1);
+                r[3][k] = g2;
+            }
+#pragma unroll
+            for (int i = 0; i < 4; ++i) {
+                const float a = r[i][0], bb = r[i][1], cc = r[i][2];
+                o[q][4 * i + 0] = a;
+                o[q][4 * i + 1] = 0.5f * ((a + cc) + bb);
+                o[q][4 * i + 2] = 0.5f * ((a + cc) - bb);
+                o[q][4 * i + 3] = cc;
+            }
+        }
+        float* dst = e.wp + tile * 8192 + 2 * tid;
+        if (vec) {
+#pragma unroll
+            for (int xi = 0; xi < 16; ++xi) *reinterpret_cast<float2*>(dst + xi * 512) = make_float2(o[0][xi], o[1][xi]);
+        } else {
+#pragma unroll
+            for (int xi = 0; xi < 16; ++xi) { dst[xi * 512] = o[0][xi]; dst[xi * 512 + 1] = o[1][xi]; }
+        }
+    }
+}
+
 __global__ void __launch_bounds__(256)
 permute_weights_multi_kernel(const DcfpWpEntry* __restrict__ table, int n) {
+    __shared__ float s[kWpLdsFloats];
     const long long blk = blockIdx.x;
     int lo = 0, hi = n - 1;
     while (lo < hi) {
@@ -38,17 +129,14 @@
         if (table[mid].first_block <= blk) lo = mid; else hi = mid - 1;
     }
     const DcfpWpEntry e = table[lo];
-    const long long base = (blk - e.first_block) * kWpBlockElems;
+    const long long b = blk - e.first_block;
     if (e.perm8 >= 2) {
-        const long long pairs = (long long)e.CkP * e.Mpad;
-#pragma unroll 1
-        for (int u = 0; u < kWpBlockElems / 256; ++u) {
-            const long long i = base + u * 256 + threadIdx.x;
-            if (i >= pairs) return;
-            wino_filter2_pair(e.w, e.sAm, e.sAc, e.perm8 == 3, e.M, e.Ck, e.Mpad, i, e.wp);
-        }
+        wp_wino_tiles(e, b, s);
         return;
     }
+    if (e.T == 1) { wp_copy_tiles<1, 64, 64>(e, b, s); return; }
+    if (e.T == 9) { wp_copy_tiles<9, 32, 32>(e, b, s); return; }
+    const long long base = b * kWpBlockElems;
     const long long total = (long long)e.T * e.CkP * e.Mpad;
 #pragma unroll
     for (int u = 0; u < kWpBlockElems / 256; ++u) {
@@ -1011,6 +1099,15 @@
     DCFP_RETURN_LAUNCH();
 }
 
+int dcfp_igemm2_permute_one(const DcfpWpEntry* e, hipStream_t stream) {
+    const long long total = (long long)e->T * e->CkP * e->Mpad;
+    long long b = (total + 255) / 256;
+    if (b > 2048) b = 2048;
+    hipLaunchKernelGGL(permute_weights_kernel, dim3((unsigned)b), dim3(256), 0, stream, e->w, e->wp, e->T, e->Ck, e->CkP,
+                       e->M, e->Mpad, e->sAm, e->sAc, e->perm8);
+    DCFP_RETURN_LAUNCH();
+}
+
 bool dcfp_igemm2_persist() {
     static const bool persist = [] { const char* e = getenv("DCFP_IGEMM_PERSIST"); return !e || atoi(e) != 0; }();
     return persist;
diff --git a/dcfp_amd/csrc/conv_winograd.hip b/dcfp_amd/csrc/conv_winograd.hip
--- a/dcfp_amd/csrc/conv_winograd.hip
+++ b/dcfp_amd/csrc/conv_winograd.hip
@@ -17,7 +17,8 @@
 int dcfp_wino_fused_run(const float* in, long long in_nstride, int in_pitch, const float* w, int sAm, int sAc, int flip,
                         float* out, long long out_nstride, int N, int M, int Ck, int H, int W, int d, int accumulate,
                         void* workspace, size_t workspace_bytes, hipStream_t stream, float* xform_out, float* stat_part,
-                        const float* scale, const float* shift, const float* residual, int relu, int wp_valid);
+                        const float* scale, const float* shift, const float* residual, int relu, int wp_valid,
+                        const float* chan_add = nullptr, float chan_scale = 0.f);
 
 namespace {
 
diff --git a/dcfp_amd/csrc/conv_winograd2.hip b/dcfp_amd/csrc/conv_winograd2.hip
--- a/dcfp_amd/csrc/conv_winograd2.hip
+++ b/dcfp_amd/csrc/conv_winograd2.hip
@@ -29,7 +29,18 @@
     int ragged_c;
     int vec_epi;
     unsigned out_bytes;
+    const float* chan_add;
+    float chan_scale;
 };
+
+__device__ __forceinline__ float chan_term(float c, float s) {
+#pragma clang fp contract(off)
+    return c * s;
+}
+__device__ __forceinline__ float chan_plus(float v, float t) {
+#pragma clang fp contract(off)
+    return v + t;
+}
 
 template <int DM, bool SIDE, bool RAGGED>
 __global__ void __launch_bounds__(256, 1) wino_fused_kernel(const WinoFusedParams p) {
@@ -375,6 +386,12 @@
                 }
             }
             if (acc_out) v += __builtin_bit_cast(f32x4, __builtin_amdgcn_raw_buffer_load_b128(o_rsrc, vo, so, 0));
+            if (p.chan_add) {
+                const int mm = m_lane + mr < p.M ? m_lane + mr : p.M - 1;
+                const float t = chan_term(p.chan_add[(long long)n * p.M + mm], p.chan_scale);
+#pragma unroll
+                for (int e = 0; e < 4; ++e) v[e] = chan_plus(v[e], t);
+            }
             __builtin_amdgcn_raw_buffer_store_b128(__builtin_bit_cast(u32x4, v), o_rsrc, vo, so, 0);
         });
         return;
@@ -402,7 +419,13 @@
         }
         if (m < p.M) {
             float* e = obase + (long long)m * HW;
-            if (acc_out) {
+            if (acc_out && p.chan_add) {
+                const float t = chan_term(p.chan_add[(long long)n * p.M + m], p.chan_scale);
+                if (okr0 && okc0) e[0] = chan_plus(e[0] + o[0][0], t);
+                if (okr0 && okc1) e[d] = chan_plus(e[d] + o[0][1], t);
+                if (okr1 && okc0) e[dW] = chan_plus(e[dW] + o[1][0], t);
+                if (okr1 && okc1) e[dW + d] = chan_plus(e[dW + d] + o[1][1], t);
+            } else if (acc_out) {
                 if (okr0 && okc0) e[0] += o[0][0];
                 if (okr0 && okc1) e[d] += o[0][1];
                 if (okr1 && okc0) e[dW] += o[1][0];
@@ -476,6 +499,14 @@
     *CkP = pl.CkP; *Mpad = pl.Mpad;
 }
 
+int dcfp_wino_filter2_run(const float* w, int sAm, int sAc, int flip, int M, int Ck, int CkP, int Mpad, float* Ug,
+                          hipStream_t stream) {
+    long long b = ((long long)CkP * Mpad + 255) / 256;
+    if (b > 4096) b = 4096;
+    hipLaunchKernelGGL(wino_filter2_kernel, dim3((unsigned)b), dim3(256), 0, stream, w, sAm, sAc, flip, M, Ck, CkP, Mpad, Ug);
+    DCFP_RETURN_LAUNCH();
+}
+
 size_t dcfp_wino_fused_workspace_bytes(int N, int H, int W, int d, int M, int Ck) {
     return (size_t)fused_plan(N, H, W, d, M, Ck).ug_floats * sizeof(float);
 }
@@ -483,7 +514,9 @@
 int dcfp_wino_fused_run(const float* in, long long in_nstride, int in_pitch, const float* w, int sAm, int sAc, int flip,
                         float* out, long long out_nstride, int N, int M, int Ck, int H, int W, int d, int accumulate,
                         void* workspace, size_t workspace_bytes, hipStream_t stream, float* xform_out, float* stat_part,
-                        const float* scale, const float* shift, const float* residual, int relu, int wp_valid) {
+                        const float* scale, const float* shift, const float* residual, int relu, int wp_valid,
+                        const float* chan_add, float chan_scale) {
+    if (chan_add && (!accumulate || scale || stat_part || xform_out)) return DCFP_E_UNSUPPORTED;
     const FusedPlan pl = fused_plan(N, H, W, d, M, Ck);
     if (!workspace || !dcfp_aligned16(workspace) || workspace_bytes < (size_t)pl.ug_floats * sizeof(float))
         return DCFP_E_WORKSPACE;
@@ -514,6 +547,7 @@
     p.T = pl.T; p.T16 = pl.T16;
     p.mblocks = pl.mblocks; p.tblocks = pl.tblocks; p.nk = pl.nk;
     p.accumulate = accumulate;
+    p.chan_add = chan_add; p.chan_scale = chan_scale;
     p.ragged_c = (Ck % 16) != 0;
     {
         const long long ospan = ((long long)(N - 1) * out_nstride + (long long)M * H * W) * 4;
diff --git a/dcfp_amd/csrc/conv_winograd3.hip b/dcfp_amd/csrc/conv_winograd3.hip
--- a/dcfp_amd/csrc/conv_winograd3.hip
+++ b/dcfp_amd/csrc/conv_winograd3.hip
@@ -1,5 +1,7 @@
 #include "wino_patch.h"
 #include <stdlib.h>
+#include <atomic>
+#include <mutex>
 
 namespace {
 
@@ -392,6 +394,86 @@
     return pl;
 }
 
+struct WgTableKey {
+    int dev, N, H, W, d, TH, TW, x_pitch, lead, dy_pitch, dm;
+    long long x_nstride, dy_nstride, npairs, T;
+};
+bool wg_key_eq(const WgTableKey& a, const WgTableKey& b) {
+    return a.dev == b.dev && a.N == b.N && a.H == b.H && a.W == b.W && a.d == b.d && a.TH == b.TH && a.TW == b.TW &&
+           a.x_pitch == b.x_pitch && a.lead == b.lead && a.dy_pitch == b.dy_pitch && a.dm == b.dm &&
+           a.x_nstride == b.x_nstride && a.dy_nstride == b.dy_nstride && a.npairs == b.npairs && a.T == b.T;
+}
+
+std::atomic<long long> g_wg_table_builds{0}, g_wg_table_hits{0};
+
+void wg_table_build(unsigned* table, const WgTableKey& k, hipStream_t stream) {
+    hipLaunchKernelGGL(wino_wg_table_kernel, dim3((unsigned)((k.npairs + 255) / 256)), dim3(256), 0, stream, table, k.npairs, k.T,
+                       k.N, k.H, k.W, k.d, k.TH, k.TW, k.x_nstride, k.x_pitch, k.lead, k.dy_nstride, k.dy_pitch, k.dm);
+    g_wg_table_builds.fetch_add(1, std::memory_order_relaxed);
+}
+
+constexpr int kWgTableSlots = 32;
+struct WgTableSlot {
+    WgTableKey key;
+    hipStream_t stream;
+    unsigned* buf;
+    size_t cap;
+    int dev;
+    unsigned long long used;
+    bool valid;
+};
+
+bool wg_table_cache_enabled() {
+    static const bool v = [] { const char* e = getenv("DCFP_WINO_WG_TABLE_CACHE"); return !e || atoi(e) != 0; }();
+    return v;
+}
+
+const unsigned* wg_table_cached(WgTableKey key, hipStream_t stream) {
+    if (!wg_table_cache_enabled()) return nullptr;
+    hipStreamCaptureStatus cap = hipStreamCaptureStatusNone;
+    if (hipStreamIsCapturing(stream, &cap) != hipSuccess) { (void)hipGetLastError(); return nullptr; }
+    if (cap != hipStreamCaptureStatusNone) return nullptr;
+    if (hipGetDevice(&key.dev) != hipSuccess) { (void)hipGetLastError(); return nullptr; }
+    static std::mutex mu;
+    static WgTableSlot slots[kWgTableSlots] = {};
+    static unsigned long long tick = 0;
+    std::lock_guard<std::mutex> lock(mu);
+    WgTableSlot* lru = nullptr;
+    for (WgTableSlot& s : slots) {
+        if (s.valid && wg_key_eq(s.key, key)) {
+            if (s.stream != stream) return nullptr;
+            s.used = ++tick;
+            g_wg_table_hits.fetch_add(1, std::memory_order_relaxed);
+            return s.buf;
+        }
+        if (!lru || (lru->valid && !s.valid) || (lru->valid == s.valid && s.used < lru->used)) lru = &s;
+    }
+    const size_t bytes = (size_t)key.npairs * 32;
+    if (!lru->buf || lru->cap < bytes || lru->dev != key.dev || (lru->valid && lru->stream != stream)) {
+        lru->valid = false;
+        if (lru->buf) (void)hipFree(lru->buf);
+        lru->buf = nullptr;
+        lru->cap = 0;
+        void* ptr = nullptr;
+        if (hipMalloc(&ptr, bytes) != hipSuccess) { (void)hipGetLastError(); return nullptr; }
+        lru->buf = static_cast<unsigned*>(ptr);
+        lru->cap = bytes;
+        lru->dev = key.dev;
+    }
+    wg_table_build(lru->buf, key, stream);
+    lru->key = key;
+    lru->stream = stream;
+    lru->valid = true;
+    lru->used = ++tick;
+    return lru->buf;
+}
+
+}
+
+extern "C" int dcfp_wino_wgrad_table_counters(int64_t* builds, int64_t* hits) {
+    if (builds) *builds = g_wg_table_builds.load(std::memory_order_relaxed);
+    if (hits) *hits = g_wg_table_hits.load(std::memory_order_relaxed);
+    return DCFP_OK;
 }
 
 bool dcfp_wino_wgrad_fused_enabled() {
@@ -427,12 +509,17 @@
     const WgPlan pl = wg_plan(N, H, W, d, M, C);
     if (!workspace || !dcfp_aligned16(workspace) || workspace_bytes < dcfp_wino_wgrad_fused_workspace_bytes(N, H, W, d, M, C))
         return DCFP_E_WORKSPACE;
-    unsigned* table = static_cast<unsigned*>(workspace);
+    const unsigned* table = static_cast<const unsigned*>(workspace);
     float* slabs = static_cast<float*>(workspace) + pl.table_floats;
     const int lead = mode == 4 ? 0 : 4;
     const long long npairs = pl.T16 / 2;
-    hipLaunchKernelGGL(wino_wg_table_kernel, dim3((unsigned)((npairs + 255) / 256)), dim3(256), 0, stream, table, npairs, pl.T,
-                       N, H, W, d, pl.TH, pl.TW, x_nstride, x_pitch, lead, dy_nstride, dy_pitch, mode);
+    const WgTableKey key = {0, N, H, W, d, pl.TH, pl.TW, x_pitch, lead, dy_pitch, mode, x_nstride, dy_nstride, npairs, pl.T};
+    const unsigned* cached = wg_table_cached(key, stream);
+    if (cached) {
+        table = cached;
+    } else {
+        wg_table_build(static_cast<unsigned*>(workspace), key, stream);
+    }
     WinoWgParams p;
     p.x_base = x - lead;
     p.x_bytes = (unsigned)(((long long)(N - 1) * x_nstride + (long long)C * H * x_pitch + lead) * 4);
diff --git a/dcfp_amd/ops.py b/dcfp_amd/ops.py
--- a/dcfp_amd/ops.py
+++ b/dcfp_amd/ops.py
@@ -329,7 +329,23 @@
     return (y, None) if want_stats else y
 
 
-def conv2d_dgrad(dy, w, xshape, stride, pad, dil, out=None, accumulate=False):
+def conv2d_dgrad_chan_add_ok(dy, w, xshape, stride, pad, dil):
+    if not dy.is_cuda or not w.is_cuda:
+        return False
+    dp = _pitch_of(dy)
+    d = _desc(xshape, w.shape, stride, pad, dil, 0, dp)
+    N, Cc, H, W = dy.shape
+    st = dy.stride()
+    if dp:
+        ns = st[0]
+    elif st[3] == 1 and st[2] == W and st[1] == H * W and N > 1 and st[0] >= Cc * H * W:
+        ns = st[0]
+    else:
+        ns = Cc * H * W
+    return bool(_lib.lib().dcfp_conv2d_dgrad_chan_add_supported(C.byref(d), ns))
+
+
+def conv2d_dgrad(dy, w, xshape, stride, pad, dil, out=None, accumulate=False, chan_add=None, chan_scale=1.0):
     _require(dy, "dy")
     w = w if w.is_contiguous() else w.contiguous()
     dp = _pitch_of(dy)
@@ -347,6 +363,16 @@
         accumulate = False
     L = _lib.lib()
     ws, valid = _conv_workspace(w, _lib.CONV_DGRAD, d)
+    if chan_add is not None:
+        _require(chan_add, "chan_add")
+        if not accumulate:
+            raise RuntimeError("conv2d_dgrad: chan_add needs accumulate=True and out")
+        if chan_add.numel() != xshape[0] * xshape[1] or not chan_add.is_contiguous() or chan_add.dtype != torch.float32:
+            raise RuntimeError("conv2d_dgrad: chan_add must be a contiguous fp32 [N, Cin] tensor")
+        _timed("conv_dgrad", d, _conv_flops(d), lambda: check(
+            L.dcfp_conv2d_dgrad_chan_add_f32_nchw(C.byref(d), _p(dy), ns, _p(w), _p(dx), _p(chan_add), float(chan_scale),
+                                                  _p(ws), ws.numel(), valid, _stream()), "conv2d_dgrad_chan_add"))
+        return dx
     _timed("conv_dgrad", d, _conv_flops(d), lambda: check(
         L.dcfp_conv2d_dgrad_f32_nchw(C.byref(d), _p(dy), ns, _p(w), _p(dx), int(bool(accumulate)),
                                      _p(ws), ws.numel(), valid, _stream()), "conv2d_dgrad"))
@@ -1074,6 +1100,7 @@
         grads = [None] * 15
         dx = None
         pending = None
+        last = None
         for k in range(4):
             w, g, b = tensors[3 * k:3 * k + 3]
             pad, dil = convs[k]
@@ -1084,7 +1111,10 @@
             if pending is not None:
                 grads[3 * (k - 1)] = res[4]
             if need_dx:
-                dx = conv2d_dgrad(d_c, w, tuple(x.shape), 1, pad, dil, out=dx, accumulate=dx is not None)
+                if k == 3 and dx is not None and conv2d_dgrad_chan_add_ok(d_c, w, tuple(x.shape), 1, pad, dil):
+                    last = (d_c, w, pad, dil)
+                else:
+                    dx = conv2d_dgrad(d_c, w, tuple(x.shape), 1, pad, dil, out=dx, accumulate=dx is not None)
             pending = (lambda d_c=d_c, w=w, pad=pad, dil=dil, kp=ctx.keeps[k]:
                        wgrad_into_param(d_c, x, w, None, 1, pad, dil, keep=kp)[0])
         w5, g5, b5 = tensors[12:15]
@@ -1094,7 +1124,12 @@
         grads[12], _ = wgrad_into_param(d_c5, pooled, w5, None, 1, 0, 1)
         if need_dx:
             d_pooled = conv2d_dgrad(d_c5, w5, tuple(pooled.shape), 1, 0, 1)
-            dx = broadcast_hw(d_pooled, H, W, 1.0 / (H * W), out=dx, accumulate=dx is not None)
+            if last is not None:
+                d_c, w, pad, dil = last
+                dx = conv2d_dgrad(d_c, w, tuple(x.shape), 1, pad, dil, out=dx, accumulate=True,
+                                  chan_add=d_pooled.contiguous(), chan_scale=1.0 / (H * W))
+            else:
+                dx = broadcast_hw(d_pooled, H, W, 1.0 / (H * W), out=dx, accumulate=dx is not None)
         return (dx, None) + tuple(grads)
 
 
diff --git a/include/dcfp_hip.h b/include/dcfp_hip.h
--- a/include/dcfp_hip.h
+++ b/include/dcfp_hip.h
@@ -41,6 +41,7 @@
 int dcfp_conv2d_wp_layout(const DcfpConvDesc* d, int pass, DcfpWpEntry* entry);
 int dcfp_conv2d_permute_weights_multi_f32(const DcfpWpEntry* table, int n_entries, int64_t total_blocks,
                                           dcfp_stream_t stream);
+int dcfp_conv2d_permute_weights_one_f32(const DcfpWpEntry* entry, dcfp_stream_t stream);
 
 int dcfp_conv2d_pitch_supported(const DcfpConvDesc* d);
 
@@ -84,10 +85,16 @@
                                const float* w, float* dx, int accumulate,
                                void* workspace, size_t workspace_bytes, int wp_valid,
                                dcfp_stream_t stream);
+int dcfp_conv2d_dgrad_chan_add_supported(const DcfpConvDesc* d, int64_t dy_nstride);
+int dcfp_conv2d_dgrad_chan_add_f32_nchw(const DcfpConvDesc* d, const float* dy, int64_t dy_nstride,
+                                        const float* w, float* dx, const float* chan_add, float chan_scale,
+                                        void* workspace, size_t workspace_bytes, int wp_valid,
+                                        dcfp_stream_t stream);
 int dcfp_conv2d_wgrad_f32_nchw(const DcfpConvDesc* d, const float* dy, int64_t dy_nstride,
                                const float* x, float* dw, float* db,
                                void* workspace, size_t workspace_bytes,
                                dcfp_stream_t stream);
+int dcfp_wino_wgrad_table_counters(int64_t* builds, int64_t* hits);
 
 typedef struct DcfpBnRunning {
     float* running_mean;
```

Result: no change. 12.25 images/s, median of 6 (+0.2%).
